# zjykzj/YOLOv4

Hardware: AMD Instinct MI355X
Metric: images/sec fwd+bwd @608x608 bs=64 per GPU (YOLOv4 training step: forward + YOLOLoss + backward) (higher is better)
Workload: dtype f32

## Files before the change

### include/yolov4_amd.h

```cpp
#ifndef YOLOV4_AMD_H
#define YOLOV4_AMD_H

#include <stddef.h>
#include <stdint.h>

#ifdef __cplusplus
extern "C" {
#endif

#define Y4_OK 0
#define Y4_ERR_SHAPE 1
#define Y4_ERR_NULL 2
#define Y4_ERR_LAUNCH 3
#define Y4_ERR_WORKSPACE 4
#define Y4_ERR_NODEVICE 5

#define Y4_ACT_LINEAR 0
#define Y4_ACT_LEAKY 1
#define Y4_ACT_MISH 2
#define Y4_ACT_RELU 3

const char* y4_strerror(int code);
int y4_version(void);
int y4_device_count(void);

int y4_set_conv_mode(int mode);
int y4_get_conv_mode(void);
int y4_set_planes_bf16(int on);
int y4_get_planes_bf16(void);
int y4_conv_planes_fit(int B, int H, int W, int Cin, int Cout, int k, int stride, int dgrad_planes);
size_t y4_conv2d_fwd_workspace(int Cin, int Cout, int k);
int y4_conv2d_fwd_f32(const float* x, int ldx, const float* w, float* y, int ldy,
                      int B, int H, int W, int Cin, int Cout, int k, int stride,
                      const float* scale, const float* shift, int act,
                      const float* residual, int ldr, const unsigned* x_amax ,
                      unsigned* y_amax ,
                      void* workspace, size_t workspace_bytes, void* stream);
size_t y4_conv2d_prepared_bytes(int Cout, int K);
int y4_conv2d_prepare_filter_f32(const float* w, int Cout, int K, void* prepared, size_t prepared_bytes, void* stream);
int y4_conv2d_fwd_prepared_f32(const float* x, int ldx, void* w_prepared, float* y, int ldy,
                               int B, int H, int W, int Cin, int Cout, int k, int stride,
                               const float* scale, const float* shift, int act,
                               const float* residual, int ldr, const unsigned* x_amax, unsigned* y_amax, void* stream);
int y4_amax_f32(const float* x, int ldx, long long M, int C, unsigned* amax_bits, void* stream);
int y4_amax_merge_u32(unsigned* dst, const unsigned* src, void* stream);

int y4_last_conv_kernel(char* buf, int cap);

size_t y4_conv2d_bnstats_workspace(int B, int H, int W, int Cin, int Cout, int k, int stride);
int y4_conv2d_fwd_bnstats_f32(const float* x, int ldx, const float* w, float* y, int ldy,
                              int B, int H, int W, int Cin, int Cout, int k, int stride,
                              float* partials, size_t partial_bytes, long long* nparts_host,
                              const unsigned* x_amax ,
                              void* workspace, size_t workspace_bytes ,
                              void* dgrad_filter ,
                              size_t dgrad_filter_bytes , void* stream);

int y4_planes_split_f32(const float* x, int ldx, long long M, int C, const unsigned* amax, void* planes, void* stream);
int y4_planes_split_into_f32(const float* x, int ldx, long long M, int C, const unsigned* amax, void* planes, int ld_planes, int c_valid,
                             void* stream);
int y4_conv2d_fwd_planes_f32(const void* x_planes, const float* w, float* y, int ldy,
                             int B, int H, int W, int Cin, int Cout, int k, int stride,
                             float* partials, size_t partial_bytes, long long* nparts_host, const unsigned* x_amax,
                             void* workspace, size_t workspace_bytes,
                             void* dgrad_filter ,
                             size_t dgrad_filter_bytes,
                             int y_bf16 ,
                             const float* bias ,
                             void* stream);

int y4_conv2d_dgrad_planes_f32(const void* dy_planes, const float* w , float* dx, int lddx,
                               int B, int H, int W, int Cin, int Cout, int k,
                               int stride ,
                               void* workspace, size_t workspace_bytes, const unsigned* dy_amax,
                               const float* residual, int ldr, void* stream);
size_t y4_conv2d_wgrad_planes_workspace(int B, int H, int W, int Cin, int Cout, int k, int stride);
int y4_conv2d_wgrad_planes_f32(const void* x_planes, const void* dy_planes, float* dw,
                               int B, int H, int W, int Cin, int Cout, int k, int stride,
                               void* workspace, size_t workspace_bytes, const unsigned* x_amax, const unsigned* dy_amax,
                               void* stream);

int y4_conv2d_generic_fwd_f32(const float* x, int ldx, const float* w, float* y, int ldy,
                              int B, int H, int W, int Cin, int Cout, int k, int stride,
                              const float* scale, const float* shift, int act, const float* residual, int ldr, void* stream);
int y4_conv2d_generic_dgrad_f32(const float* dy, int lddy, const float* w, float* dx, int lddx,
                                int B, int H, int W, int Cin, int Cout, int k, int stride,
                                const float* residual, int ldr, void* stream);
int y4_conv2d_generic_wgrad_f32(const float* x, int ldx, const float* dy, int lddy, float* dw,
                                int B, int H, int W, int Cin, int Cout, int k, int stride, void* stream);
int y4_conv2d_stem_dgrad_f32(const float* dy, int lddy, const float* w, float* dx, long long sxb, long long sxc, long long sxh,
                             long long sxw, int B, int H, int W, int Cout, void* stream);

int y4_conv2d_stem_fwd_f32(const float* x, long long sxb, long long sxc, long long sxh, long long sxw,
                           const float* w, float* y, int ldy, int B, int H, int W, int Cout,
                           const float* scale, const float* shift, int act,
                           float* bnstats_partials, void* stream);

size_t y4_conv2d_dgrad_workspace(int Cin, int Cout, int k);
int y4_conv2d_dgrad_f32(const float* dy, int lddy, const float* w , float* dx, int lddx,
                        int B, int H, int W, int Cin, int Cout, int k, int stride,
                        void* workspace, size_t workspace_bytes, const unsigned* dy_amax ,
                        const float* residual, int ldr, void* stream);

size_t y4_conv2d_wgrad_workspace(int B, int H, int W, int Cin, int Cout, int k, int stride);
int y4_conv2d_wgrad_f32(const float* x, int ldx, const float* dy, int lddy, float* dw,
                        int B, int H, int W, int Cin, int Cout, int k, int stride,
                        void* workspace, size_t workspace_bytes,
                        const unsigned* x_amax, const unsigned* dy_amax , void* stream);
size_t y4_conv2d_stem_wgrad_workspace(int B, int H, int W, int Cout);
int y4_conv2d_stem_wgrad_f32(const float* x, long long sxb, long long sxc, long long sxh, long long sxw,
                             const float* dy, int lddy, float* dw, int B, int H, int W, int Cout,
                             void* workspace, size_t workspace_bytes, void* stream);

size_t y4_bn_workspace(long long M, int C);
size_t y4_bn_finalize_workspace(int C);
int y4_bn_stats_f32(const float* y, int ldy, long long M, int C, float* mean, float* invstd,
                    float* running_mean, float* running_var, long long* num_batches_tracked,
                    float momentum, float eps, void* workspace, size_t workspace_bytes, void* stream);
int y4_bn_finalize_partials_f32(const float* partials, long long nparts, long long M, int C,
                                float* mean, float* invstd, float* running_mean, float* running_var,
                                long long* num_batches_tracked, float momentum, float eps,
                                void* workspace, size_t workspace_bytes, void* stream);
int y4_bn_planes_bound_f32(const float* gamma, const float* beta, int C, long long M, const unsigned* floor_word, unsigned* out,
                           void* stream);
int y4_bn_act_fwd_f32(const float* y, int ldy, const float* mean, const float* invstd,
                      const float* gamma, const float* beta, int act,
                      const float* residual, int ldr, float* z, int ldz,
                      long long M, int C, unsigned* out_amax, int z_planes, const unsigned* res_amax, float* planes_twin,
                      void* stream);
int y4_bn_act_bwd_f32(const float* dz, int lddz, const float* y, int ldy,
                      const float* mean, const float* invstd, const float* gamma, const float* beta,
                      int act, float* dy, int lddy, float* dgamma, float* dbeta,
                      long long M, int C, void* workspace, size_t workspace_bytes,
                      unsigned* out_amax ,
                      unsigned* f16_planes ,
                      float* planes_twin ,
                      int frozen_stats ,
                      void* stream);
size_t y4_bias_grad_workspace(long long M, int C);
int y4_bias_grad_f32(const float* dy, int lddy, long long M, int C, float* dbias,
                     void* workspace, size_t workspace_bytes, void* stream);
int y4_bn_fold_f32(const float* gamma, const float* beta, const float* running_mean,
                   const float* running_var, float eps, float* scale, float* shift, int C, void* stream);

int y4_copy_channels_f32(const float* src, int lds, float* dst, int ldd, long long M, int C, void* stream);
int y4_add_f32(const float* a, int lda, const float* b, int ldb, float* out, int ldo,
               long long M, int C, void* stream);
int y4_maxpool_s1_fwd_f32(const float* x, int ldx, float* y, int ldy, signed char* idx,
                          int B, int H, int W, int C, int ksize, void* stream);
int y4_maxpool_s1_bwd_f32(const float* dy, int lddy, const signed char* idx, float* dx, int lddx,
                          int accumulate, int B, int H, int W, int C, int ksize, void* stream);
int y4_upsample2x_fwd_f32(const float* x, int ldx, float* y, int ldy, int B, int H, int W, int C, void* stream);
int y4_upsample2x_bwd_f32(const float* dy, int lddy, float* dx, int lddx, int B, int H, int W, int C, void* stream);

int y4_yolo_decode_train_f32(const float* logits, int ldl, float* output, float* pred,
                             int B, int F, int A, int n_classes, const float* anchors_wh_host, void* stream);
int y4_yolo_decode_eval_f32(const float* logits, int ldl, float* out, long long n_total, long long box_off,
                            int B, int F, int A, int n_classes, const float* anchors_wh_host,
                            float stride, void* stream);
int y4_yolo_decode_bwd_f32(const float* logits, int ldl, const float* g_output, const float* g_pred,
                           float* g_logits, int B, int F, int A, int n_classes,
                           const float* anchors_wh_host, void* stream);

size_t y4_yolo_loss_workspace(int B, int F, int A, int K, int n_classes);
int y4_yolo_loss_fwd_f32(const float* output, const float* pred, const float* labels, int K,
                         int B, int F, int A, int n_classes, float stride, float ignore_thresh,
                         const float* all_anchors_host, int n_all_anchors, const int* anch_mask_host,
                         float* obj_mask, double* loss_parts,
                         void* workspace, size_t workspace_bytes, void* stream);
int y4_yolo_loss_bwd_f32(const float* output, int output_is_masked, const float* obj_mask,
                         const float* gscale, float* g_output,
                         int B, int F, int A, int K, int n_classes,
                         const void* workspace, size_t workspace_bytes, void* stream);
int y4_yolo_loss_mask_output_f32(float* output, const float* obj_mask, int B, int F, int A, int K,
                                 int n_classes, const void* workspace, size_t workspace_bytes, void* stream);
int y4_yolo_loss_dense_targets_f32(float* target, float* tgt_mask, float* tgt_scale,
                                   int B, int F, int A, int K, int n_classes,
                                   const void* workspace, size_t workspace_bytes, void* stream);

int y4_post_scan_i32(const int* counts, int n_segments, long long cap, int* seg_offsets, int* info, void* stream);
int y4_post_compact_f32(const float* det_rows, const int* seg_offsets, const int* kept, int B, int n_classes,
                        float* out_rows, int* out_offsets, int* img_offsets, void* stream);
int y4_post_count_f32(float* prediction, int B, long long N, int n_classes, float conf_thre,
                      int convert_xyxy, int* counts, void* stream);
size_t y4_post_nms_workspace(long long total_candidates, int n_segments);
int y4_post_nms_f32(const float* prediction, int B, long long N, int n_classes, float conf_thre,
                    float nms_thre, const int* seg_offsets , long long total_candidates,
                    float* det_rows , int* kept ,
                    void* workspace, size_t workspace_bytes, void* stream);
size_t y4_nms_workspace(long long R);
int y4_nms_f32(const float* boxes, const float* scores , long long R, float thresh,
               int limit, int* keep_idx , int* n_keep ,
               void* workspace, size_t workspace_bytes, void* stream);

int y4_bboxes_iou_f32(const float* boxes_a, long long Na, const float* boxes_b, long long Nb, int xyxy, float* iou,
                      void* stream);
int y4_act_fwd_f32(const float* x, float* y, long long n, int act, void* stream);
int y4_act_bwd_f32(const float* x, const float* dy, float* dx, long long n, int act, void* stream);
int y4_upsample_nearest_fwd_f32(const float* x, int ldx, float* y, int ldy, int B, int H, int W, int Ho, int Wo, int C,
                                int integer_factor, void* stream);
int y4_upsample_nearest_bwd_f32(const float* dy, int lddy, float* dx, int lddx, int B, int H, int W, int Ho, int Wo, int C,
                                int integer_factor, void* stream);

int y4_adam_step_f32(float* param, const float* grad, float* exp_avg, float* exp_avg_sq, long long n,
                     float lr, float beta1, float beta2, float eps, float weight_decay, int step,
                     float grad_scale, void* stream);
int y4_adam_hyper_f32(float lr, float beta1, float beta2, float weight_decay, int step, float* out4_host);
int y4_adam_multi_step_f32(const void* chunks_dev, int nchunks, const float* hyper_host, int nhyper,
                           float beta1, float beta2, float eps, float grad_scale, void* stream);
int y4_sgd_multi_step_f32(const void* chunks_dev, int nchunks, const float* hyper_host, int nhyper,
                          float grad_scale, void* stream);

int y4_preprocess_u8_f32(const void* src, int src_h, int src_w, long long src_pitch_bytes, int swap_rb,
                         float* dst, long long dst_sc, long long dst_sh, long long dst_sw, int S, void* stream);

#ifdef __cplusplus
}
#endif
#endif
```

### yolov4_amd/_lib.py

```python
import ctypes
import os
from ctypes import c_char_p, c_double, c_float, c_int, c_longlong, c_size_t, c_void_p

_HERE = os.path.dirname(os.path.abspath(__file__))
LIB_PATH = os.environ.get('Y4_LIB_PATH') or os.path.join(_HERE, 'lib', 'libyolov4_amd.so')

ACT_IDS = {'linear': 0, 'leaky_relu': 1, 'mish': 2, 'relu': 3}


class Y4Error(RuntimeError):
    pass


P = c_void_p
I, L, F, Z = c_int, c_longlong, c_float, c_size_t

PROTOTYPES = {
    'y4_strerror': (c_char_p, [I]),
    'y4_version': (I, []),
    'y4_device_count': (I, []),
    'y4_set_conv_mode': (I, [I]),
    'y4_get_conv_mode': (I, []),
    'y4_set_planes_bf16': (I, [I]),
    'y4_get_planes_bf16': (I, []),
    'y4_conv_planes_fit': (I, [I, I, I, I, I, I, I, I]),
    'y4_conv2d_fwd_workspace': (Z, [I, I, I]),
    'y4_conv2d_fwd_f32': (I, [P, I, P, P, I, I, I, I, I, I, I, I, P, P, I, P, I, P, P, P, Z, P]),
    'y4_amax_f32': (I, [P, I, L, I, P, P]),
    'y4_conv2d_prepared_bytes': (Z, [I, I]),
    'y4_conv2d_prepare_filter_f32': (I, [P, I, I, P, Z, P]),
    'y4_conv2d_fwd_prepared_f32': (I, [P, I, P, P, I, I, I, I, I, I, I, I, P, P, I, P, I, P, P, P]),
    'y4_amax_merge_u32': (I, [P, P, P]),
    'y4_last_conv_kernel': (I, [ctypes.c_char_p, I]),
    'y4_conv2d_bnstats_workspace': (Z, [I, I, I, I, I, I, I]),
    'y4_conv2d_fwd_bnstats_f32': (I, [P, I, P, P, I, I, I, I, I, I, I, I, P, Z, P, P, P, Z, P, Z, P]),
    'y4_planes_split_f32': (I, [P, I, L, I, P, P, P]),
    'y4_planes_split_into_f32': (I, [P, I, L, I, P, P, I, I, P]),
    'y4_conv2d_fwd_planes_f32': (I, [P, P, P, I, I, I, I, I, I, I, I, P, Z, P, P, P, Z, P, Z, I, P, P]),
    'y4_conv2d_dgrad_planes_f32': (I, [P, P, P, I, I, I, I, I, I, I, I, P, Z, P, P, I, P]),
    'y4_conv2d_wgrad_planes_workspace': (Z, [I, I, I, I, I, I, I]),
    'y4_conv2d_wgrad_planes_f32': (I, [P, P, P, I, I, I, I, I, I, I, P, Z, P, P, P]),
    'y4_conv2d_generic_fwd_f32': (I, [P, I, P, P, I, I, I, I, I, I, I, I, P, P, I, P, I, P]),
    'y4_conv2d_generic_dgrad_f32': (I, [P, I, P, P, I, I, I, I, I, I, I, I, P, I, P]),
    'y4_conv2d_generic_wgrad_f32': (I, [P, I, P, I, P, I, I, I, I, I, I, I, P]),
    'y4_conv2d_stem_dgrad_f32': (I, [P, I, P, P, L, L, L, L, I, I, I, I, P]),
    'y4_conv2d_stem_fwd_f32': (I, [P, L, L, L, L, P, P, I, I, I, I, I, P, P, I, P, P]),
    'y4_conv2d_dgrad_workspace': (Z, [I, I, I]),
    'y4_conv2d_dgrad_f32': (I, [P, I, P, P, I, I, I, I, I, I, I, I, P, Z, P, P, I, P]),
    'y4_conv2d_wgrad_workspace': (Z, [I, I, I, I, I, I, I]),
    'y4_conv2d_wgrad_f32': (I, [P, I, P, I, P, I, I, I, I, I, I, I, P, Z, P, P, P]),
    'y4_conv2d_stem_wgrad_workspace': (Z, [I, I, I, I]),
    'y4_conv2d_stem_wgrad_f32': (I, [P, L, L, L, L, P, I, P, I, I, I, I, P, Z, P]),
    'y4_bn_workspace': (Z, [L, I]),
    'y4_bn_finalize_workspace': (Z, [I]),
    'y4_bn_finalize_partials_f32': (I, [P, L, L, I, P, P, P, P, P, F, F, P, Z, P]),
    'y4_bn_stats_f32': (I, [P, I, L, I, P, P, P, P, P, F, F, P, Z, P]),
    'y4_bn_act_fwd_f32': (I, [P, I, P, P, P, P, I, P, I, P, I, L, I, P, I, P, P, P]),
    'y4_bn_planes_bound_f32': (I, [P, P, I, L, P, P, P]),
    'y4_bn_act_bwd_f32': (I, [P, I, P, I, P, P, P, P, I, P, I, P, P, L, I, P, Z, P, P, P, I, P]),
    'y4_bias_grad_workspace': (Z, [L, I]),
    'y4_bias_grad_f32': (I, [P, I, L, I, P, P, Z, P]),
    'y4_bn_fold_f32': (I, [P, P, P, P, F, P, P, I, P]),
    'y4_copy_channels_f32': (I, [P, I, P, I, L, I, P]),
    'y4_add_f32': (I, [P, I, P, I, P, I, L, I, P]),
    'y4_maxpool_s1_fwd_f32': (I, [P, I, P, I, P, I, I, I, I, I, P]),
    'y4_maxpool_s1_bwd_f32': (I, [P, I, P, P, I, I, I, I, I, I, I, P]),
    'y4_upsample2x_fwd_f32': (I, [P, I, P, I, I, I, I, I, P]),
    'y4_upsample2x_bwd_f32': (I, [P, I, P, I, I, I, I, I, P]),
    'y4_yolo_decode_train_f32': (I, [P, I, P, P, I, I, I, I, P, P]),
    'y4_yolo_decode_eval_f32': (I, [P, I, P, L, L, I, I, I, I, P, F, P]),
    'y4_yolo_decode_bwd_f32': (I, [P, I, P, P, P, I, I, I, I, P, P]),
    'y4_yolo_loss_workspace': (Z, [I, I, I, I, I]),
    'y4_yolo_loss_fwd_f32': (I, [P, P, P, I, I, I, I, I, F, F, P, I, P, P, P, P, Z, P]),
    'y4_yolo_loss_bwd_f32': (I, [P, I, P, P, P, I, I, I, I, I, P, Z, P]),
    'y4_yolo_loss_mask_output_f32': (I, [P, P, I, I, I, I, I, P, Z, P]),
    'y4_yolo_loss_dense_targets_f32': (I, [P, P, P, I, I, I, I, I, P, Z, P]),
    'y4_post_count_f32': (I, [P, I, L, I, F, I, P, P]),
    'y4_post_scan_i32': (I, [P, I, L, P, P, P]),
    'y4_post_compact_f32': (I, [P, P, P, I, I, P, P, P, P]),
    'y4_post_nms_workspace': (Z, [L, I]),
    'y4_post_nms_f32': (I, [P, I, L, I, F, F, P, L, P, P, P, Z, P]),
    'y4_nms_workspace': (Z, [L]),
    'y4_nms_f32': (I, [P, P, L, F, I, P, P, P, Z, P]),
    'y4_bboxes_iou_f32': (I, [P, L, P, L, I, P, P]),
    'y4_act_fwd_f32': (I, [P, P, L, I, P]),
    'y4_act_bwd_f32': (I, [P, P, P, L, I, P]),
    'y4_upsample_nearest_fwd_f32': (I, [P, I, P, I, I, I, I, I, I, I, I, P]),
    'y4_upsample_nearest_bwd_f32': (I, [P, I, P, I, I, I, I, I, I, I, I, P]),
    'y4_adam_step_f32': (I, [P, P, P, P, L, F, F, F, F, F, I, F, P]),
    'y4_adam_hyper_f32': (I, [F, F, F, F, I, P]),
    'y4_adam_multi_step_f32': (I, [P, I, P, I, F, F, F, F, P]),
    'y4_sgd_multi_step_f32': (I, [P, I, P, I, F, P]),
    'y4_preprocess_u8_f32': (I, [P, I, I, L, I, P, L, L, L, I, P]),
}

_lib = None


def lib():
    global _lib
    if _lib is None:
        if not os.path.isfile(LIB_PATH):
            raise Y4Error(f'{LIB_PATH} is missing: build it with `make -C yolov4_amd/csrc` '
                          '(hipcc --offload-arch=gfx950); there is no fallback path')
        handle = ctypes.CDLL(LIB_PATH)
        for name, (res, args) in PROTOTYPES.items():
            fn = getattr(handle, name)
            fn.restype = res
            fn.argtypes = args
        _lib = handle
        if os.environ.get('Y4_CONV_MODE'):
            handle.y4_set_conv_mode(int(os.environ['Y4_CONV_MODE']))
    return _lib


def check(code, what=''):
    if code != 0:
        msg = lib().y4_strerror(code).decode()
        raise Y4Error(f'{what}: {msg} (code {code})')


def float_array(values):
    arr = (c_float * len(values))(*[float(v) for v in values])
    return arr


def int_array(values):
    return (c_int * len(values))(*[int(v) for v in values])
```

### yolov4_amd/csrc/conv_geom.h

```cpp
#pragma once
#include "common.h"

namespace y4 {

struct ConvGeom {
    const float* src; const float* wt; float* dst;
    const float* scale; const float* shift; const float* res;
    float* stats;
    long long lds_, ldd, ldr;
    int B, Hs, Ws, Cs;
    int Cs_valid;
    int Hd, Wd, N;
    int k, stride, pad;
    int M;
    int K;
    int act;
    int mtiles, ntiles;
    int cls_tile0[5];
    int cls_h[2], cls_w[2];
    int cls_slot0[5];
    unsigned long long src_total_bytes;
    unsigned wt_bytes;
    const unsigned short* wt_planes;
    const unsigned* src_amax; const unsigned* wt_amax;
    unsigned* dst_amax;
};

struct WgradGeom {
    const float* x; const float* dy; float* out;
    long long ldx, lddy;
    int B, H, W, Cin, Ho, Wo, Cout;
    int k, stride, pad;
    int M;
    int J;
    int ntn, ntj, splits, chunks_per_split;
    int tn, tj;
    const unsigned* x_amax; const unsigned* dy_amax;
    unsigned long long x_total_bytes, dy_total_bytes;
};

int f16x2_gather(const ConvGeom& g, bool transposed, hipStream_t st, int* nparts);
int f16x2_wgrad(const WgradGeom& g, hipStream_t st);
int f16x2_refresh_prepared(const float* w, void* prepared, int Cout, int K, hipStream_t st);
int f16x2_filter_planes(const float* w, unsigned short* planes, int Cout, int K, unsigned* amax_out, unsigned* part, hipStream_t st);
int f16x2_filter_planes_dual(const float* w, unsigned short* planes, unsigned* amax_out, unsigned* part, unsigned short* planes_t,
                             unsigned* amax_out_t, int Cout, int Cin, int kk, int Cout_pad, bool mirror, hipStream_t st);
int f16x2_filter_planes_transposed(const float* w, unsigned short* planes, int Cout, int Cin, int kk, int Cout_pad,
                                   unsigned* amax_out, unsigned* part, hipStream_t st, bool mirror = false);
int slab_reduce(const float* slabs, float* dw, long long n, int splits, hipStream_t st);
int amax_launch(const float* x, long long ld, long long M, int C, unsigned* amax_bits, hipStream_t st,
                bool prezeroed = false);
int amax_merge(unsigned* dst, const unsigned* src, hipStream_t st);


bool tile_conv_ok(int Cs, int Cs_valid, int N, int k, int stride, int H, int W);
int f16x2_tile(const ConvGeom& g, hipStream_t st, int* nparts);
bool tile_dgrad_s2_ok(int Cs, int Cs_valid, int N, int k, int stride, int Hs, int Ws);
int f16x2_tile_dgrad_s2(const ConvGeom& g, hipStream_t st);

bool tile_wgrad_ok(int Cin, int Cout, int k, int stride, int H, int W, long long ldx, long long lddy);
int tile_wgrad_slabs(int Cin, int Cout);
int f16x2_wgrad_tile(const WgradGeom& g, hipStream_t st);

bool planes_conv_ok(int Cin, int Cout, int k, int stride);
int planes_conv(const void* src, const unsigned* src_amax, const void* wt_planes, const unsigned* wt_amax, float* dst, long long ldd,
                const float* res, long long ldr, float* stats, int* nparts, int B, int Hs, int Ws, int Cs, int N, int k, int stride,
                hipStream_t st, bool bf = false, bool dst_bf16 = false);
int planes_dgrad_s2(const void* dy, const unsigned* dy_amax, const void* wt_planes, const unsigned* wt_amax, float* dx, long long lddx,
                    int B, int H, int W, int Cin, int Cout, hipStream_t st, bool bf = false);
int planes_split(const float* x, long long ld, long long M, int C, const unsigned* amax, void* planes, hipStream_t st, bool bf = false,
                 long long pitch_ch = 0, int c_valid = 0);
void planes_wgrad_plan(int B, int H, int W, int Cin, int Cout, int k, int* ntn, int* ntj, int* splits, int* sps, int tn = 128, bool bf = false);
int planes_wgrad_tn(int Cout, bool bf);
int planes_wgrad(const void* x, const unsigned* x_amax, const void* dy, const unsigned* dy_amax, float* dw, void* workspace,
                 size_t workspace_bytes, int B, int H, int W, int Cin, int Cout, int k, hipStream_t st, bool bf = false,
                 int stride = 1);

void note_kernel(const char* fmt, ...);
}
```

### yolov4_amd/csrc/conv_igemm.hip

```cpp
#include <stdlib.h>
#include "common.h"
#include <cstdarg>
#include <cstdio>
#include "conv_geom.h"

namespace {

constexpr int BK = 32;


using y4::ConvGeom;
using y4::WgradGeom;

template <int BM, int BN, int WM, int WN, bool TRANSPOSED, int BKT = 32>
__global__ __launch_bounds__(256, (BKT == 16 ? 3 : 2)) void conv_gather_mfma_f32(const ConvGeom g) {
    constexpr int LPR = BKT / 4;
    constexpr int RPP = 256 / LPR;
    constexpr int PA = BM / RPP, PB = BN / RPP;
    constexpr int LDS_PITCH = BKT + 4;
    constexpr int BK = BKT;
    constexpr int WTM = BM / WM, WTN = BN / WN;
    constexpr int TM = WTM / 32, TN = WTN / 32;
    static_assert(WM * WN == 4, "4 waves");
    extern __shared__ __attribute__((aligned(16))) float smem[];
// ... 1073 lines not shown
    f32x4 ra[4], rb[4];
    int ld_chunk = 0;
    auto load_chunk = [&]() {
        const int pbase = (chunk0 + ld_chunk) * 32 + pg * 4;
#pragma unroll
        for (int i = 0; i < 4; ++i) {
            const bool ok = an_ok && pbase + i < g.M;
            ra[i] = y4_buf_load4(dy_rsrc, ok ? a_off0 + (unsigned)i * dy_pix_bytes : OOB, (unsigned)ld_chunk * chunk_bytes);
        }
#pragma unroll
        for (int i = 0; i < 4; ++i) {
            const int hi = pb_h[i] * g.stride - g.pad + jr, wi = pb_w[i] * g.stride - g.pad + jq;
            const bool ok = bj_ok && pbase + i < g.M && (unsigned)hi < (unsigned)g.H && (unsigned)wi < (unsigned)g.W;
            const unsigned off = (unsigned)((pb_b[i] * g.H + hi) * g.W + wi) * x_pix_bytes + (unsigned)jc * 4u;
            rb[i] = y4_buf_load4(x_rsrc, ok ? off : OOB, 0u);
            pb_w[i] += 32;
            while (pb_w[i] >= g.Wo) { pb_w[i] -= g.Wo; if (++pb_h[i] == g.Ho) { pb_h[i] = 0; ++pb_b[i]; } }
        }
        ++ld_chunk;
    };
    auto split_store = [&](const f32x4 (&v)[4], unsigned char* base, int rows) {
        if constexpr (NP == 1) {
#pragma unroll
            for (int e = 0; e < 4; ++e) {
                u32x2 p;
                p[0] = pack_hi16(rn_bf16_bits(v[1][e]), rn_bf16_bits(v[0][e]));
                p[1] = pack_hi16(rn_bf16_bits(v[3][e]), rn_bf16_bits(v[2][e]));
                *reinterpret_cast<u32x2*>(base + (cg * 4 + e) * PITCH_B + pg * 8) = p;
            }
            return;
        }
        unsigned h1[4][4], h2[4][4], h3[4][4];
#pragma unroll
        for (int i = 0; i < 4; ++i)
#pragma unroll
            for (int e = 0; e < 4; ++e) {
                h1[i][e] = __float_as_uint(v[i][e]);
                const float r1 = v[i][e] - __uint_as_float(h1[i][e] & 0xffff0000u);
                h2[i][e] = __float_as_uint(r1);
                const float r2 = r1 - __uint_as_float(h2[i][e] & 0xffff0000u);
                h3[i][e] = __float_as_uint(r2);
            }
#pragma unroll
        for (int e = 0; e < 4; ++e) {
            unsigned char* d = base + (cg * 4 + e) * PITCH_B + pg * 8;
            u32x2 p;
            p[0] = pack_hi16(h1[1][e], h1[0][e]); p[1] = pack_hi16(h1[3][e], h1[2][e]);
            *reinterpret_cast<u32x2*>(d) = p;
            p[0] = pack_hi16(h2[1][e], h2[0][e]); p[1] = pack_hi16(h2[3][e], h2[2][e]);
            *reinterpret_cast<u32x2*>(d + rows * PITCH_B) = p;
            p[0] = pack_hi16(h3[1][e], h3[0][e]); p[1] = pack_hi16(h3[3][e], h3[2][e]);
            *reinterpret_cast<u32x2*>(d + 2 * rows * PITCH_B) = p;
        }
    };
    auto store_chunk = [&]() {
        if (a_act) split_store(ra, As, TN_);
        if (b_act) split_store(rb, Bs, TJ_);
    };

    f32x16 acc[MI][MJ];
#pragma unroll
    for (int i = 0; i < MI; ++i)
#pragma unroll
        for (int jj = 0; jj < MJ; ++jj)
#pragma unroll
            for (int e = 0; e < 16; ++e) acc[i][jj][e] = 0.f;

    const int fr = lane & 31, fh = lane >> 5;
    const unsigned char* a_frag = As + (wm * (TN_ / 2) + fr) * PITCH_B + fh * 16;
    const unsigned char* b_frag = Bs + (wn * (TJ_ / 2) + fr) * PITCH_B + fh * 16;
    if (nchunks > 0) {
        load_chunk();
        store_chunk();
        __syncthreads();
        for (int ch = 0; ch < nchunks; ++ch) {
            if (ch + 1 < nchunks) load_chunk();
#pragma unroll
            for (int ks = 0; ks < 2; ++ks) {
                bf16x8 fa[MI][NP], fb[MJ][NP];
#pragma unroll
                for (int i = 0; i < MI; ++i)
#pragma unroll
                    for (int pl = 0; pl < NP; ++pl)
                        fa[i][pl] = *reinterpret_cast<const bf16x8*>(a_frag + pl * TN_ * PITCH_B + i * 32 * PITCH_B + ks * 32);
#pragma unroll
                for (int jj = 0; jj < MJ; ++jj)
#pragma unroll
                    for (int pl = 0; pl < NP; ++pl)
                        fb[jj][pl] = *reinterpret_cast<const bf16x8*>(b_frag + pl * TJ_ * PITCH_B + jj * 32 * PITCH_B + ks * 32);
#pragma unroll
                for (int i = 0; i < MI; ++i)
#pragma unroll
                    for (int jj = 0; jj < MJ; ++jj) {
                        f32x16 c = acc[i][jj];
                        if constexpr (NP == 3) {
                            c = __builtin_amdgcn_mfma_f32_32x32x16_bf16(fa[i][2], fb[jj][0], c, 0, 0, 0);
                            c = __builtin_amdgcn_mfma_f32_32x32x16_bf16(fa[i][1], fb[jj][1], c, 0, 0, 0);
                            c = __builtin_amdgcn_mfma_f32_32x32x16_bf16(fa[i][0], fb[jj][2], c, 0, 0, 0);
                            c = __builtin_amdgcn_mfma_f32_32x32x16_bf16(fa[i][1], fb[jj][0], c, 0, 0, 0);
                            c = __builtin_amdgcn_mfma_f32_32x32x16_bf16(fa[i][0], fb[jj][1], c, 0, 0, 0);
                        }
                        c = __builtin_amdgcn_mfma_f32_32x32x16_bf16(fa[i][0], fb[jj][0], c, 0, 0, 0);
                        acc[i][jj] = c;
                    }
            }
            __syncthreads();
            if (ch + 1 < nchunks) store_chunk();
            __syncthreads();
        }
    }
    float* out = g.out + (long long)split * g.Cout * g.J;
#pragma unroll
    for (int jj = 0; jj < MJ; ++jj) {
        const int jcol = j0 + wn * (TJ_ / 2) + jj * 32 + fr;
#pragma unroll
        for (int i = 0; i < MI; ++i) {
            const int nb = n0 + wm * (TN_ / 2) + i * 32 + 4 * fh;
#pragma unroll
            for (int e = 0; e < 16; ++e) {
                const int n = nb + (e & 3) + 8 * (e >> 2);
                if (n < g.Cout && jcol < g.J) out[(long long)n * g.J + jcol] = acc[i][jj][e];
            }
        }
    }
}

template <int VEC>
__global__ __launch_bounds__(256) void slab_reduce_vec_kernel(const f32x4* __restrict__ slabs, f32x4* __restrict__ out,
                                                              long long nvec, int splits) {
    constexpr int SG = 256 / VEC;
    __shared__ f32x4 red[SG][VEC];
    const int v = threadIdx.x % VEC, sg = threadIdx.x / VEC;
    const long long i = (long long)blockIdx.x * VEC + v;
    f32x4 s0 = {0.f, 0.f, 0.f, 0.f}, s1 = s0, s2 = s0, s3 = s0;
    if (i < nvec) {
        int k = sg;
        for (; k + 3 * SG < splits; k += 4 * SG) {
            const f32x4 a = slabs[(long long)k * nvec + i], b = slabs[(long long)(k + SG) * nvec + i];
            const f32x4 c = slabs[(long long)(k + 2 * SG) * nvec + i], d = slabs[(long long)(k + 3 * SG) * nvec + i];
            s0 += a; s1 += b; s2 += c; s3 += d;
        }
        for (; k < splits; k += SG) s0 += slabs[(long long)k * nvec + i];
    }
    red[sg][v] = (s0 + s1) + (s2 + s3);
    __syncthreads();
    if (sg == 0 && i < nvec) {
        f32x4 t = red[0][v];
#pragma unroll
        for (int g = 1; g < SG; ++g) t += red[g][v];
        out[i] = t;
    }
}

__global__ void slab_reduce_kernel(const float* __restrict__ slabs, float* __restrict__ out,
                                   long long n, int splits) {
    for (long long i = blockIdx.x * (long long)blockDim.x + threadIdx.x; i < n;
         i += (long long)gridDim.x * blockDim.x) {
        float s = 0.f;
        for (int k = 0; k < splits; ++k) s += slabs[(long long)k * n + i];
        out[i] = s;
    }
}

void wgrad_plan(int B, int H, int W, int Cin, int Cout, int k, int stride, WgradGeom& g) {
    const int pad = (k - 1) / 2;
    g.B = B; g.H = H; g.W = W; g.Cin = Cin; g.Cout = Cout; g.k = k; g.stride = stride; g.pad = pad;
    g.Ho = (H + 2 * pad - k) / stride + 1;
    g.Wo = (W + 2 * pad - k) / stride + 1;
    g.M = B * g.Ho * g.Wo;
    g.J = k * k * Cin;
    g.tn = Cout <= 64 ? 64 : 128;
    g.tj = g.J <= 64 ? 64 : 128;
    g.ntn = (Cout + g.tn - 1) / g.tn;
    g.ntj = (g.J + g.tj - 1) / g.tj;
    const int tiles = g.ntn * g.ntj;
    const int chunks = (g.M + 31) / 32;
    int per_cu = (160 * 1024) / (2 * 32 * (g.tn + g.tj) * 4);
    if (per_cu > 4) per_cu = 4;
    if (g.tn + g.tj == 256 && per_cu > 2) per_cu = 2;
    const int slots = 256 * per_cu;
    int max_s = chunks / 16;
    if (max_s < 1) max_s = 1;
    if (max_s > 4096) max_s = 4096;
    int best_s = 1;
    double best_eff = -1.0;
    for (int sp = 1; sp <= max_s; ++sp) {
        const long long blocks = (long long)tiles * sp;
        const long long rounds = (blocks + slots - 1) / slots;
        double eff = (double)blocks / (double)(rounds * slots);
        if (rounds > 6) eff = 1.0;
        if (eff > best_eff + 0.02) { best_eff = eff; best_s = sp; }
        if (blocks >= 2ll * slots && eff >= 0.93) break;
        if (blocks >= 6ll * slots) break;
    }
    { static const char* fs = getenv("Y4_WGRAD_SPLITS"); if (fs) { best_s = atoi(fs); if (best_s > max_s) best_s = max_s; if (best_s < 1) best_s = 1; } }
    g.chunks_per_split = (chunks + best_s - 1) / best_s;
    const unsigned long long per_px = 8ull * (unsigned long long)((Cout + 3) / 4 * 4 > Cin * stride * stride ? (Cout + 3) / 4 * 4 : Cin * stride * stride);
    const unsigned long long slack = 2ull * g.Ho * g.Wo;
    const unsigned long long max_px = 0xf0000000ull / per_px;
    if (max_px > slack + 32 && (unsigned long long)g.chunks_per_split * 32ull + slack > max_px)
        g.chunks_per_split = (int)((max_px - slack) / 32ull);
    g.splits = (chunks + g.chunks_per_split - 1) / g.chunks_per_split;
}

template <int TN_, int TJ_, int NP = 0>
int launch_wgrad(const WgradGeom& g, hipStream_t st) {
    constexpr bool SPLIT = NP > 0;
    const size_t smem = SPLIT ? (size_t)NP * (TN_ + TJ_) * 80 : 2ull * 32 * (TN_ + TJ_) * sizeof(float);
    void (*kern)(const WgradGeom);
    if constexpr (SPLIT) kern = conv_wgrad_bf16x3<TN_, TJ_, (NP > 0 ? NP : 3)>;
    else kern = conv_wgrad_mfma_f32<TN_, TJ_>;
    static Y4DynLds lds_attr;
    if (!lds_attr.ensure(reinterpret_cast<const void*>(kern), smem)) return Y4_ERR_LAUNCH;
    hipLaunchKernelGGL(kern, dim3(g.ntn * g.ntj * g.splits), dim3(256), smem, st, g);
    Y4_CHECK_LAUNCH();
    return Y4_OK;
}

struct StemGeom {
    const float* x; const float* w; float* y; const float* scale; const float* shift;
    float* stats;
    long long sxb, sxc, sxh, sxw, ldy;
    int B, H, W, Cout, act;
    long long M;
};

__global__ __launch_bounds__(256) void conv_stem_fwd_kernel(const StemGeom g) {
    __shared__ float tile[4][64][33];
    __shared__ __attribute__((aligned(16))) float wl[27 * 32];
    const int tid = threadIdx.x, lane = tid & 63, wave = tid >> 6;
    for (int i = tid; i < 27 * 32; i += 256) {
        const int n = i & 31, kk = i >> 5;
        wl[i] = n < g.Cout ? g.w[n * 27 + kk] : 0.f;
    }
    __syncthreads();
    const long long pix0 = (long long)blockIdx.x * 256 + wave * 64;
    const long long pix = pix0 + lane;
    float acc[32];
#pragma unroll
    for (int n = 0; n < 32; ++n) acc[n] = 0.f;
    if (pix < g.M) {
        const int b = (int)(pix / ((long long)g.H * g.W));
        const int rem = (int)(pix - (long long)b * g.H * g.W);
        const int h = rem / g.W, w = rem - h * g.W;
        const float* xb = g.x + b * g.sxb;
        float xv[27];
#pragma unroll
        for (int r = 0; r < 3; ++r)
#pragma unroll
            for (int q = 0; q < 3; ++q) {
                const int hi = h + r - 1, wi = w + q - 1;
                const bool ok = (unsigned)hi < (unsigned)g.H && (unsigned)wi < (unsigned)g.W;
#pragma unroll
                for (int c = 0; c < 3; ++c) xv[(r * 3 + q) * 3 + c] = ok ? xb[c * g.sxc + hi * g.sxh + wi * g.sxw] : 0.f;
            }
#pragma unroll
        for (int kk = 0; kk < 27; ++kk) {
            const f32x4* wp = reinterpret_cast<const f32x4*>(wl + kk * 32);
            const float v = xv[kk];
#pragma unroll
            for (int n4 = 0; n4 < 8; ++n4) {
                const f32x4 wv = wp[n4];
#pragma unroll
                for (int e = 0; e < 4; ++e) acc[n4 * 4 + e] = fmaf(v, wv[e], acc[n4 * 4 + e]);
            }
            __builtin_amdgcn_sched_barrier(0);
        }
    }
#pragma unroll
    for (int n = 0; n < 32; ++n) {
        float v = acc[n];
        if (n < g.Cout) {
            v = v * (g.scale ? g.scale[n] : 1.f) + (g.shift ? g.shift[n] : 0.f);
            v = y4_act(v, g.act);
        }
        tile[wave][lane][n] = v;
    }
    __syncthreads();
    const int ch = lane & 31;
    if (ch < g.Cout) {
#pragma unroll 4
        for (int it = 0; it < 32; ++it) {
            const int pl = it * 2 + (lane >> 5);
            const long long p = pix0 + pl;
            if (p < g.M) g.y[p * g.ldy + ch] = tile[wave][pl][ch];
        }
    }
    if (g.stats) {
        __shared__ float sred[8][32][2];
        const int grp = tid >> 5;
        float cs = 0.f, css = 0.f;
        for (int i = 0; i < 32; ++i) { const float v = tile[grp >> 1][(grp & 1) * 32 + i][ch]; cs += v; css += v * v; }
        sred[grp][ch][0] = cs; sred[grp][ch][1] = css;
        __syncthreads();
        if (tid < 64) {
            const int c = tid & 31, which = tid >> 5;
            float t = 0.f;
            for (int k = 0; k < 8; ++k) t += sred[k][c][which];
            if (c < g.Cout) g.stats[((long long)blockIdx.x * 2 + which) * g.Cout + c] = t;
        }
    }
}

__global__ __launch_bounds__(256) void conv_stem_fwd_bf16x3_kernel(const StemGeom g, const int ngroups, const float inv_hw,
                                                                   const float inv_w) {
    __shared__ float sred[4][32][2];
    const int tid = threadIdx.x, lane = tid & 63, wave = tid >> 6;
    const int fr = lane & 31, fh = lane >> 5;
    const int HW = g.H * g.W;
    bf16x8 fb[2][3];
    int koff[16];
    int ktap[16];
#pragma unroll
    for (int i = 0; i < 16; ++i) {
        const int k = (i >> 3) * 16 + fh * 8 + (i & 7);
        const int r = k / 9, c = (k - r * 9) / 3, q = k - r * 9 - c * 3;
        const bool kv = k < 27;
        koff[i] = kv ? (int)(c * g.sxc + (r - 1) * g.sxh + (q - 1) * g.sxw) * 4 : 0;
        ktap[i] = kv ? r * 3 + q : 9;
    }
#pragma unroll
    for (int ks = 0; ks < 2; ++ks) {
        f32x4 w0, w1;
#pragma unroll
        for (int i = 0; i < 8; ++i) {
            const int k = ks * 16 + fh * 8 + i;
            const int r = k / 9, c = (k - r * 9) / 3, q = k - r * 9 - c * 3;
            const float v = (k < 27 && fr < g.Cout) ? g.w[fr * 27 + (r * 3 + q) * 3 + c] : 0.f;
            if (i < 4) w0[i] = v; else w1[i - 4] = v;
        }
        u32x2 a1, a2, a3, b1, b2, b3;
        split3x4(w0, a1, a2, a3);
        split3x4(w1, b1, b2, b3);
        const u32x4 q1 = {a1[0], a1[1], b1[0], b1[1]}, q2 = {a2[0], a2[1], b2[0], b2[1]}, q3 = {a3[0], a3[1], b3[0], b3[1]};
        fb[ks][0] = __builtin_bit_cast(bf16x8, q1); fb[ks][1] = __builtin_bit_cast(bf16x8, q2); fb[ks][2] = __builtin_bit_cast(bf16x8, q3);
    }
    const float sc = (g.scale && fr < g.Cout) ? g.scale[fr] : 1.f;
    const float sh = (g.shift && fr < g.Cout) ? g.shift[fr] : 0.f;
    const __amdgpu_buffer_rsrc_t rsrc = y4_make_rsrc(g.x, 0xfffffff0u);
    float xv0[16], xv1[16];
    auto load = [&](float (&xv)[16], long long tile) {
        const long long p = tile * 32 + fr;
        unsigned base = 0xffffffffu;
        unsigned m9 = 0;
        if (p < g.M) {
            int b = (int)((float)p * inv_hw);
            int rem = (int)(p - (long long)b * HW);
            if (rem < 0) { --b; rem += HW; } else if (rem >= HW) { ++b; rem -= HW; }
            int h = (int)((float)rem * inv_w);
            int w = rem - h * g.W;
            if (w < 0) { --h; w += g.W; } else if (w >= g.W) { ++h; w -= g.W; }
            base = (unsigned)(b * g.sxb + h * g.sxh + w * g.sxw) * 4u;
            const unsigned hm = (h > 0 ? 1u : 0u) | 2u | (h + 1 < g.H ? 4u : 0u);
            const unsigned wm = (w > 0 ? 1u : 0u) | 2u | (w + 1 < g.W ? 4u : 0u);
            m9 = ((hm & 1u) ? wm : 0u) | ((hm & 2u) ? wm << 3 : 0u) | ((hm & 4u) ? wm << 6 : 0u);
        }
#pragma unroll
        for (int i = 0; i < 16; ++i) {
            const bool ok = (m9 >> ktap[i]) & 1u;
            xv[i] = __builtin_bit_cast(float, __builtin_amdgcn_raw_buffer_load_b32(rsrc, ok ? (int)(base + (unsigned)koff[i]) : -1, 0, 0));
        }
    };
    float cs = 0.f, css = 0.f;
    auto compute = [&](float (&xv)[16], long long tile) {
        f32x16 acc;
#pragma unroll
        for (int e = 0; e < 16; ++e) acc[e] = 0.f;
#pragma unroll
        for (int ks = 0; ks < 2; ++ks) {
            const f32x4 v0 = {xv[ks * 8 + 0], xv[ks * 8 + 1], xv[ks * 8 + 2], xv[ks * 8 + 3]};
            const f32x4 v1 = {xv[ks * 8 + 4], xv[ks * 8 + 5], xv[ks * 8 + 6], xv[ks * 8 + 7]};
            u32x2 a1, a2, a3, b1, b2, b3;
            split3x4(v0, a1, a2, a3);
            split3x4(v1, b1, b2, b3);
            const u32x4 q1 = {a1[0], a1[1], b1[0], b1[1]}, q2 = {a2[0], a2[1], b2[0], b2[1]}, q3 = {a3[0], a3[1], b3[0], b3[1]};
            const bf16x8 f1 = __builtin_bit_cast(bf16x8, q1), f2 = __builtin_bit_cast(bf16x8, q2), f3 = __builtin_bit_cast(bf16x8, q3);
            acc = __builtin_amdgcn_mfma_f32_32x32x16_bf16(f3, fb[ks][0], acc, 0, 0, 0);
            acc = __builtin_amdgcn_mfma_f32_32x32x16_bf16(f2, fb[ks][1], acc, 0, 0, 0);
            acc = __builtin_amdgcn_mfma_f32_32x32x16_bf16(f1, fb[ks][2], acc, 0, 0, 0);
            acc = __builtin_amdgcn_mfma_f32_32x32x16_bf16(f2, fb[ks][0], acc, 0, 0, 0);
            acc = __builtin_amdgcn_mfma_f32_32x32x16_bf16(f1, fb[ks][1], acc, 0, 0, 0);
            acc = __builtin_amdgcn_mfma_f32_32x32x16_bf16(f1, fb[ks][0], acc, 0, 0, 0);
        }
        const long long mbase = tile * 32 + 4 * fh;
#pragma unroll
        for (int e = 0; e < 16; ++e) {
            const float raw = acc[e];
            cs += raw; css += raw * raw;
            const long long m = mbase + (e & 3) + 8 * (e >> 2);
            if (fr < g.Cout && m < g.M) g.y[m * g.ldy + fr] = y4_act(raw * sc + sh, g.act);
        }
    };
    for (int grp = blockIdx.x; grp < ngroups; grp += gridDim.x) {
        const long long t0 = (long long)grp * 8 + wave * 2;
        load(xv0, t0);
        load(xv1, t0 + 1);
        cs = 0.f; css = 0.f;
        compute(xv0, t0);
        compute(xv1, t0 + 1);
        if (g.stats) {
            cs += __shfl_xor(cs, 32, 64);
            css += __shfl_xor(css, 32, 64);
            if (fh == 0) { sred[wave][fr][0] = cs; sred[wave][fr][1] = css; }
            __syncthreads();
            if (tid < 64) {
                const int c = tid & 31, which = tid >> 5;
                const float t = (sred[0][c][which] + sred[1][c][which]) + (sred[2][c][which] + sred[3][c][which]);
                if (c < g.Cout) g.stats[((long long)grp * 2 + which) * g.Cout + c] = t;
            }
            __syncthreads();
        }
    }
}

struct StemWgradGeom {
    const float* x; const float* dy; float* slabs;
    long long sxb, sxc, sxh, sxw, lddy;
    int B, H, W, Cout;
    long long M, pix_per_wave;
};

__global__ __launch_bounds__(256) void conv_stem_wgrad_kernel(const StemWgradGeom g) {
    const int tid = threadIdx.x, lane = tid & 63;
    const long long wave_id = (long long)blockIdx.x * 4 + (tid >> 6);
    const long long p_begin = wave_id * g.pix_per_wave;
    long long p_end = p_begin + g.pix_per_wave;
    if (p_end > g.M) p_end = g.M;
    const int fr = lane & 31, fh = lane >> 5;
    const bool jok = fr < 27;
    const int tap = jok ? fr / 3 : 0, c = jok ? fr - tap * 3 : 0;
    const int r = tap / 3 - 1, q = tap - (tap / 3) * 3 - 1;
    const bool nok = fr < g.Cout;
    f32x16 acc;
#pragma unroll
    for (int e = 0; e < 16; ++e) acc[e] = 0.f;
    long long p = p_begin + fh;
    int b = 0, h = 0, w = 0;
    if (p < g.M) {
        b = (int)(p / ((long long)g.H * g.W));
        const int rem = (int)(p - (long long)b * g.H * g.W);
        h = rem / g.W; w = rem - h * g.W;
    }
    const long long dy_first = p_begin < g.M ? p_begin : 0;
    const __amdgpu_buffer_rsrc_t dy_rsrc = y4_make_rsrc(g.dy + dy_first * g.lddy, (unsigned)(g.pix_per_wave * g.lddy * 4));
    const __amdgpu_buffer_rsrc_t x_rsrc = y4_make_rsrc(g.x, 0xfffffff0u);
    const unsigned dy_step = (unsigned)g.lddy * 8u;
    unsigned dy_off = ((unsigned)fh * (unsigned)g.lddy + (unsigned)fr) * 4u;
    const long long coff = c * g.sxc;
    for (long long pc = p_begin; pc < p_end; pc += 16) {
        float a[8], bv[8];
#pragma unroll
        for (int u = 0; u < 8; ++u) {
            const bool pok = p < p_end;
            const int hi = h + r, wi = w + q;
            const bool xok = pok && jok && (unsigned)hi < (unsigned)g.H && (unsigned)wi < (unsigned)g.W;
            const unsigned xo = (unsigned)(b * g.sxb + coff + hi * g.sxh + wi * g.sxw) * 4u;
            a[u] = __builtin_bit_cast(float, __builtin_amdgcn_raw_buffer_load_b32(dy_rsrc, (pok && nok) ? (int)dy_off : -1, 0, 0));
            bv[u] = __builtin_bit_cast(float, __builtin_amdgcn_raw_buffer_load_b32(x_rsrc, xok ? (int)xo : -1, 0, 0));
            dy_off += dy_step;
            p += 2;
            w += 2;
            if (w >= g.W) { w -= g.W; if (++h == g.H) { h = 0; ++b; } }
        }
#pragma unroll
        for (int u = 0; u < 8; ++u) acc = __builtin_amdgcn_mfma_f32_32x32x2f32(a[u], bv[u], acc, 0, 0, 0);
    }
    float* out = g.slabs + wave_id * 1024;
#pragma unroll
    for (int e = 0; e < 16; ++e) {
        const int n = (e & 3) + 8 * (e >> 2) + 4 * fh;
        out[n * 32 + fr] = acc[e];
    }
}

__global__ __launch_bounds__(256) void stem_wgrad_reduce1_kernel(const float* __restrict__ slabs, double* __restrict__ part,
                                                                 int nslabs) {
    const int per = (nslabs + gridDim.x - 1) / gridDim.x;
    const int k0 = blockIdx.x * per;
    const int k1 = min(nslabs, k0 + per);
    double s[4] = {0, 0, 0, 0};
    for (int k = k0; k < k1; ++k) {
        const f32x4 v = *reinterpret_cast<const f32x4*>(slabs + (long long)k * 1024 + threadIdx.x * 4);
#pragma unroll
        for (int e = 0; e < 4; ++e) s[e] += (double)v[e];
    }
#pragma unroll
    for (int e = 0; e < 4; ++e) part[(long long)blockIdx.x * 1024 + threadIdx.x * 4 + e] = s[e];
}
__global__ __launch_bounds__(256) void stem_wgrad_reduce2_kernel(const double* __restrict__ part, float* __restrict__ dw,
                                                                 int nparts, int Cout) {
    for (int i = threadIdx.x; i < Cout * 27; i += 256) {
        const int n = i / 27, j = i - n * 27;
        double s = 0.0;
        for (int k = 0; k < nparts; ++k) s += part[(long long)k * 1024 + n * 32 + j];
        dw[i] = (float)s;
    }
}

constexpr int STEM_WAVES = 4096;

}

namespace y4 {
int slab_reduce(const float* slabs, float* dw, long long n, int splits, hipStream_t st) {
    if ((n & 3) == 0 && !(reinterpret_cast<uintptr_t>(dw) & 15) && !(reinterpret_cast<uintptr_t>(slabs) & 15)) {
        const long long nvec = n / 4;
        if (nvec >= 64 * 1024)
            hipLaunchKernelGGL(slab_reduce_vec_kernel<64>, dim3((unsigned)((nvec + 63) / 64)), dim3(256), 0, st,
                               reinterpret_cast<const f32x4*>(slabs), reinterpret_cast<f32x4*>(dw), nvec, splits);
        else
            hipLaunchKernelGGL(slab_reduce_vec_kernel<16>, dim3((unsigned)((nvec + 15) / 16)), dim3(256), 0, st,
                               reinterpret_cast<const f32x4*>(slabs), reinterpret_cast<f32x4*>(dw), nvec, splits);
    } else {
        const int blocks = (int)((n + 255) / 256 > 2048 ? 2048 : (n + 255) / 256);
        hipLaunchKernelGGL(slab_reduce_kernel, dim3(blocks), dim3(256), 0, st, slabs, dw, n, splits);
    }
    Y4_CHECK_LAUNCH();
    return Y4_OK;
}
}

extern "C" {

int y4_set_conv_mode(int mode) {
    if (mode < 0 || mode > 3) return Y4_ERR_SHAPE;
    g_conv_mode = mode;
    return Y4_OK;
}
int y4_get_conv_mode(void) { return g_conv_mode; }

constexpr size_t FWD_WS_HDR = 64 + 4096;

size_t y4_conv2d_fwd_workspace(int Cin, int Cout, int k) {
    if (Cin <= 0 || Cout <= 0 || k <= 0) return 0;
    return FWD_WS_HDR + (size_t)Cout * k * k * Cin * 6;
}

static int conv_fwd_impl(const float* x, int ldx, const float* w, float* y, int ldy,
                         int B, int H, int W, int Cin, int Cout, int k, int stride,
                         const float* scale, const float* shift, int act,
                         const float* residual, int ldr, float* stats, int* nparts, const unsigned* x_amax,
                         unsigned* y_amax, void* workspace, size_t workspace_bytes, void* stream,
                         void* w_prepared = nullptr, void* dgrad_filter = nullptr, size_t dgrad_filter_bytes = 0) {
    if (!x || (!w && !w_prepared) || !y) return Y4_ERR_NULL;
    if (B <= 0 || H <= 0 || W <= 0 || Cout <= 0 || (k != 1 && k != 3) || (stride != 1 && stride != 2))
        return Y4_ERR_SHAPE;
    if (Cin <= 0 || Cin % BK != 0 || ldx < Cin || ldy < Cout || (ldx & 3) || (residual && ldr < Cout))
        return Y4_ERR_SHAPE;
    if ((reinterpret_cast<uintptr_t>(x) & 15) || (reinterpret_cast<uintptr_t>(w) & 15)) return Y4_ERR_SHAPE;
    const int pad = (k - 1) / 2;
    ConvGeom g{};
    g.src = x; g.wt = w; g.dst = y; g.scale = scale; g.shift = shift; g.res = residual; g.stats = stats;
    g.lds_ = ldx; g.ldd = ldy; g.ldr = ldr;
    g.B = B; g.Hs = H; g.Ws = W; g.Cs = Cin; g.Cs_valid = Cin;
    g.Hd = (H + 2 * pad - k) / stride + 1;
    g.Wd = (W + 2 * pad - k) / stride + 1;
    g.N = Cout; g.k = k; g.stride = stride; g.pad = pad;
    const long long M = (long long)B * g.Hd * g.Wd;
    if (M >= (1ll << 31)) return Y4_ERR_SHAPE;
    g.M = (int)M; g.K = k * k * Cin; g.act = act;
    if (w_prepared) {
        if (g_conv_mode != 3) return Y4_ERR_SHAPE;
        if (reinterpret_cast<uintptr_t>(w_prepared) & 15) return Y4_ERR_SHAPE;
        unsigned* hdr = static_cast<unsigned*>(w_prepared);
        g.wt_planes = reinterpret_cast<unsigned short*>(static_cast<char*>(w_prepared) + 64 + 4096);
        if (!x_amax) {
            const int rc = y4::amax_launch(x, ldx, (long long)B * H * W, Cin, hdr + 1, y4_stream(stream));
            if (rc != Y4_OK) return rc;
            x_amax = hdr + 1;
        }
        g.src_amax = x_amax; g.wt_amax = hdr; g.dst_amax = y_amax;
        return y4::f16x2_gather(g, false, y4_stream(stream), nparts);
    }
    if (g_conv_mode != 0) {
        const long long nw = (long long)Cout * g.K;
        if (!workspace) return Y4_ERR_NULL;
        if (workspace_bytes < y4_conv2d_fwd_workspace(Cin, Cout, k)) return Y4_ERR_WORKSPACE;
        if (reinterpret_cast<uintptr_t>(workspace) & 15) return Y4_ERR_SHAPE;
        unsigned* hdr = static_cast<unsigned*>(workspace);
        unsigned short* planes = reinterpret_cast<unsigned short*>(static_cast<char*>(workspace) + FWD_WS_HDR);
        g.wt_planes = planes;
        if (g_conv_mode == 3) {
            int rc;
            if (dgrad_filter) {
                if (dgrad_filter_bytes < y4_conv2d_dgrad_workspace(Cin, Cout, k)) return Y4_ERR_WORKSPACE;
                if (reinterpret_cast<uintptr_t>(dgrad_filter) & 15) return Y4_ERR_SHAPE;
                const int cp = (Cout + 31) / 32 * 32;
                unsigned* hdr_t = reinterpret_cast<unsigned*>(static_cast<char*>(dgrad_filter) + (size_t)Cin * k * k * cp * 6);
                rc = y4::f16x2_filter_planes_dual(w, planes, hdr, hdr + 16, static_cast<unsigned short*>(dgrad_filter), hdr_t, Cout, Cin,
                                                  k * k, cp, y4::tile_conv_ok(cp, Cout, Cin, k, stride, H, W), y4_stream(stream));
            } else {
                rc = y4::f16x2_filter_planes(w, planes, Cout, g.K, hdr, hdr + 16, y4_stream(stream));
            }
            if (rc != Y4_OK) return rc;
            if (!x_amax) {
                rc = y4::amax_launch(x, ldx, (long long)B * H * W, Cin, hdr + 1, y4_stream(stream));
                if (rc != Y4_OK) return rc;
                x_amax = hdr + 1;
            }
            g.src_amax = x_amax; g.wt_amax = hdr; g.dst_amax = y_amax;
            return y4::f16x2_gather(g, false, y4_stream(stream), nparts);
        }
        const int blocks = (int)((nw + 255) / 256 > 4096 ? 4096 : (nw + 255) / 256);
        hipLaunchKernelGGL(split_filter_kernel, dim3(blocks), dim3(256), 0, y4_stream(stream), w, planes, nw,
                           g_conv_mode == 2 ? 1 : 3);
        Y4_CHECK_LAUNCH();
    }
    return dispatch_gather<false>(g, y4_stream(stream), nparts);
}

int y4_conv2d_fwd_f32(const float* x, int ldx, const float* w, float* y, int ldy,
                      int B, int H, int W, int Cin, int Cout, int k, int stride,
                      const float* scale, const float* shift, int act,
                      const float* residual, int ldr, const unsigned* x_amax, unsigned* y_amax,
                      void* workspace, size_t workspace_bytes, void* stream) {
    return conv_fwd_impl(x, ldx, w, y, ldy, B, H, W, Cin, Cout, k, stride, scale, shift, act, residual, ldr, nullptr,
                         nullptr, x_amax, y_amax, workspace, workspace_bytes, stream);
}

int y4_amax_f32(const float* x, int ldx, long long M, int C, unsigned* amax_bits, void* stream) {
    if (!x || !amax_bits) return Y4_ERR_NULL;
    if (M < 0 || C <= 0 || ldx < C) return Y4_ERR_SHAPE;
    return y4::amax_launch(x, ldx, M, C, amax_bits, y4_stream(stream));
}

int y4_amax_merge_u32(unsigned* dst, const unsigned* src, void* stream) {
    if (!dst || !src) return Y4_ERR_NULL;
    return y4::amax_merge(dst, src, y4_stream(stream));
}

size_t y4_conv2d_bnstats_workspace(int B, int H, int W, int Cin, int Cout, int k, int stride) {
    if (B <= 0 || H <= 0 || W <= 0 || Cout <= 0 || (k != 1 && k != 3) || (stride != 1 && stride != 2)) return 0;
    const int pad = (k - 1) / 2;
    const long long M = (long long)B * ((H + 2 * pad - k) / stride + 1) * ((W + 2 * pad - k) / stride + 1);
    long long rows = Cin == 3 ? (M + 255) / 256 : (M + 63) / 64;
    const long long per_img = (long long)B * ((M / B + 127) / 128);
    if (per_img > rows) rows = per_img;
    return (size_t)rows * 2 * Cout * sizeof(float);
}

int y4_conv2d_fwd_bnstats_f32(const float* x, int ldx, const float* w, float* y, int ldy,
                              int B, int H, int W, int Cin, int Cout, int k, int stride,
                              float* partials, size_t partial_bytes, long long* nparts_host, const unsigned* x_amax,
                              void* workspace, size_t workspace_bytes, void* dgrad_filter, size_t dgrad_filter_bytes,
                              void* stream) {
    if (!partials || !nparts_host) return Y4_ERR_NULL;
    if (dgrad_filter && g_conv_mode != 3) return Y4_ERR_SHAPE;
    if (partial_bytes < y4_conv2d_bnstats_workspace(B, H, W, Cin, Cout, k, stride)) return Y4_ERR_WORKSPACE;
    int np = 0;
    const int rc = conv_fwd_impl(x, ldx, w, y, ldy, B, H, W, Cin, Cout, k, stride, nullptr, nullptr, Y4_ACT_LINEAR,
                                 nullptr, 0, partials, &np, x_amax, nullptr, workspace, workspace_bytes, stream, nullptr,
                                 dgrad_filter, dgrad_filter_bytes);
    if (rc != Y4_OK) return rc;
    *nparts_host = np;
    return Y4_OK;
}

size_t y4_conv2d_dgrad_workspace(int Cin, int Cout, int k) {
    const size_t cp = (size_t)((Cout + 31) / 32) * 32;
    return (size_t)Cin * k * k * cp * 6 + 64 + 4096;
}

static int conv_dgrad_impl(const float* dy, int lddy, const float* w, float* dx, int lddx,
                           int B, int H, int W, int Cin, int Cout, int k, int stride,
                           void* workspace, size_t workspace_bytes, const unsigned* dy_amax,
                           const float* residual, int ldr, void* stream) {
    if (!dy || !dx || !workspace) return Y4_ERR_NULL;
    if (!w && g_conv_mode != 3) return Y4_ERR_NULL;
    if (B <= 0 || H <= 0 || W <= 0 || Cin <= 0 || Cout <= 0 || (k != 1 && k != 3) || (stride != 1 && stride != 2))
        return Y4_ERR_SHAPE;
    const int Cout_pad = (Cout + 31) / 32 * 32;
    if (lddy < Cout_pad || (lddy & 3) || lddx < Cin) return Y4_ERR_SHAPE;
    if (workspace_bytes < y4_conv2d_dgrad_workspace(Cin, Cout, k)) return Y4_ERR_WORKSPACE;
    if ((reinterpret_cast<uintptr_t>(dy) & 15) || (reinterpret_cast<uintptr_t>(workspace) & 15)) return Y4_ERR_SHAPE;
    hipStream_t st = y4_stream(stream);
    float* wt = static_cast<float*>(workspace);
    const long long total = (long long)Cin * k * k * Cout_pad;
    const int blocks = (int)((total + 255) / 256 > 4096 ? 4096 : (total + 255) / 256);
    unsigned* hdr = reinterpret_cast<unsigned*>(static_cast<char*>(workspace) + (size_t)total * 6);
    unsigned* wamax = hdr;
    if (g_conv_mode == 3) {
        if (w) {
            const int rc = y4::f16x2_filter_planes_transposed(w, static_cast<unsigned short*>(workspace), Cout, Cin, k * k, Cout_pad,
                                                              wamax, hdr + 16, st, y4::tile_conv_ok(Cout_pad, Cout, Cin, k, stride, H, W));
            if (rc != Y4_OK) return rc;
        }
    } else if (g_conv_mode != 0)
        hipLaunchKernelGGL(transpose_split_filter_kernel, dim3(blocks), dim3(256), 0, st, w,
                           static_cast<unsigned short*>(workspace), Cout, Cin, k * k, Cout_pad, g_conv_mode == 2 ? 1 : 3);
    else
        hipLaunchKernelGGL(transpose_filter_kernel, dim3(blocks), dim3(256), 0, st, w, wt, Cout, Cin, k * k, Cout_pad);
    Y4_CHECK_LAUNCH();
    const int pad = (k - 1) / 2;
    ConvGeom g{};
    if (residual && ldr < Cin) return Y4_ERR_SHAPE;
    g.src = dy; g.wt = wt; g.dst = dx; g.scale = nullptr; g.shift = nullptr; g.res = residual;
    g.wt_planes = static_cast<const unsigned short*>(workspace);
    g.lds_ = lddy; g.ldd = lddx; g.ldr = ldr;
    g.B = B;
    g.Hs = (H + 2 * pad - k) / stride + 1;
    g.Ws = (W + 2 * pad - k) / stride + 1;
    g.Cs = Cout_pad; g.Cs_valid = Cout;
    g.Hd = H; g.Wd = W; g.N = Cin; g.k = k; g.stride = stride; g.pad = pad;
    const long long M = (long long)B * H * W;
    if (M >= (1ll << 31)) return Y4_ERR_SHAPE;
    g.M = (int)M; g.K = k * k * Cout_pad; g.act = Y4_ACT_LINEAR;
    if (g_conv_mode == 3) {
        if (!dy_amax) {
            const int rc = y4::amax_launch(dy, lddy, (long long)B * g.Hs * g.Ws, Cout, hdr + 1, st);
            if (rc != Y4_OK) return rc;
            dy_amax = hdr + 1;
        }
        g.src_amax = dy_amax; g.wt_amax = wamax;
        if (y4::tile_conv_ok(Cout_pad, Cout, Cin, k, stride, H, W)) return y4::f16x2_tile(g, st, nullptr);
        if (y4::tile_dgrad_s2_ok(Cout_pad, Cout, Cin, k, stride, g.Hs, g.Ws)) return y4::f16x2_tile_dgrad_s2(g, st);
        return y4::f16x2_gather(g, true, st, nullptr);
    }
    return dispatch_gather<true>(g, st);
}

int y4_conv2d_dgrad_f32(const float* dy, int lddy, const float* w, float* dx, int lddx,
                        int B, int H, int W, int Cin, int Cout, int k, int stride,
                        void* workspace, size_t workspace_bytes, const unsigned* dy_amax,
                        const float* residual, int ldr, void* stream) {
    return conv_dgrad_impl(dy, lddy, w, dx, lddx, B, H, W, Cin, Cout, k, stride, workspace, workspace_bytes, dy_amax,
                           residual, ldr, stream);
}

int y4_last_conv_kernel(char* buf, int cap) {
    if (!buf || cap <= 0) return Y4_ERR_NULL;
    snprintf(buf, (size_t)cap, "%s", g_last_kernel);
    g_last_kernel[0] = 0;
    return Y4_OK;
}

size_t y4_conv2d_prepared_bytes(int Cout, int K) {
    if (Cout <= 0 || K <= 0) return 0;
    return 64 + 4096 + (size_t)Cout * (size_t)K * 4;
}

int y4_conv2d_prepare_filter_f32(const float* w, int Cout, int K, void* prepared, size_t prepared_bytes, void* stream) {
    if (!w || !prepared) return Y4_ERR_NULL;
    if (Cout <= 0 || K <= 0 || (K & 31)) return Y4_ERR_SHAPE;
    if (prepared_bytes < y4_conv2d_prepared_bytes(Cout, K)) return Y4_ERR_WORKSPACE;
    if ((reinterpret_cast<uintptr_t>(prepared) & 15) || (reinterpret_cast<uintptr_t>(w) & 15)) return Y4_ERR_SHAPE;
    return y4::f16x2_refresh_prepared(w, prepared, Cout, K, y4_stream(stream));
}

int y4_conv2d_fwd_prepared_f32(const float* x, int ldx, void* w_prepared, float* y, int ldy,
                               int B, int H, int W, int Cin, int Cout, int k, int stride,
                               const float* scale, const float* shift, int act,
                               const float* residual, int ldr, const unsigned* x_amax, unsigned* y_amax, void* stream) {
    if (!w_prepared) return Y4_ERR_NULL;
    return conv_fwd_impl(x, ldx, nullptr, y, ldy, B, H, W, Cin, Cout, k, stride, scale, shift, act, residual, ldr, nullptr,
                         nullptr, x_amax, y_amax, nullptr, 0, stream, w_prepared);
}

size_t y4_conv2d_wgrad_workspace(int B, int H, int W, int Cin, int Cout, int k, int stride) {
    WgradGeom g{};
    wgrad_plan(B, H, W, Cin, Cout, k, stride, g);
    int splits = g.splits;
    if (y4::tile_wgrad_ok(Cin, Cout, k, stride, H, W, 0, 0) && y4::tile_wgrad_slabs(Cin, Cout) > splits) splits = y4::tile_wgrad_slabs(Cin, Cout);
    return (splits > 1 ? (size_t)splits * Cout * g.J * sizeof(float) : 0) + 64;
}

int y4_conv2d_wgrad_f32(const float* x, int ldx, const float* dy, int lddy, float* dw,
                        int B, int H, int W, int Cin, int Cout, int k, int stride,
                        void* workspace, size_t workspace_bytes, const unsigned* x_amax, const unsigned* dy_amax,
                        void* stream) {
    if (!x || !dy || !dw) return Y4_ERR_NULL;
    if (B <= 0 || H <= 0 || W <= 0 || Cout <= 0 || (k != 1 && k != 3) || (stride != 1 && stride != 2))
        return Y4_ERR_SHAPE;
    if (Cin <= 0 || (Cin & 3) || ldx < Cin || (ldx & 3) || (lddy & 3) || lddy < ((Cout + 3) & ~3)) return Y4_ERR_SHAPE;
    if ((reinterpret_cast<uintptr_t>(x) & 15) || (reinterpret_cast<uintptr_t>(dy) & 15)) return Y4_ERR_SHAPE;
    WgradGeom g{};
    wgrad_plan(B, H, W, Cin, Cout, k, stride, g);
    if ((long long)B * g.Ho * g.Wo >= (1ll << 31)) return Y4_ERR_SHAPE;
    g.x = x; g.dy = dy; g.ldx = ldx; g.lddy = lddy;
    {
        g.x_total_bytes = (unsigned long long)B * H * W * (unsigned long long)ldx * 4ull;
        g.dy_total_bytes = (unsigned long long)B * g.Ho * g.Wo * (unsigned long long)lddy * 4ull;
        const unsigned long long range_px = (unsigned long long)g.chunks_per_split * 32ull + 2ull * g.Ho * g.Wo;
        const unsigned long long per_px = 4ull * (unsigned long long)(lddy > ldx * stride * stride ? lddy : ldx * stride * stride);
        if (range_px * per_px >= 0xfffffff0ull) return Y4_ERR_SHAPE;
    }
    hipStream_t st = y4_stream(stream);
    const bool tile = g_conv_mode == 3 && y4::tile_wgrad_ok(Cin, Cout, k, stride, H, W, ldx, lddy);
    if (tile) g.splits = y4::tile_wgrad_slabs(Cin, Cout);
    const size_t slab_bytes = g.splits > 1 ? (size_t)g.splits * Cout * g.J * sizeof(float) : 0;
    if (g.splits > 1) {
        if (!workspace) return Y4_ERR_NULL;
        if (workspace_bytes < slab_bytes) return Y4_ERR_WORKSPACE;
        g.out = static_cast<float*>(workspace);
    } else {
        g.out = dw;
    }
    int rc;
    if (g_conv_mode == 3) {
        if (!x_amax || !dy_amax) {
            if (!workspace || workspace_bytes < slab_bytes + 64) return Y4_ERR_WORKSPACE;
            unsigned* hdr = reinterpret_cast<unsigned*>(static_cast<char*>(workspace) + slab_bytes);
            if (!x_amax) {
                rc = y4::amax_launch(x, ldx, (long long)B * H * W, Cin, hdr, st);
                if (rc != Y4_OK) return rc;
                x_amax = hdr;
            }
            if (!dy_amax) {
                rc = y4::amax_launch(dy, lddy, (long long)B * g.Ho * g.Wo, Cout, hdr + 1, st);
                if (rc != Y4_OK) return rc;
                dy_amax = hdr + 1;
            }
        }
        g.x_amax = x_amax; g.dy_amax = dy_amax;
        rc = tile ? y4::f16x2_wgrad_tile(g, st) : y4::f16x2_wgrad(g, st);
    } else if (g_conv_mode == 1) {
        if (g.tn == 128 && g.tj == 128) rc = launch_wgrad<128, 128, 3>(g, st);
        else if (g.tn == 128) rc = launch_wgrad<128, 64, 3>(g, st);
        else if (g.tj == 128) rc = launch_wgrad<64, 128, 3>(g, st);
        else rc = launch_wgrad<64, 64, 3>(g, st);
    } else if (g_conv_mode == 2) {
        if (g.tn == 128 && g.tj == 128) rc = launch_wgrad<128, 128, 1>(g, st);
        else if (g.tn == 128) rc = launch_wgrad<128, 64, 1>(g, st);
        else if (g.tj == 128) rc = launch_wgrad<64, 128, 1>(g, st);
        else rc = launch_wgrad<64, 64, 1>(g, st);
    } else if (g.tn == 128 && g.tj == 128) rc = launch_wgrad<128, 128>(g, st);
    else if (g.tn == 128) rc = launch_wgrad<128, 64>(g, st);
    else if (g.tj == 128) rc = launch_wgrad<64, 128>(g, st);
    else rc = launch_wgrad<64, 64>(g, st);
    if (rc != Y4_OK) return rc;
    if (g.splits > 1) {
        const int rc2 = y4::slab_reduce(static_cast<const float*>(workspace), dw, (long long)Cout * g.J, g.splits, st);
        if (rc2 != Y4_OK) return rc2;
    }
    return Y4_OK;
}

int y4_conv2d_stem_fwd_f32(const float* x, long long sxb, long long sxc, long long sxh, long long sxw,
                           const float* w, float* y, int ldy, int B, int H, int W, int Cout,
                           const float* scale, const float* shift, int act,
                           float* bnstats_partials, void* stream) {
    if (!x || !w || !y) return Y4_ERR_NULL;
    if (B <= 0 || H <= 0 || W <= 0 || Cout <= 0 || Cout > 32 || ldy < Cout) return Y4_ERR_SHAPE;
    StemGeom g{};
    g.x = x; g.w = w; g.y = y; g.scale = scale; g.shift = shift; g.stats = bnstats_partials;
    g.sxb = sxb; g.sxc = sxc; g.sxh = sxh; g.sxw = sxw; g.ldy = ldy;
    g.B = B; g.H = H; g.W = W; g.Cout = Cout; g.act = act;
    g.M = (long long)B * H * W;
    const long long blocks = (g.M + 255) / 256;
    if (blocks >= (1ll << 31)) return Y4_ERR_SHAPE;
    const bool mfma_ok = (g_conv_mode >= 1 && g_conv_mode <= 3) && sxb >= 0 && sxc >= 0 && sxh >= 0 && sxw >= 0 &&
                         ((long long)(B - 1) * sxb + 2 * sxc + (long long)(H - 1) * sxh + (long long)(W - 1) * sxw + 1) * 4 < 0xfffffff0ll &&
                         (long long)H * W < (1 << 24);
    if (mfma_ok) {
        const int grid = (int)(blocks < 2048 ? blocks : 2048);
        hipLaunchKernelGGL(conv_stem_fwd_bf16x3_kernel, dim3(grid), dim3(256), 0, y4_stream(stream), g, (int)blocks,
                           1.0f / (float)((long long)H * W), 1.0f / (float)W);
        Y4_CHECK_LAUNCH();
        return Y4_OK;
    }
    hipLaunchKernelGGL(conv_stem_fwd_kernel, dim3((unsigned)blocks), dim3(256), 0, y4_stream(stream), g);
    Y4_CHECK_LAUNCH();
    return Y4_OK;
}

size_t y4_conv2d_stem_wgrad_workspace(int, int, int, int) {
    return (size_t)STEM_WAVES * 1024 * sizeof(float) + 64 * 1024 * sizeof(double);
}

int y4_conv2d_stem_wgrad_f32(const float* x, long long sxb, long long sxc, long long sxh, long long sxw,
                             const float* dy, int lddy, float* dw, int B, int H, int W, int Cout,
                             void* workspace, size_t workspace_bytes, void* stream) {
    if (!x || !dy || !dw || !workspace) return Y4_ERR_NULL;
    if (B <= 0 || H <= 0 || W < 2 || Cout <= 0 || Cout > 32 || lddy < Cout) return Y4_ERR_SHAPE;
    if (workspace_bytes < y4_conv2d_stem_wgrad_workspace(B, H, W, Cout)) return Y4_ERR_WORKSPACE;
    StemWgradGeom g{};
    g.x = x; g.dy = dy; g.slabs = static_cast<float*>(workspace);
    g.sxb = sxb; g.sxc = sxc; g.sxh = sxh; g.sxw = sxw; g.lddy = lddy;
    g.B = B; g.H = H; g.W = W; g.Cout = Cout;
    g.M = (long long)B * H * W;
    long long ppw = (g.M + STEM_WAVES - 1) / STEM_WAVES;
    ppw = (ppw + 15) & ~15ll;
    if ((long long)ppw * lddy * 4 >= 0xfffffff0ll || sxb < 0 || sxc < 0 || sxh < 0 || sxw < 0 ||
        ((long long)(B - 1) * sxb + 2 * sxc + (long long)(H - 1) * sxh + (long long)(W - 1) * sxw + 1) * 4 >= 0xfffffff0ll)
        return Y4_ERR_SHAPE;
    g.pix_per_wave = ppw;
    hipStream_t st = y4_stream(stream);
    hipLaunchKernelGGL(conv_stem_wgrad_kernel, dim3(STEM_WAVES / 4), dim3(256), 0, st, g);
    Y4_CHECK_LAUNCH();
    double* part = reinterpret_cast<double*>(static_cast<char*>(workspace) + (size_t)STEM_WAVES * 1024 * sizeof(float));
    hipLaunchKernelGGL(stem_wgrad_reduce1_kernel, dim3(64), dim3(256), 0, st, static_cast<const float*>(workspace), part,
                       STEM_WAVES);
    Y4_CHECK_LAUNCH();
    hipLaunchKernelGGL(stem_wgrad_reduce2_kernel, dim3(1), dim3(256), 0, st, part, dw, 64, Cout);
    Y4_CHECK_LAUNCH();
    return Y4_OK;
}

}
```

### yolov4_amd/csrc/pointwise.hip

```cpp
#include "common.h"

namespace {

constexpr int PW_THREADS = 256;
constexpr int PW_UNROLL = 4;
#define Y4_ACT_SWITCH(ACTV, CALL)                                              \
    switch (ACTV) {                                                            \
        case Y4_ACT_MISH: { constexpr int A_ = Y4_ACT_MISH; CALL; } break;     \
        case Y4_ACT_LEAKY: { constexpr int A_ = Y4_ACT_LEAKY; CALL; } break;   \
        case Y4_ACT_RELU: { constexpr int A_ = Y4_ACT_RELU; CALL; } break;     \
        default: { constexpr int A_ = Y4_ACT_LINEAR; CALL; } break;            \
    }

struct RowMap {
    int tpr;
    int rpb;
};
static inline RowMap row_map(int C) {
    RowMap r;
    int c4 = C / 4;
    r.tpr = c4 < PW_THREADS ? c4 : PW_THREADS;
    int p = 1;
    while (p * 2 <= r.tpr) p *= 2;
    r.tpr = p;
// ... 694 lines not shown
    for (long long i = blockIdx.x * (long long)blockDim.x + threadIdx.x; i < total;
         i += (long long)gridDim.x * blockDim.x) {
        const int c = (int)(i % C4) * 4;
        const long long pix = i / C4;
        const int w = (int)(pix % W);
        const int h = (int)((pix / W) % H);
        const long long b = pix / ((long long)W * H);
        const long long o = (b * H2 + 2 * h) * W2 + 2 * w;
        f32x4 s = ld4(dy + o * lddy + c) + ld4(dy + (o + 1) * lddy + c);
        s += ld4(dy + (o + W2) * lddy + c) + ld4(dy + (o + W2 + 1) * lddy + c);
        st4(dx + pix * lddx + c, s);
    }
}

__device__ __forceinline__ int nearest_src(int d, int f, float scale, int n_in) {
    if (f > 0) return d / f;
    const int s = (int)floorf((float)d * scale);
    return s < n_in - 1 ? s : n_in - 1;
}
__global__ __launch_bounds__(PW_THREADS) void upsample_nearest_fwd_kernel(const float* __restrict__ x, long long ldx,
                                                                          float* __restrict__ y, long long ldy,
                                                                          int B, int H, int W, int Ho, int Wo, int C4,
                                                                          int fh, int fw, float sh, float sw) {
    const long long total = (long long)B * Ho * Wo * C4;
    for (long long i = blockIdx.x * (long long)blockDim.x + threadIdx.x; i < total;
         i += (long long)gridDim.x * blockDim.x) {
        const int c = (int)(i % C4) * 4;
        const long long pix = i / C4;
        const int w = (int)(pix % Wo);
        const int h = (int)((pix / Wo) % Ho);
        const long long b = pix / ((long long)Wo * Ho);
        const int hs = nearest_src(h, fh, sh, H), ws = nearest_src(w, fw, sw, W);
        st4(y + pix * ldy + c, ld4(x + ((b * H + hs) * W + ws) * ldx + c));
    }
}
__device__ __forceinline__ void nearest_range(int s, int f, float scale, int n_in, int n_out, int& lo, int& hi) {
    if (f > 0) { lo = s * f; hi = lo + f; if (hi > n_out) hi = n_out; return; }
    int d = (int)((float)s / scale) - 2;
    if (d < 0) d = 0;
    while (d < n_out && nearest_src(d, 0, scale, n_in) < s) ++d;
    lo = d;
    while (d < n_out && nearest_src(d, 0, scale, n_in) == s) ++d;
    hi = d;
}
__global__ __launch_bounds__(PW_THREADS) void upsample_nearest_bwd_kernel(const float* __restrict__ dy, long long lddy,
                                                                          float* __restrict__ dx, long long lddx,
                                                                          int B, int H, int W, int Ho, int Wo, int C4,
                                                                          int fh, int fw, float sh, float sw) {
    const long long total = (long long)B * H * W * C4;
    for (long long i = blockIdx.x * (long long)blockDim.x + threadIdx.x; i < total;
         i += (long long)gridDim.x * blockDim.x) {
        const int c = (int)(i % C4) * 4;
        const long long pix = i / C4;
        const int w = (int)(pix % W);
        const int h = (int)((pix / W) % H);
        const long long b = pix / ((long long)W * H);
        int h0, h1, w0, w1;
        nearest_range(h, fh, sh, H, Ho, h0, h1);
        nearest_range(w, fw, sw, W, Wo, w0, w1);
        f32x4 s = {0.f, 0.f, 0.f, 0.f};
        for (int hh = h0; hh < h1; ++hh)
            for (int ww = w0; ww < w1; ++ww) s += ld4(dy + ((b * Ho + hh) * Wo + ww) * lddy + c);
        st4(dx + pix * lddx + c, s);
    }
}

__global__ __launch_bounds__(PW_THREADS) void act_fwd_flat_kernel(const float* __restrict__ x, float* __restrict__ y,
                                                                  long long n, int act) {
    const long long n4 = n >> 2;
    const bool vec = ((reinterpret_cast<uintptr_t>(x) | reinterpret_cast<uintptr_t>(y)) & 15) == 0;
    const long long stride = (long long)gridDim.x * blockDim.x, t = blockIdx.x * (long long)blockDim.x + threadIdx.x;
    long long done = 0;
    if (vec) {
        for (long long i = t; i < n4; i += stride) {
            f32x4 v = ld4(x + 4 * i);
#pragma unroll
            for (int e = 0; e < 4; ++e) v[e] = y4_act(v[e], act);
            st4(y + 4 * i, v);
        }
        done = n4 << 2;
    }
    for (long long i = done + t; i < n; i += stride) y[i] = y4_act(x[i], act);
}
__global__ __launch_bounds__(PW_THREADS) void act_bwd_flat_kernel(const float* __restrict__ x, const float* __restrict__ dy,
                                                                  float* __restrict__ dx, long long n, int act) {
    const long long n4 = n >> 2;
    const bool vec = ((reinterpret_cast<uintptr_t>(x) | reinterpret_cast<uintptr_t>(dy) | reinterpret_cast<uintptr_t>(dx)) & 15) == 0;
    const long long stride = (long long)gridDim.x * blockDim.x, t = blockIdx.x * (long long)blockDim.x + threadIdx.x;
    long long done = 0;
    if (vec) {
        for (long long i = t; i < n4; i += stride) {
            const f32x4 v = ld4(x + 4 * i), g = ld4(dy + 4 * i);
            f32x4 o;
#pragma unroll
            for (int e = 0; e < 4; ++e) o[e] = g[e] * y4_act_grad(v[e], act);
            st4(dx + 4 * i, o);
        }
        done = n4 << 2;
    }
    for (long long i = done + t; i < n; i += stride) dx[i] = dy[i] * y4_act_grad(x[i], act);
}

inline int grid_for(long long total, int cap = 256 * 16) {
    long long b = (total + PW_THREADS - 1) / PW_THREADS;
    if (b > cap) b = cap;
    if (b < 1) b = 1;
    return (int)b;
}
inline bool vec_ok(const void* p, long long ld, int C) {
    return p && (reinterpret_cast<uintptr_t>(p) & 15) == 0 && (ld & 3) == 0 && (C & 3) == 0 && ld >= C && C > 0;
}

}

extern "C" {

static long long bn_blocks(long long M, int C) {
    const RowMap rm = row_map(C);
    const long long rows_per_block = (long long)rm.rpb * stat_rows(M, rm.rpb);
    return (M + rows_per_block - 1) / rows_per_block;
}
size_t y4_bn_workspace(long long M, int C) {
    if (M <= 0 || C <= 0) return 0;
    return y4_bn_finalize_workspace(C) + (size_t)bn_blocks(M, C) * 2 * C * sizeof(float);
}
size_t y4_bn_finalize_workspace(int C) {
    return C > 0 ? (size_t)(1 + FOLD_BLOCKS) * 2 * C * sizeof(double) : 0;
}
static inline bool bn_loads_nt(long long M, int C) {
    static const char* e = getenv("Y4_BN_NT");
    if (e && *e) return atoi(e) != 0;
    (void)M;
    return C >= 64;
}
static int fold_partials(const float* part, long long nparts, int C, double* bacc, int* nb, hipStream_t st) {
    long long want = (nparts + 15) / 16;
    int blocks = (int)(want < FOLD_BLOCKS ? want : FOLD_BLOCKS);
    if (blocks < 1) blocks = 1;
    const long long per = (nparts + blocks - 1) / blocks;
    blocks = (int)((nparts + per - 1) / per);
    if (blocks < 1) blocks = 1;
    *nb = blocks;
    int cw = 32;
    while (cw < 2 * C && cw < PW_THREADS) cw *= 2;
    hipLaunchKernelGGL(fold_partials_kernel, dim3(blocks), dim3(PW_THREADS), 0, st, part, nparts, 2 * C, cw, bacc);
    Y4_CHECK_LAUNCH();
    return Y4_OK;
}

int y4_bn_stats_f32(const float* y, int ldy, long long M, int C, float* mean, float* invstd,
                    float* running_mean, float* running_var, long long* num_batches_tracked,
                    float momentum, float eps, void* workspace, size_t workspace_bytes, void* stream) {
    if (!y || !mean || !invstd || !workspace) return Y4_ERR_NULL;
    if (!vec_ok(y, ldy, C) || M <= 0) return Y4_ERR_SHAPE;
    if (workspace_bytes < y4_bn_workspace(M, C)) return Y4_ERR_WORKSPACE;
    hipStream_t st = y4_stream(stream);
    double* acc = static_cast<double*>(workspace);
    double* bacc = acc + 2 * C;
    float* part = reinterpret_cast<float*>(acc + (size_t)(1 + FOLD_BLOCKS) * 2 * C);
    const RowMap rm = row_map(C);
    const int nrows = stat_rows(M, rm.rpb);
    const long long blocks = bn_blocks(M, C);
    hipLaunchKernelGGL(bn_stats_kernel, dim3((unsigned)blocks), dim3(PW_THREADS), 0, st, y, (long long)ldy, M, C,
                       rm.tpr, rm.rpb, nrows, part);
    Y4_CHECK_LAUNCH();
    int nb = 0;
    { const int rc = fold_partials(part, blocks, C, bacc, &nb, st); if (rc != Y4_OK) return rc; }
    hipLaunchKernelGGL(bn_finalize_kernel, dim3((C + 31) / 32), dim3(256), 0, st, bacc, nb, M, C, eps, momentum, mean,
                       invstd, running_mean, running_var, num_batches_tracked);
    Y4_CHECK_LAUNCH();
    return Y4_OK;
}

int y4_bn_finalize_partials_f32(const float* partials, long long nparts, long long M, int C,
                                float* mean, float* invstd, float* running_mean, float* running_var,
                                long long* num_batches_tracked, float momentum, float eps,
                                void* workspace, size_t workspace_bytes, void* stream) {
    if (!partials || !mean || !invstd || !workspace) return Y4_ERR_NULL;
    if (nparts <= 0 || M <= 0 || C <= 0) return Y4_ERR_SHAPE;
    if (workspace_bytes < y4_bn_finalize_workspace(C)) return Y4_ERR_WORKSPACE;
    hipStream_t st = y4_stream(stream);
    double* bacc = static_cast<double*>(workspace) + 2 * C;
    int nb = 0;
    { const int rc = fold_partials(partials, nparts, C, bacc, &nb, st); if (rc != Y4_OK) return rc; }
    hipLaunchKernelGGL(bn_finalize_kernel, dim3((C + 31) / 32), dim3(256), 0, st, bacc, nb, M, C, eps, momentum, mean,
                       invstd, running_mean, running_var, num_batches_tracked);
    Y4_CHECK_LAUNCH();
    return Y4_OK;
}

int y4_bn_planes_bound_f32(const float* gamma, const float* beta, int C, long long M, const unsigned* floor_word, unsigned* out,
                           void* stream) {
    if (!gamma || !beta || !out) return Y4_ERR_NULL;
    if (C <= 0 || M <= 0) return Y4_ERR_SHAPE;
    hipLaunchKernelGGL(bn_planes_bound_kernel, dim3(1), dim3(256), 0, y4_stream(stream), gamma, beta, C,
                       sqrtf((float)(M > 1 ? M - 1 : 1)), nullptr, out, floor_word);
    Y4_CHECK_LAUNCH();
    return Y4_OK;
}

int y4_bn_act_fwd_f32(const float* y, int ldy, const float* mean, const float* invstd,
                      const float* gamma, const float* beta, int act,
                      const float* residual, int ldr, float* z, int ldz,
                      long long M, int C, unsigned* out_amax, int z_planes, const unsigned* res_amax, float* planes_twin,
                      void* stream) {
    if (!y || !mean || !invstd || !gamma || !beta) return Y4_ERR_NULL;
    const int ybf = (z_planes >> 4) & 1;
    z_planes &= 15;
    if (!z && (!out_amax || z_planes)) return Y4_ERR_NULL;
    if (z_planes < 0 || z_planes > 3) return Y4_ERR_SHAPE;
    if (planes_twin && (!z_planes || (reinterpret_cast<uintptr_t>(planes_twin) & 15))) return Y4_ERR_SHAPE;
    if (z_planes && ((!out_amax && z_planes != 3) || (C & 31))) return Y4_ERR_SHAPE;
    if (z_planes && !planes_twin && ldz != C && (ldz < C || (ldz & 31) || (reinterpret_cast<uintptr_t>(z) & 127))) return Y4_ERR_SHAPE;
    if (z_planes == 2) {
        if (residual && !res_amax) return Y4_ERR_NULL;
        hipLaunchKernelGGL(bn_planes_bound_kernel, dim3(1), dim3(256), 0, y4_stream(stream), gamma, beta, C,
                           sqrtf((float)(M > 1 ? M - 1 : 1)), residual ? res_amax : nullptr, out_amax);
        Y4_CHECK_LAUNCH();
    }
    if (!vec_ok(y, ldy, C) || (z && !vec_ok(z, ldz, C)) || (residual && !vec_ok(residual, ldr, C)) || M <= 0)
        return Y4_ERR_SHAPE;
    const RowMap rm = row_map(C);
    long long blocks = (M + rm.rpb * PW_UNROLL - 1) / (rm.rpb * PW_UNROLL);
    if (blocks > 256 * 16) blocks = 256 * 16;
    const bool nt = bn_loads_nt(M, C);
#define Y4_BN_FWD(RES_, YBF_)                                                                                                    \
    if (nt) Y4_BN_FWD_(RES_, YBF_, true); else Y4_BN_FWD_(RES_, YBF_, false)
#define Y4_BN_FWD_(RES_, YBF_, NT_)                                                                                              \
    hipLaunchKernelGGL((bn_act_fwd_kernel<A_, RES_, YBF_, NT_>), dim3((unsigned)blocks), dim3(PW_THREADS), 0, y4_stream(stream), y, \
                       (long long)ldy, mean, invstd, gamma, beta, residual, (long long)ldr, z, (long long)ldz, M, C, rm.tpr,      \
                       rm.rpb, z_planes == 3 ? nullptr : out_amax, z_planes == 3 ? 2 : (z_planes ? 1 : 0), planes_twin)
    if (residual) {
        if (ybf) { Y4_ACT_SWITCH(act, Y4_BN_FWD(true, true)); }
        else { Y4_ACT_SWITCH(act, Y4_BN_FWD(true, false)); }
    } else {
        if (ybf) { Y4_ACT_SWITCH(act, Y4_BN_FWD(false, true)); }
        else { Y4_ACT_SWITCH(act, Y4_BN_FWD(false, false)); }
    }
#undef Y4_BN_FWD
#undef Y4_BN_FWD_
    Y4_CHECK_LAUNCH();
    return Y4_OK;
}

static int bn_act_bwd_impl(const float* dz, int lddz, const float* y, int ldy,
                           const float* mean, const float* invstd, const float* gamma, const float* beta,
                           int act, float* dy, int lddy, float* dgamma, float* dbeta,
                           long long M, int C, void* workspace, size_t workspace_bytes, unsigned* out_amax,
                           unsigned* f16_planes, float* planes_twin, int flags, void* stream) {
    if (!dz || !y || !mean || !invstd || !gamma || !beta || !dy || !dgamma || !dbeta || !workspace) return Y4_ERR_NULL;
    const int frozen = flags & 1, bf = (flags >> 1) & 1, ybf = (flags >> 2) & 1;
    if (frozen && f16_planes) return Y4_ERR_SHAPE;
    if (bf && (f16_planes || (!planes_twin && lddy != C) || (C & 31))) return Y4_ERR_SHAPE;
    if (planes_twin && ((!f16_planes && !bf) || (reinterpret_cast<uintptr_t>(planes_twin) & 15))) return Y4_ERR_SHAPE;
    if (!vec_ok(dz, lddz, C) || !vec_ok(y, ldy, C) || !vec_ok(dy, lddy, C) || M <= 0) return Y4_ERR_SHAPE;
    if (workspace_bytes < y4_bn_workspace(M, C)) return Y4_ERR_WORKSPACE;
    hipStream_t st = y4_stream(stream);
    double* acc = static_cast<double*>(workspace);
    double* bacc = acc + 2 * C;
    float* part = reinterpret_cast<float*>(acc + (size_t)(1 + FOLD_BLOCKS) * 2 * C);
    const RowMap rm = row_map(C);
    const int nrows = stat_rows(M, rm.rpb);
    const long long rblocks = bn_blocks(M, C);
    int nb = 0;
    const bool nt = bn_loads_nt(M, C);
    {
#define Y4_BN_RED(BND_, YBF_)                                                                                                    \
        if (nt) Y4_BN_RED_(BND_, YBF_, true); else Y4_BN_RED_(BND_, YBF_, false)
#define Y4_BN_RED_(BND_, YBF_, NT_)                                                                                              \
        hipLaunchKernelGGL((bn_act_bwd_reduce_kernel<A_, BND_, YBF_, NT_>), dim3((unsigned)rblocks), dim3(PW_THREADS), 0, st, dz,  \
                           (long long)lddz, y, (long long)ldy, mean, invstd, gamma, beta, M, C, rm.tpr, rm.rpb, nrows, part,       \
                           f16_planes)
        if (f16_planes && ybf) return Y4_ERR_SHAPE;
        if (f16_planes) { Y4_ACT_SWITCH(act, Y4_BN_RED(true, false)); }
        else if (ybf) { Y4_ACT_SWITCH(act, Y4_BN_RED(false, true)); }
        else { Y4_ACT_SWITCH(act, Y4_BN_RED(false, false)); }
#undef Y4_BN_RED
#undef Y4_BN_RED_
        Y4_CHECK_LAUNCH();
        const int rc = fold_partials(part, rblocks, C, bacc, &nb, st);
        if (rc != Y4_OK) return rc;
    }
    if (f16_planes && ((!planes_twin && lddy != C) || (C & 31))) return Y4_ERR_SHAPE;
    hipLaunchKernelGGL(bn_bwd_finalize_kernel, dim3((C + 31) / 32), dim3(256), 0, st, bacc, nb, C, acc, dgamma, dbeta, gamma,
                       invstd, 1.0 / (double)M, f16_planes);
    Y4_CHECK_LAUNCH();
    long long blocks = (M + rm.rpb * PW_UNROLL - 1) / (rm.rpb * PW_UNROLL);
    if (blocks > 256 * 16) blocks = 256 * 16;
#define Y4_BN_APP(YBF_)                                                                                                          \
    if (nt) Y4_BN_APP_(YBF_, true); else Y4_BN_APP_(YBF_, false)
#define Y4_BN_APP_(YBF_, NT_)                                                                                                    \
    hipLaunchKernelGGL((bn_act_bwd_apply_kernel<A_, YBF_, NT_>), dim3((unsigned)blocks), dim3(PW_THREADS), 0, st, dz,              \
                       (long long)lddz,                                                                                          \
                       y, (long long)ldy, mean, invstd, gamma, beta, acc, dy, (long long)lddy, M, C, rm.tpr, rm.rpb, out_amax,    \
                       f16_planes, frozen ? 1 : 0, bf, planes_twin)
    if (ybf) { Y4_ACT_SWITCH(act, Y4_BN_APP(true)); }
    else { Y4_ACT_SWITCH(act, Y4_BN_APP(false)); }
#undef Y4_BN_APP
#undef Y4_BN_APP_
    Y4_CHECK_LAUNCH();
    return Y4_OK;
}

int y4_bn_act_bwd_f32(const float* dz, int lddz, const float* y, int ldy,
                      const float* mean, const float* invstd, const float* gamma, const float* beta,
                      int act, float* dy, int lddy, float* dgamma, float* dbeta,
                      long long M, int C, void* workspace, size_t workspace_bytes, unsigned* out_amax,
                      unsigned* f16_planes, float* planes_twin, int frozen_stats, void* stream) {
    return bn_act_bwd_impl(dz, lddz, y, ldy, mean, invstd, gamma, beta, act, dy, lddy, dgamma, dbeta, M, C, workspace,
                           workspace_bytes, out_amax, f16_planes, planes_twin, frozen_stats, stream);
}

static int colsum_rows(long long M) { return (int)(M < 1024 ? M : 1024); }

size_t y4_bias_grad_workspace(long long M, int C) {
    if (M <= 0 || C <= 0) return 0;
    return (size_t)colsum_rows(M) * (size_t)C * sizeof(float);
}

int y4_bias_grad_f32(const float* dy, int lddy, long long M, int C, float* dbias,
                     void* workspace, size_t workspace_bytes, void* stream) {
    if (!dy || !dbias || !workspace) return Y4_ERR_NULL;
    if (M <= 0 || C <= 0 || lddy < C) return Y4_ERR_SHAPE;
    if (workspace_bytes < y4_bias_grad_workspace(M, C)) return Y4_ERR_WORKSPACE;
    hipStream_t st = y4_stream(stream);
    float* part = static_cast<float*>(workspace);
    const int R = colsum_rows(M);
    hipLaunchKernelGGL(colsum_kernel, dim3((unsigned)R, (C + 255) / 256), dim3(256), 0, st, dy, (long long)lddy, M, C, part);
    Y4_CHECK_LAUNCH();
    hipLaunchKernelGGL(colsum_finalize_kernel, dim3((C + 7) / 8), dim3(256), 0, st, part, R, C, dbias);
    Y4_CHECK_LAUNCH();
    return Y4_OK;
}

int y4_bn_fold_f32(const float* gamma, const float* beta, const float* running_mean,
                   const float* running_var, float eps, float* scale, float* shift, int C, void* stream) {
    if (!gamma || !beta || !running_mean || !running_var || !scale || !shift) return Y4_ERR_NULL;
    if (C <= 0) return Y4_ERR_SHAPE;
    hipLaunchKernelGGL(bn_fold_kernel, dim3((C + 255) / 256), dim3(256), 0, y4_stream(stream), gamma, beta,
                       running_mean, running_var, eps, scale, shift, C);
    Y4_CHECK_LAUNCH();
    return Y4_OK;
}

int y4_copy_channels_f32(const float* src, int lds, float* dst, int ldd, long long M, int C, void* stream) {
    if (!vec_ok(src, lds, C) || !vec_ok(dst, ldd, C) || M <= 0) return Y4_ERR_SHAPE;
    hipLaunchKernelGGL(copy_rows_kernel, dim3(grid_for(M * (C / 4))), dim3(PW_THREADS), 0, y4_stream(stream),
                       src, (long long)lds, dst, (long long)ldd, M, C / 4);
    Y4_CHECK_LAUNCH();
    return Y4_OK;
}

int y4_add_f32(const float* a, int lda, const float* b, int ldb, float* out, int ldo,
               long long M, int C, void* stream) {
    if (!vec_ok(a, lda, C) || !vec_ok(b, ldb, C) || !vec_ok(out, ldo, C) || M <= 0) return Y4_ERR_SHAPE;
    hipLaunchKernelGGL(add_rows_kernel, dim3(grid_for(M * (C / 4))), dim3(PW_THREADS), 0, y4_stream(stream),
                       a, (long long)lda, b, (long long)ldb, out, (long long)ldo, M, C / 4);
    Y4_CHECK_LAUNCH();
    return Y4_OK;
}

int y4_maxpool_s1_fwd_f32(const float* x, int ldx, float* y, int ldy, signed char* idx,
                          int B, int H, int W, int C, int ksize, void* stream) {
    if (!vec_ok(x, ldx, C) || !vec_ok(y, ldy, C) || B <= 0 || H <= 0 || W <= 0) return Y4_ERR_SHAPE;
    if (ksize < 1 || (ksize & 1) == 0 || ksize > 11) return Y4_ERR_SHAPE;
    hipLaunchKernelGGL(maxpool_fwd_kernel, dim3(grid_for((long long)B * H * W * (C / 4))), dim3(PW_THREADS), 0,
                       y4_stream(stream), x, (long long)ldx, y, (long long)ldy, idx, B, H, W, C / 4, ksize);
    Y4_CHECK_LAUNCH();
    return Y4_OK;
}

int y4_maxpool_s1_bwd_f32(const float* dy, int lddy, const signed char* idx, float* dx, int lddx,
                          int accumulate, int B, int H, int W, int C, int ksize, void* stream) {
    if (!idx) return Y4_ERR_NULL;
    if (!vec_ok(dy, lddy, C) || !vec_ok(dx, lddx, C) || B <= 0 || H <= 0 || W <= 0) return Y4_ERR_SHAPE;
    if (ksize < 1 || (ksize & 1) == 0 || ksize > 11) return Y4_ERR_SHAPE;
    const int grid = grid_for((long long)B * H * W * (C / 4));
    if (accumulate)
        hipLaunchKernelGGL(maxpool_bwd_kernel<true>, dim3(grid), dim3(PW_THREADS), 0, y4_stream(stream), dy,
                           (long long)lddy, idx, dx, (long long)lddx, B, H, W, C / 4, ksize);
    else
        hipLaunchKernelGGL(maxpool_bwd_kernel<false>, dim3(grid), dim3(PW_THREADS), 0, y4_stream(stream), dy,
                           (long long)lddy, idx, dx, (long long)lddx, B, H, W, C / 4, ksize);
    Y4_CHECK_LAUNCH();
    return Y4_OK;
}

int y4_upsample2x_fwd_f32(const float* x, int ldx, float* y, int ldy, int B, int H, int W, int C, void* stream) {
    if (!vec_ok(x, ldx, C) || !vec_ok(y, ldy, C) || B <= 0 || H <= 0 || W <= 0) return Y4_ERR_SHAPE;
    hipLaunchKernelGGL(upsample2x_fwd_kernel, dim3(grid_for((long long)B * 4 * H * W * (C / 4))), dim3(PW_THREADS), 0,
                       y4_stream(stream), x, (long long)ldx, y, (long long)ldy, B, H, W, C / 4);
    Y4_CHECK_LAUNCH();
    return Y4_OK;
}

int y4_upsample2x_bwd_f32(const float* dy, int lddy, float* dx, int lddx, int B, int H, int W, int C, void* stream) {
    if (!vec_ok(dy, lddy, C) || !vec_ok(dx, lddx, C) || B <= 0 || H <= 0 || W <= 0) return Y4_ERR_SHAPE;
    hipLaunchKernelGGL(upsample2x_bwd_kernel, dim3(grid_for((long long)B * H * W * (C / 4))), dim3(PW_THREADS), 0,
                       y4_stream(stream), dy, (long long)lddy, dx, (long long)lddx, B, H, W, C / 4);
    Y4_CHECK_LAUNCH();
    return Y4_OK;
}

int y4_upsample_nearest_fwd_f32(const float* x, int ldx, float* y, int ldy, int B, int H, int W, int Ho, int Wo, int C,
                                int integer_factor, void* stream) {
    if (!vec_ok(x, ldx, C) || !vec_ok(y, ldy, C) || B <= 0 || H <= 0 || W <= 0 || Ho <= 0 || Wo <= 0) return Y4_ERR_SHAPE;
    int fh = 0, fw = 0;
    if (integer_factor) {
        if (Ho % H || Wo % W) return Y4_ERR_SHAPE;
        fh = Ho / H; fw = Wo / W;
    }
    hipLaunchKernelGGL(upsample_nearest_fwd_kernel, dim3(grid_for((long long)B * Ho * Wo * (C / 4))), dim3(PW_THREADS), 0,
                       y4_stream(stream), x, (long long)ldx, y, (long long)ldy, B, H, W, Ho, Wo, C / 4, fh, fw,
                       (float)H / (float)Ho, (float)W / (float)Wo);
    Y4_CHECK_LAUNCH();
    return Y4_OK;
}

int y4_upsample_nearest_bwd_f32(const float* dy, int lddy, float* dx, int lddx, int B, int H, int W, int Ho, int Wo, int C,
                                int integer_factor, void* stream) {
    if (!vec_ok(dy, lddy, C) || !vec_ok(dx, lddx, C) || B <= 0 || H <= 0 || W <= 0 || Ho <= 0 || Wo <= 0) return Y4_ERR_SHAPE;
    int fh = 0, fw = 0;
    if (integer_factor) {
        if (Ho % H || Wo % W) return Y4_ERR_SHAPE;
        fh = Ho / H; fw = Wo / W;
    }
    hipLaunchKernelGGL(upsample_nearest_bwd_kernel, dim3(grid_for((long long)B * H * W * (C / 4))), dim3(PW_THREADS), 0,
                       y4_stream(stream), dy, (long long)lddy, dx, (long long)lddx, B, H, W, Ho, Wo, C / 4, fh, fw,
                       (float)H / (float)Ho, (float)W / (float)Wo);
    Y4_CHECK_LAUNCH();
    return Y4_OK;
}

int y4_act_fwd_f32(const float* x, float* y, long long n, int act, void* stream) {
    if (!x || !y) return Y4_ERR_NULL;
    if (n <= 0 || act < 0 || act > 3) return Y4_ERR_SHAPE;
    hipLaunchKernelGGL(act_fwd_flat_kernel, dim3(grid_for((n + 3) / 4)), dim3(PW_THREADS), 0, y4_stream(stream), x, y, n, act);
    Y4_CHECK_LAUNCH();
    return Y4_OK;
}

int y4_act_bwd_f32(const float* x, const float* dy, float* dx, long long n, int act, void* stream) {
    if (!x || !dy || !dx) return Y4_ERR_NULL;
    if (n <= 0 || act < 0 || act > 3) return Y4_ERR_SHAPE;
    hipLaunchKernelGGL(act_bwd_flat_kernel, dim3(grid_for((n + 3) / 4)), dim3(PW_THREADS), 0, y4_stream(stream), x, dy, dx, n, act);
    Y4_CHECK_LAUNCH();
    return Y4_OK;
}

}
```

### yolov4_amd/ops.py

```python
import ctypes
import functools
import os

import torch

from ._lib import ACT_IDS, Y4Error, check, float_array, int_array, lib

CL = torch.channels_last


def _stream():
    return ctypes.c_void_p(torch.cuda.current_stream().cuda_stream)


def _ptr(t):
    return ctypes.c_void_p(t.data_ptr()) if t is not None else None


def _require_gpu(t, what):
    if not t.is_cuda:
        raise Y4Error(f'{what}: tensor is on {t.device}; the yolov4_amd hot path runs on an MI355X only '
                      '(no CPU fallback)')
    if t.dtype != torch.float32:
        raise Y4Error(f'{what}: expected float32, got {t.dtype}')


def nhwc_pitch(t):
    if t.dim() != 4:
        return None
    B, C, H, W = t.shape
    sb, sc, sh, sw = t.stride()
    if C > 1 and sc != 1:
        return None
    ld = sw if W > 1 else (sh if H > 1 else (sb if B > 1 else C))
    if ld < C:
        return None
    if W > 1 and sw != ld:
        return None
    if H > 1 and sh != W * ld:
        return None
    if B > 1 and sb != H * W * ld:
        return None
    return ld


def empty_nhwc(B, C, H, W, device, pad_to=1):
    Cp = (C + pad_to - 1) // pad_to * pad_to
    buf = torch.empty((B, Cp, H, W), device=device, dtype=torch.float32, memory_format=CL)
    return buf if Cp == C else buf[:, :C]


def as_nhwc(t, need_vec4=True, min_pitch=0):
    ld = nhwc_pitch(t)
    ok = ld is not None and (not need_vec4 or (ld % 4 == 0 and t.data_ptr() % 16 == 0)) and ld >= min_pitch
    if ok:
        return t, ld
    B, C, H, W = t.shape
    pad = 1
    if need_vec4:
        pad = 4
    if min_pitch > C:
        pad = max(pad, 32)
    out = empty_nhwc(B, C, H, W, t.device, pad_to=pad)
    out.copy_(t)
    return out, nhwc_pitch(out)


def krsc(w):
    if w.dim() != 4:
        raise Y4Error('conv weight must be 4-D')
    Co, Ci, kh, kw = w.shape
    exp = (kh * kw * Ci, 1, kw * Ci, Ci)
    st = w.stride()
    same = all(w.shape[i] == 1 or st[i] == exp[i] for i in range(4))
    return w if same else w.contiguous(memory_format=CL)


def _ws(nbytes, device):
    return torch.empty((max(int(nbytes), 16),), dtype=torch.uint8, device=device)


_AMAX = {'pool': {}, 'N': 8192}


def f16x2_mode():
    return lib().y4_get_conv_mode() == 3


def planes_mode():
    m = lib().y4_get_conv_mode()
    if m == 2 or (m == 3 and lib().y4_get_planes_bf16()):
        return 'bf16'
    return 'f16x2' if m == 3 else None


def new_amax(device, n=1):
    key = device.index if device.index is not None else torch.cuda.current_device()
    st = _AMAX['pool'].get(key)
    if st is None:
        st = {'buf': torch.zeros(_AMAX['N'], dtype=torch.int32, device=device), 'i': 0, 'gen': [0, 0]}
        _AMAX['pool'][key] = st
    half = _AMAX['N'] // 2
    i = (st['i'] + n - 1) // n * n
    if i >= _AMAX['N']:
        i = 0
    if i // half != (st['i'] - 1) // half or st['i'] == 0:
        h0 = i // half * half
        st['buf'][h0:h0 + half].zero_()
        st['gen'][i // half] += 1
    st['i'] = i + n
    cell = st['buf'][i:i + n]
    cell.y4_gen = (st, i // half, st['gen'][i // half])
    return cell


PLANES = {'on': os.environ.get('Y4_PLANES', '1') != '0'}
_PCELLS = {}


def planes_cell(device, n=8):
    key = device.index if device.index is not None else torch.cuda.current_device()
    st = _PCELLS.get(key)
    if st is None or st['i'] + n > st['buf'].numel():
        st = {'buf': torch.zeros(2048, dtype=torch.int32, device=device), 'i': 0}
        _PCELLS[key] = st
    cell = st['buf'][st['i']:st['i'] + n]
    st['i'] += n
    return cell


def live(cell):
    if cell is None:
        return None
    g = getattr(cell, 'y4_gen', None)
    if g is None:
        return cell
    st, half, gen = g
    return cell if st['gen'][half] == gen else None


def amax_of(t):
    return live(getattr(t, 'y4_amax', None)) if t is not None else None


def tag_amax(t, cell):
    if cell is not None and t is not None:
        t.y4_amax = cell
    return t


def amax_raw(t, valid_channels=None):
    B, C, H, W = t.shape
    t, ld = as_nhwc(t, need_vec4=False)
    cell = torch.empty(1, dtype=torch.int32, device=t.device)
    check(lib().y4_amax_f32(_ptr(t), ld, B * H * W, int(valid_channels or C), _ptr(cell), _stream()), 'amax')
    return cell


def amax_merge(dst, src):
    check(lib().y4_amax_merge_u32(_ptr(dst), _ptr(src), _stream()), 'amax_merge')


def conv_out_hw(H, W, k, s):
    p = (k - 1) // 2
    return (H + 2 * p - k) // s + 1, (W + 2 * p - k) // s + 1


def prepared_filter(param):
    w = krsc(param)
    L = lib()
    Cout, K = w.shape[0], w.shape[1] * w.shape[2] * w.shape[3]
    key = (w.data_ptr(), Cout, K, w.device)
    hit = getattr(param, '_y4_prepared', None)
    if hit is None or hit[0] != key:
        nbytes = L.y4_conv2d_prepared_bytes(Cout, K)
        buf = torch.empty(nbytes, dtype=torch.uint8, device=w.device)
        buf[:64].zero_()
        hit = (key, buf)
        param._y4_prepared = hit
    buf = hit[1]
    check(L.y4_conv2d_prepare_filter_f32(_ptr(w), Cout, K, _ptr(buf), buf.numel(), _stream()), 'conv2d_prepare_filter')
    return buf


def fast_conv_shape(Cin, k, s):
    return k in (1, 3) and s in (1, 2) and (Cin % 32 == 0 or (Cin == 3 and k == 3 and s == 1))


def planes_stride2_ok(k, s, H, W):
    return (s == 2 and k == 3 and H % 2 == 0 and W % 2 == 0 and _S2_PLANES
            and (planes_mode() == 'f16x2' or (planes_mode() == 'bf16' and f16x2_mode())))


@functools.lru_cache(maxsize=4096)
def _planes_fit(mode, B, H, W, ci, co, k, s, dgrad):
    return bool(lib().y4_conv_planes_fit(B, H, W, ci, co, k, s, 1 if dgrad else 0))


def planes_fit(B, H, W, ci, co, k, s, dgrad=True):
    return _planes_fit((lib().y4_get_conv_mode(), lib().y4_get_planes_bf16()), int(B), int(H), int(W), int(ci), int(co),
                       int(k), int(s), bool(dgrad))


def s2_plane_dgrad(B, H, W, ci, co):
    floor = 64 if planes_mode() == 'bf16' else 128
    return _S2_DGRAD_PLANES and ci >= floor and planes_fit(B, H, W, ci, co, 3, 2, dgrad=True)


_S2_PLANES = os.environ.get('Y4_PLANES_S2', '1') != '0'
_S2_DGRAD_PLANES = os.environ.get('Y4_PLANES_S2_DGRAD', '1') != '0'
_BF16_Y = os.environ.get('Y4_BF16_Y', '1') != '0'


def conv_fwd_raw(x, w, k, s, scale=None, shift=None, act='linear', residual=None, out=None, out_pad=1, x_amax=None,
                 out_amax=None, w_prepared=None):
    L = lib()
    B, Cin, H, W = x.shape
    Cout = w.shape[0]
    Ho, Wo = conv_out_hw(H, W, k, s)
    if out is None:
        out = empty_nhwc(B, Cout, Ho, Wo, x.device, pad_to=out_pad)
    ldy = nhwc_pitch(out)
    w = krsc(w)
    if not fast_conv_shape(Cin, k, s) or (Cin == 3 and (Cout > 32 or residual is not None)):
        if k % 2 == 0:
            raise Y4Error('even kernel sizes are not supported (pad = (k - 1) // 2 would not keep the map size)')
        x, ldx = as_nhwc(x, need_vec4=False)
        ldr = 0
        if residual is not None:
            residual, ldr = as_nhwc(residual, need_vec4=False)
        check(L.y4_conv2d_generic_fwd_f32(_ptr(x), ldx, _ptr(w), _ptr(out), ldy, B, H, W, Cin, Cout, k, s, _ptr(scale), _ptr(shift),
                                          ACT_IDS[act], _ptr(residual), ldr, _stream()), 'conv2d_generic_fwd')
        return out
    if Cin == 3:
        if k != 3 or s != 1 or residual is not None:
            raise Y4Error('Cin=3 is supported for the 3x3/s1 stem only')
        sb, sc, sh, sw = x.stride()
        check(L.y4_conv2d_stem_fwd_f32(_ptr(x), sb, sc, sh, sw, _ptr(w), _ptr(out), ldy, B, H, W, Cout,
                                       _ptr(scale), _ptr(shift), ACT_IDS[act], None, _stream()), 'conv2d_stem_fwd')
        return out
    x, ldx = as_nhwc(x)
    ldr = 0
    if residual is not None:
        residual, ldr = as_nhwc(residual, need_vec4=False)
    if w_prepared is not None:
        check(L.y4_conv2d_fwd_prepared_f32(_ptr(x), ldx, _ptr(w_prepared), _ptr(out), ldy, B, H, W, Cin, Cout, k, s,
                                           _ptr(scale), _ptr(shift), ACT_IDS[act], _ptr(residual), ldr, _ptr(x_amax),
                                           _ptr(out_amax), _stream()), 'conv2d_fwd_prepared')
        return out
    nbytes = L.y4_conv2d_fwd_workspace(Cin, Cout, k)
    ws = _ws(nbytes, x.device)
    check(L.y4_conv2d_fwd_f32(_ptr(x), ldx, _ptr(w), _ptr(out), ldy, B, H, W, Cin, Cout, k, s,
                              _ptr(scale), _ptr(shift), ACT_IDS[act], _ptr(residual), ldr, _ptr(x_amax), _ptr(out_amax),
                              _ptr(ws), nbytes, _stream()), 'conv2d_fwd')
    return out


def dgrad_filter_buffer(Cin, Cout, k, device):
    return _ws(lib().y4_conv2d_dgrad_workspace(Cin, Cout, k), device)


def conv_fwd_bnstats_raw(x, w, k, s, running_mean, running_var, nbt, momentum, eps, x_amax=None, dgrad_filter=None):
    L = lib()
    B, Cin, H, W = x.shape
    Cout = w.shape[0]
    Ho, Wo = conv_out_hw(H, W, k, s)
    if not fast_conv_shape(Cin, k, s) or (Cin == 3 and Cout > 32) or Cout % 4:
        if Cout % 4:
            raise Y4Error('BatchNorm over a channel count that is not a multiple of 4 is not supported')
        y = conv_fwd_raw(x, w, k, s, out=empty_nhwc(B, Cout, Ho, Wo, x.device, pad_to=4), x_amax=x_amax)
        mean, invstd = bn_stats_raw(y, running_mean, running_var, nbt, momentum, eps)
        return y, mean, invstd
    y = empty_nhwc(B, Cout, Ho, Wo, x.device)
    ldy = nhwc_pitch(y)
    w = krsc(w)
    pbytes = L.y4_conv2d_bnstats_workspace(B, H, W, Cin, Cout, k, s)
    part = _ws(pbytes, x.device)
    if Cin == 3:
        if k != 3 or s != 1:
            raise Y4Error('Cin=3 is supported for the 3x3/s1 stem only')
        sb, sc, sh, sw = x.stride()
        check(L.y4_conv2d_stem_fwd_f32(_ptr(x), sb, sc, sh, sw, _ptr(w), _ptr(y), ldy, B, H, W, Cout,
                                       None, None, ACT_IDS['linear'], _ptr(part), _stream()), 'conv2d_stem_fwd')
        nparts = (B * H * W + 255) // 256
    else:
        x, ldx = as_nhwc(x)
        n = ctypes.c_longlong(0)
        nbytes = L.y4_conv2d_fwd_workspace(Cin, Cout, k)
        cws = _ws(nbytes, x.device)
        check(L.y4_conv2d_fwd_bnstats_f32(_ptr(x), ldx, _ptr(w), _ptr(y), ldy, B, H, W, Cin, Cout, k, s,
                                          _ptr(part), pbytes, ctypes.byref(n), _ptr(x_amax), _ptr(cws), nbytes,
                                          _ptr(dgrad_filter), dgrad_filter.numel() if dgrad_filter is not None else 0, _stream()),
              'conv2d_fwd_bnstats')
        nparts = n.value
    mean = torch.empty(Cout, device=x.device, dtype=torch.float32)
    invstd = torch.empty(Cout, device=x.device, dtype=torch.float32)
    wsb = L.y4_bn_finalize_workspace(Cout)
    ws = _ws(wsb, x.device)
    check(L.y4_bn_finalize_partials_f32(_ptr(part), nparts, B * Ho * Wo, Cout, _ptr(mean), _ptr(invstd),
                                        _ptr(running_mean), _ptr(running_var), _ptr(nbt), float(momentum), float(eps),
                                        _ptr(ws), wsb, _stream()), 'bn_finalize_partials')
    return y, mean, invstd


class Planes:
    __slots__ = ('buf', 'shape', 'amax')

    def __init__(self, buf, shape, amax):
        self.buf, self.shape, self.amax = buf, tuple(shape), amax


class PlanesTensor(torch.Tensor):
    __torch_function__ = torch._C._disabled_torch_function_impl

    def _refuse(self, *a, **kw):
        raise Y4Error('this tensor holds a PRE-SPLIT activation (two fp16 pieces per element, csrc/conv_planes.hip), not '
                      'float32 values: only ConvBNAct can consume it.  Register the forward hook before the forward pass '
                      '(hooked modules return fp32), or run with Y4_PLANES=0 to keep every intermediate tensor fp32.')

    cpu = to = numpy = tolist = item = float = double = half = bfloat16 = int = long = clone = _refuse
    sum = mean = abs = max = min = amax = amin = norm = std = var = exp = log = sigmoid = tanh = relu = _refuse
    __add__ = __radd__ = __sub__ = __rsub__ = __mul__ = __rmul__ = __truediv__ = __rtruediv__ = __neg__ = __pow__ = _refuse
    __iadd__ = __isub__ = __imul__ = __itruediv__ = __matmul__ = __getitem__ = __setitem__ = _refuse
    __lt__ = __le__ = __gt__ = __ge__ = __float__ = __int__ = __bool__ = __array__ = __dlpack__ = _refuse
    __reduce_ex__ = __reduce__ = __deepcopy__ = _refuse

    def __repr__(self, *a, **kw):
        return (f'PlanesTensor(shape={tuple(self.shape)}, device={self.device}: pre-split fp16 pairs, NOT float32 values; '
                'see yolov4_amd.ops.PlanesTensor)')

    __str__ = __repr__

    def __format__(self, spec):
        return self.__repr__()

    def detach(self):
        return as_planes(torch.Tensor.detach(self), getattr(self, 'y4_amax', None))


def as_planes(t, cell=None):
    if type(t) is not PlanesTensor:
        t = t.as_subclass(PlanesTensor)
    t.y4_planes = True
    if cell is not None:
        t.y4_amax = cell
    return t


def planes_split_raw(x, amax=None):
    L = lib()
    B, C, H, W = x.shape
    x, ldx = as_nhwc(x)
    if planes_mode() == 'bf16':
        amax = None
    else:
        if amax is None:
            amax = amax_of(x)
        if amax is None:
            amax = amax_raw(x)
    buf = torch.empty((B, H, W, C * 4), dtype=torch.uint8, device=x.device)
    check(L.y4_planes_split_f32(_ptr(x), ldx, B * H * W, C, _ptr(amax), _ptr(buf), _stream()), 'planes_split')
    return Planes(buf, (B, C, H, W), amax)


def conv_fwd_planes_raw(xp, w, k, s, stats=True, dgrad_filter=None, y_bf16=False, bias=None, out=None):
    L = lib()
    B, Cin, H, W = xp.shape
    Cout = w.shape[0]
    Ho, Wo = conv_out_hw(H, W, k, s)
    y = out if _slot_ok(out, (B, Cout, Ho, Wo)) else empty_nhwc(B, Cout, Ho, Wo, xp.buf.device)
    w = krsc(w)
    nbytes = L.y4_conv2d_fwd_workspace(Cin, Cout, k)
    ws = _ws(nbytes, xp.buf.device)
    pbytes = ((B * Ho * Wo + 127) // 128) * 2 * Cout * 4 if stats else 0
    part = _ws(pbytes, xp.buf.device) if stats else None
    n = ctypes.c_longlong(0)
    check(L.y4_conv2d_fwd_planes_f32(_ptr(xp.buf), _ptr(w), _ptr(y), nhwc_pitch(y), B, H, W, Cin, Cout, k, s,
                                     _ptr(part), pbytes, ctypes.byref(n), _ptr(xp.amax), _ptr(ws), nbytes,
                                     _ptr(dgrad_filter), dgrad_filter.numel() if dgrad_filter is not None else 0,
                                     1 if y_bf16 else 0, _ptr(bias), _stream()),
          'conv2d_fwd_planes')
    return (y, part, n.value) if stats else y


def conv_fwd_planes_bnstats_raw(xp, w, k, s, running_mean, running_var, nbt, momentum, eps, dgrad_filter=None, y_bf16=False):
    L = lib()
    y, part, nparts = conv_fwd_planes_raw(xp, w, k, s, dgrad_filter=dgrad_filter, y_bf16=y_bf16)
    Cout = w.shape[0]
    M = y.shape[0] * y.shape[2] * y.shape[3]
    mean = torch.empty(Cout, device=y.device, dtype=torch.float32)
    invstd = torch.empty(Cout, device=y.device, dtype=torch.float32)
    wsb = L.y4_bn_finalize_workspace(Cout)
    ws = _ws(wsb, y.device)
    check(L.y4_bn_finalize_partials_f32(_ptr(part), nparts, M, Cout, _ptr(mean), _ptr(invstd),
                                        _ptr(running_mean), _ptr(running_var), _ptr(nbt), float(momentum), float(eps),
                                        _ptr(ws), wsb, _stream()), 'bn_finalize_partials')
    return y, mean, invstd


def planes_of(t):
    if t is None or not getattr(t, 'y4_planes', False):
        return None
    return Planes(t, t.shape, getattr(t, 'y4_amax', None))


def conv_dgrad_planes_raw(dyp, w, x_shape, k, residual=None, prepared=None, s=1):
    L = lib()
    B, Cin, H, W = x_shape
    Cout = w.shape[0]
    dx = empty_nhwc(B, Cin, H, W, dyp.buf.device)
    nbytes = L.y4_conv2d_dgrad_workspace(Cin, Cout, k)
    ws = prepared if prepared is not None else _ws(nbytes, dyp.buf.device)
    ldr = 0
    if residual is not None:
        residual, ldr = as_nhwc(residual)
    check(L.y4_conv2d_dgrad_planes_f32(_ptr(dyp.buf), None if prepared is not None else _ptr(krsc(w)), _ptr(dx), nhwc_pitch(dx), B, H, W, Cin, Cout, k,
                                       s, _ptr(ws), nbytes, _ptr(dyp.amax), _ptr(residual), ldr, _stream()), 'conv2d_dgrad_planes')
    return dx


def conv_wgrad_planes_raw(xp, dyp, w_shape, k, out=None, s=1):
    L = lib()
    B, Cin, H, W = xp.shape
    Cout = w_shape[0]
    if out is not None and tuple(out.shape) == tuple(w_shape) and _is_krsc_dense(out) and out.data_ptr() % 16 == 0:
        dw = out
        WGRAD_STATS['in_place'] += 1
    else:
        WGRAD_STATS['temporary'] += 1
        dw = krsc(torch.empty(w_shape, device=xp.buf.device, dtype=torch.float32).contiguous(memory_format=CL))
    nbytes = L.y4_conv2d_wgrad_planes_workspace(B, H, W, Cin, Cout, k, s)
    ws = _ws(nbytes, xp.buf.device)
    check(L.y4_conv2d_wgrad_planes_f32(_ptr(xp.buf), _ptr(dyp.buf), _ptr(dw), B, H, W, Cin, Cout, k, s, _ptr(ws), nbytes,
                                       _ptr(xp.amax), _ptr(dyp.amax), _stream()), 'conv2d_wgrad_planes')
    return dw


def conv_stem_dgrad_raw(dy, w, x):
    L = lib()
    B, _, H, W = x.shape
    dy, lddy = as_nhwc(dy, need_vec4=False)
    dx = torch.empty_like(x, memory_format=torch.preserve_format)
    sb, sc, sh, sw = dx.stride()
    check(L.y4_conv2d_stem_dgrad_f32(_ptr(dy), lddy, _ptr(krsc(w)), _ptr(dx), sb, sc, sh, sw, B, H, W, w.shape[0], _stream()),
          'conv2d_stem_dgrad')
    return dx


def last_conv_kernel():
    import ctypes
    buf = ctypes.create_string_buffer(160)
    check(lib().y4_last_conv_kernel(buf, 160), 'last_conv_kernel')
    return buf.value.decode()


def conv_dgrad_raw(dy, w, x_shape, k, s, dy_amax=None, residual=None, prepared=None):
    L = lib()
    B, Cin, H, W = x_shape
    Cout = w.shape[0]
    if k not in (1, 3) or s not in (1, 2):
        dy, lddy = as_nhwc(dy, need_vec4=False)
        dx = empty_nhwc(B, Cin, H, W, dy.device)
        ldr = 0
        if residual is not None:
            residual, ldr = as_nhwc(residual, need_vec4=False)
        check(L.y4_conv2d_generic_dgrad_f32(_ptr(dy), lddy, _ptr(krsc(w)), _ptr(dx), nhwc_pitch(dx), B, H, W, Cin, Cout, k, s,
                                            _ptr(residual), ldr, _stream()), 'conv2d_generic_dgrad')
        return dx
    cpad = (Cout + 31) // 32 * 32
    dy, lddy = as_nhwc(dy, min_pitch=cpad)
    dx = empty_nhwc(B, Cin, H, W, dy.device)
    nbytes = L.y4_conv2d_dgrad_workspace(Cin, Cout, k)
    ws = prepared if prepared is not None else _ws(nbytes, dy.device)
    ldr = 0
    if residual is not None:
        residual, ldr = as_nhwc(residual, need_vec4=False)
    check(L.y4_conv2d_dgrad_f32(_ptr(dy), lddy, None if prepared is not None else _ptr(krsc(w)), _ptr(dx), nhwc_pitch(dx), B, H, W, Cin, Cout, k, s,
                                _ptr(ws), nbytes, _ptr(dy_amax), _ptr(residual), ldr, _stream()),
          'conv2d_dgrad')
    return dx


def _is_krsc_dense(t):
    Co, Ci, kh, kw = t.shape
    exp = (kh * kw * Ci, 1, kw * Ci, Ci)
    st = t.stride()
    return t.dtype == torch.float32 and all(t.shape[i] == 1 or st[i] == exp[i] for i in range(4))


WGRAD_STATS = {'in_place': 0, 'temporary': 0}



def conv_wgrad_raw(x, dy, w_shape, k, s, out=None, x_amax=None, dy_amax=None):
    L = lib()
    B, Cin, H, W = x.shape
    Cout = w_shape[0]
    if out is not None and tuple(out.shape) == tuple(w_shape) and _is_krsc_dense(out) and out.data_ptr() % 16 == 0:
        dw = out
        WGRAD_STATS['in_place'] += 1
    else:
        WGRAD_STATS['temporary'] += 1
        dw = torch.empty(w_shape, device=dy.device, dtype=torch.float32).contiguous(memory_format=CL)
        dw = krsc(dw)
    if k not in (1, 3) or s not in (1, 2) or (Cin % 4 and Cin != 3) or (Cin == 3 and (k != 3 or s != 1 or Cout > 32)):
        xs, ldx = as_nhwc(x, need_vec4=False)
        dys, lddy = as_nhwc(dy, need_vec4=False)
        check(L.y4_conv2d_generic_wgrad_f32(_ptr(xs), ldx, _ptr(dys), lddy, _ptr(dw), B, H, W, Cin, Cout, k, s, _stream()),
              'conv2d_generic_wgrad')
        return dw
    if Cin == 3:
        dy, lddy = as_nhwc(dy, need_vec4=False)
        nbytes = L.y4_conv2d_stem_wgrad_workspace(B, H, W, Cout)
        ws = _ws(nbytes, dy.device)
        sb, sc, sh, sw = x.stride()
        check(L.y4_conv2d_stem_wgrad_f32(_ptr(x), sb, sc, sh, sw, _ptr(dy), lddy, _ptr(dw), B, H, W, Cout,
                                         _ptr(ws), nbytes, _stream()), 'conv2d_stem_wgrad')
        return dw
    x, ldx = as_nhwc(x)
    dy, lddy = as_nhwc(dy, min_pitch=(Cout + 3) // 4 * 4)
    nbytes = L.y4_conv2d_wgrad_workspace(B, H, W, Cin, Cout, k, s)
    ws = _ws(nbytes, dy.device)
    check(L.y4_conv2d_wgrad_f32(_ptr(x), ldx, _ptr(dy), lddy, _ptr(dw), B, H, W, Cin, Cout, k, s,
                                _ptr(ws), nbytes, _ptr(x_amax), _ptr(dy_amax), _stream()), 'conv2d_wgrad')
    return dw


def bn_stats_raw(y, running_mean, running_var, nbt, momentum, eps):
    L = lib()
    B, C, H, W = y.shape
    y, ld = as_nhwc(y)
    mean = torch.empty(C, device=y.device, dtype=torch.float32)
    invstd = torch.empty(C, device=y.device, dtype=torch.float32)
    nbytes = L.y4_bn_workspace(B * H * W, C)
    ws = _ws(nbytes, y.device)
    check(L.y4_bn_stats_f32(_ptr(y), ld, B * H * W, C, _ptr(mean), _ptr(invstd), _ptr(running_mean),
                            _ptr(running_var), _ptr(nbt), float(momentum), float(eps), _ptr(ws), nbytes, _stream()),
          'bn_stats')
    return mean, invstd


def _slot_ok(out, shape):
    if out is None:
        return False
    ld = nhwc_pitch(out)
    return (tuple(out.shape) == tuple(shape) and out.dtype == torch.float32 and ld is not None and ld % 4 == 0
            and out.data_ptr() % 16 == 0)


def bn_act_fwd_raw(y, mean, invstd, gamma, beta, act, residual=None, out=None, out_amax=None, planes=False, y_bf16=False, cell=None):
    L = lib()
    B, C, H, W = y.shape
    y, ldy = as_nhwc(y)
    ldr = 0
    if residual is not None:
        residual, ldr = as_nhwc(residual)
    yb = 16 if y_bf16 else 0
    if planes == 'slot':
        cb = out.y4_cat
        if residual is not None or not _slot_ok(out, (B, C, H, W)):
            raise Y4Error('a pre-split concat slot takes a BatchNorm result of its own shape, without a skip operand')
        bf = planes_mode() == 'bf16'
        zp = out.data_ptr()
        if bf:
            zp = cb.buf.data_ptr() + (zp - cb.buf.data_ptr()) // 2
        check(L.y4_bn_act_fwd_f32(_ptr(y), ldy, _ptr(mean), _ptr(invstd), _ptr(gamma), _ptr(beta), ACT_IDS[act], None, 0,
                                  ctypes.c_void_p(zp), nhwc_pitch(out), B * H * W, C, None if bf else _ptr(cb.cell[0:1]),
                                  (3 if bf else 1) + yb, None, None, _stream()), 'bn_act_fwd(planes slot)')
        return out
    if planes:
        both = planes == 'both'
        zp = empty_nhwc(B, C, H, W, y.device)
        z = (out if _slot_ok(out, (B, C, H, W)) else empty_nhwc(B, C, H, W, y.device)) if both else zp
        args = (_ptr(y), ldy, _ptr(mean), _ptr(invstd), _ptr(gamma), _ptr(beta), ACT_IDS[act], _ptr(residual), ldr)
        if planes_mode() == 'bf16':
            check(L.y4_bn_act_fwd_f32(*args, _ptr(z), nhwc_pitch(z), B * H * W, C, None, 3 + yb, None,
                                      _ptr(zp) if both else None, _stream()), 'bn_act_fwd(bf16)')
            zp = as_planes(zp)
            if both:
                z.y4_twin = zp
                return z
            return zp
        given = cell is not None
        if given and (residual is not None or both):
            raise Y4Error('a given plane scale goes with a plain planes-only result')
        cell = cell if given else planes_cell(y.device)
        res_cell = amax_of(residual) if residual is not None else None
        if given:
            mode = 1
        elif residual is not None and res_cell is None:
            check(L.y4_bn_act_fwd_f32(*args, None, C, B * H * W, C, _ptr(cell), yb, None, None, _stream()), 'bn_act_fwd(measure)')
            mode = 1
        else:
            mode = 2
        check(L.y4_bn_act_fwd_f32(*args, _ptr(z), nhwc_pitch(z), B * H * W, C, _ptr(cell), mode + yb, _ptr(res_cell),
                                  _ptr(zp) if both else None, _stream()), 'bn_act_fwd(planes)')
        zp = as_planes(zp, cell)
        if both:
            z.y4_twin = zp
            return tag_amax(z, cell[0:1])
        return as_planes(zp, cell[0:1])
    z = out if _slot_ok(out, (B, C, H, W)) else empty_nhwc(B, C, H, W, y.device)
    check(L.y4_bn_act_fwd_f32(_ptr(y), ldy, _ptr(mean), _ptr(invstd), _ptr(gamma), _ptr(beta), ACT_IDS[act],
                              _ptr(residual), ldr, _ptr(z), nhwc_pitch(z), B * H * W, C, _ptr(out_amax), yb, None, None, _stream()),
          'bn_act_fwd')
    return z


def bn_act_bwd_raw(dz, y, mean, invstd, gamma, beta, act, dgamma_out=None, dbeta_out=None, out_amax=None, planes=None,
                   frozen=False, bf16=False, twin=False, y_bf16=False):
    L = lib()
    B, C, H, W = y.shape
    dz, lddz = as_nhwc(dz)
    y, ldy = as_nhwc(y)
    dy = empty_nhwc(B, C, H, W, y.device)

    def slot(t):
        ok = t is not None and t.dtype == torch.float32 and tuple(t.shape) == (C,) and t.is_contiguous() and t.is_cuda
        return t if ok else torch.empty(C, device=y.device, dtype=torch.float32)
    dgamma, dbeta = slot(dgamma_out), slot(dbeta_out)
    dyp = empty_nhwc(B, C, H, W, y.device) if twin else None
    nbytes = L.y4_bn_workspace(B * H * W, C)
    ws = _ws(nbytes, y.device)
    check(L.y4_bn_act_bwd_f32(_ptr(dz), lddz, _ptr(y), ldy, _ptr(mean), _ptr(invstd), _ptr(gamma), _ptr(beta),
                              ACT_IDS[act], _ptr(dy), nhwc_pitch(dy), _ptr(dgamma), _ptr(dbeta), B * H * W, C,
                              _ptr(ws), nbytes, _ptr(out_amax), _ptr(planes), _ptr(dyp) if twin else None,
                              (1 if frozen else 0) | (2 if bf16 else 0) | (4 if y_bf16 else 0), _stream()),
          'bn_act_bwd')
    if twin:
        return dy, dgamma, dbeta, dyp
    return dy, dgamma, dbeta


def bias_grad_raw(dy):
    L = lib()
    B, C, H, W = dy.shape
    dy, ld = as_nhwc(dy, need_vec4=False)
    db = torch.empty(C, device=dy.device, dtype=torch.float32)
    nbytes = L.y4_bias_grad_workspace(B * H * W, C)
    ws = _ws(nbytes, dy.device)
    check(L.y4_bias_grad_f32(_ptr(dy), ld, B * H * W, C, _ptr(db), _ptr(ws), nbytes, _stream()), 'bias_grad')
    return db


def bn_fold_raw(gamma, beta, rm, rv, eps):
    L = lib()
    C = gamma.numel()
    scale = torch.empty(C, device=gamma.device, dtype=torch.float32)
    shift = torch.empty(C, device=gamma.device, dtype=torch.float32)
    check(L.y4_bn_fold_f32(_ptr(gamma), _ptr(beta), _ptr(rm), _ptr(rv), float(eps), _ptr(scale), _ptr(shift), C,
                           _stream()), 'bn_fold')
    return scale, shift


def add_raw(a, b):
    L = lib()
    B, C, H, W = a.shape
    a, lda = as_nhwc(a)
    b, ldb = as_nhwc(b)
    out = empty_nhwc(B, C, H, W, a.device)
    check(L.y4_add_f32(_ptr(a), lda, _ptr(b), ldb, _ptr(out), nhwc_pitch(out), B * H * W, C, _stream()), 'add')
    return out


def copy_into_raw(src, dst):
    L = lib()
    B, C, H, W = src.shape
    src, lds = as_nhwc(src)
    ldd = nhwc_pitch(dst)
    if ldd is None:
        raise Y4Error('copy_into: destination is not NHWC')
    check(L.y4_copy_channels_f32(_ptr(src), lds, _ptr(dst), ldd, B * H * W, C, _stream()), 'copy_channels')


_ASYNC = {'on': os.environ.get('Y4_ASYNC_WGRAD', '0') == '1', 'streams': {}, 'join_queued': False}


def set_async_wgrad(on):
    _ASYNC['on'] = bool(on)


def side_stream(device):
    key = device.index if device.index is not None else torch.cuda.current_device()
    st = _ASYNC['streams'].get(key)
    if st is None:
        st = torch.cuda.Stream(device=device)
        _ASYNC['streams'][key] = st
    return st


def join_side_stream(device=None):
    for st in _ASYNC['streams'].values():
        torch.cuda.current_stream(st.device).wait_stream(st)
    _ASYNC['join_queued'] = False


def _wgrad_to_param(x, dy, param, k, s, x_amax=None, dy_amax=None, fn=None):
    main = torch.cuda.current_stream(x.device)
    side = side_stream(x.device)
    ev = main.record_event()
    with torch.cuda.stream(side):
        side.wait_event(ev)
        dw = fn() if fn is not None else conv_wgrad_raw(x, dy, tuple(param.shape), k, s, x_amax=x_amax, dy_amax=dy_amax)
        if param.grad is None:
            dw.record_stream(main)
            param.grad = dw
        else:
            param.grad.record_stream(side)
            param.grad.add_(dw)
        ready = getattr(param, '_y4_grad_ready', None)
        if ready is not None:
            ready()
    x.record_stream(side)
    dy.record_stream(side)
    for cell in (x_amax, dy_amax):
        if cell is not None:
            cell.record_stream(side)
    if not _ASYNC['join_queued']:
        _ASYNC['join_queued'] = True
        torch.autograd.Variable._execution_engine.queue_callback(join_side_stream)


def _pad_out_channels(weight, bias, cop):
    co = weight.shape[0]
    if cop == co:
        return weight, bias
    wp = torch.zeros((cop,) + tuple(weight.shape[1:]), dtype=weight.dtype, device=weight.device).contiguous(memory_format=torch.channels_last)
    wp[:co].copy_(weight)
    bp = None
    if bias is not None:
        bp = torch.zeros(cop, dtype=bias.dtype, device=bias.device)
        bp[:co].copy_(bias)
    return wp, bp


def _split_padded(t, cop, amax=None):
    B, C, H, W = t.shape
    t, ld = as_nhwc(t)
    if ld < cop:
        v = empty_nhwc(B, cop, H, W, t.device)
        v[:, :C].copy_(t)
        t, ld = v, nhwc_pitch(v)
    buf = torch.empty((B, H, W, cop * 4), dtype=torch.uint8, device=t.device)
    check(lib().y4_planes_split_into_f32(_ptr(t), ld, B * H * W, cop, _ptr(amax), _ptr(buf), cop, C, _stream()), 'planes_split(padded)')
    return Planes(buf, (B, cop, H, W), amax)


class ConvBNActFn(torch.autograd.Function):

    @staticmethod
    def forward(ctx, x, weight, bias, gamma, beta, residual, cfg):
        k, s, act, training, bn = cfg['k'], cfg['s'], cfg['act'], cfg['training'], cfg['bn']
        _require_gpu(x, 'ConvBNAct input')
        _require_gpu(weight, 'ConvBNAct weight')
        dest = cfg.pop('out', None)
        ctx.cfg = {key: cfg.get(key) for key in ('k', 's', 'act', 'gamma_param', 'beta_param', 'weight_param',
                                                 'dres_put', 'dres_take', 'dx_put')}
        ctx.x_shape = tuple(x.shape)
        ctx.has_res = residual is not None
        f16 = f16x2_mode() and x.shape[1] != 3
        bfm = planes_mode() == 'bf16'
        xp = planes_of(x)
        if xp is None and cfg.get('x_twin') is not None:
            xp = planes_of(cfg['x_twin'])
        ctx.x_planes = xp is not None
        nobn_planes = xp is not None and not bn and act == 'linear' and residual is None and s == 1 and cfg.get('grad', True)
        if xp is not None and not ((f16 or bfm) and x.shape[1] % 32 == 0 and (nobn_planes or (
                bn and training and weight.shape[0] % 32 == 0 and (s == 1 or planes_stride2_ok(k, s, x.shape[2], x.shape[3]))))):
            raise Y4Error('a pre-split (planes) tensor reached a conv that cannot consume it')
        x_amax = live(cfg.get('x_amax')) if f16 else None
        z_amax = None
        io = cfg.get('io')
        if xp is not None:
            x_amax = xp.amax
        elif f16 and x_amax is None and (ctx.needs_input_grad[0] or ctx.needs_input_grad[1]):
            x_amax = amax_raw(x)
        ctx.x_amax = x_amax
        if bn and training:
            if x.shape[0] * conv_out_hw(x.shape[2], x.shape[3], k, s)[0] * conv_out_hw(x.shape[2], x.shape[3], k, s)[1] <= 1:
                raise ValueError('Expected more than 1 value per channel when training')
            ctx.dgrad_filter = None
            if ((f16 or (bfm and xp is not None)) and ctx.needs_input_grad[0] and x.shape[1] % 32 == 0 and fast_conv_shape(x.shape[1], k, s)
                    and weight.shape[0] % 4 == 0 and (xp is None or weight.shape[0] % 32 == 0)
                    and not (bfm and xp is not None and s == 2
                             and not s2_plane_dgrad(x.shape[0], x.shape[2], x.shape[3], x.shape[1], weight.shape[0]))):
                ctx.dgrad_filter = dgrad_filter_buffer(x.shape[1], weight.shape[0], k, x.device)
            ybf = ctx.y_bf16 = bool(bfm and xp is not None and weight.shape[0] % 32 == 0 and _BF16_Y)
            if xp is not None:
                y, mean, invstd = conv_fwd_planes_bnstats_raw(xp, weight, k, s, cfg['running_mean'], cfg['running_var'],
                                                              cfg['nbt'], cfg['momentum'], cfg['eps'], dgrad_filter=ctx.dgrad_filter,
                                                              y_bf16=ybf)
            else:
                y, mean, invstd = conv_fwd_bnstats_raw(x, weight, k, s, cfg['running_mean'], cfg['running_var'],
                                                       cfg['nbt'], cfg['momentum'], cfg['eps'], x_amax=x_amax,
                                                       dgrad_filter=ctx.dgrad_filter)
            want = cfg.get('out_planes')
            cb = cfg.get('out_cat')
            if cb is not None and cb.planes:
                z = bn_act_fwd_raw(y, mean, invstd, gamma, beta, act, residual, out=dest, planes='slot', y_bf16=ybf)
                if io is not None:
                    io['z_planes'] = True
                z_amax = cb.cell[0:1] if cb.cell is not None else None
            elif want and (f16 or bfm) and y.shape[1] % 32 == 0 and (want == 'both' or dest is None):
                sf = cfg.get('scale_from')
                z = bn_act_fwd_raw(y, mean, invstd, gamma, beta, act, residual, out=dest if want == 'both' else None,
                                   planes='both' if want == 'both' else True, y_bf16=ybf,
                                   cell=sf.cell if (sf is not None and sf.planes and sf.cell is not None and want is True) else None)
                z_amax = getattr(z, 'y4_amax', None)
                if io is not None:
                    io['z_planes'] = want != 'both'
                    io['z_twin'] = getattr(z, 'y4_twin', None)
            else:
                if f16x2_mode():
                    z_amax = live(cfg.get('out_amax')) if (dest is not None and _slot_ok(dest, tuple(y.shape))) else None
                    if z_amax is None:
                        z_amax = new_amax(x.device)
                z = bn_act_fwd_raw(y, mean, invstd, gamma, beta, act, residual, out=dest, out_amax=z_amax, y_bf16=ybf)
            ctx.save_for_backward(xp.buf if xp is not None else x, weight, y, mean, invstd, gamma, beta)
            ctx.mode = 'bn_train'
        elif bn and cfg.get('grad', True) and any(ctx.needs_input_grad[i] for i in (0, 1, 3, 4)):
            y = conv_fwd_raw(x, weight, k, s, x_amax=x_amax, out=empty_nhwc(x.shape[0], weight.shape[0],
                                                                              *conv_out_hw(x.shape[2], x.shape[3], k, s), x.device, pad_to=4))
            invstd, _ = bn_fold_raw(torch.ones_like(gamma), beta, cfg['running_mean'], cfg['running_var'], cfg['eps'])
            mean = cfg['running_mean']
            if f16x2_mode():
                z_amax = live(cfg.get('out_amax')) if (dest is not None and _slot_ok(dest, tuple(y.shape))) else None
                if z_amax is None:
                    z_amax = new_amax(x.device)
            z = bn_act_fwd_raw(y, mean, invstd, gamma, beta, act, residual, out=dest, out_amax=z_amax)
            ctx.save_for_backward(x, weight, y, mean.detach().clone(), invstd, gamma, beta)
            ctx.mode = 'bn_eval_grad'
        elif bn:
            frozen = not cfg.get('grad', True) and os.environ.get('Y4_NO_INFER_CACHE') != '1'
            fast = f16 and fast_conv_shape(x.shape[1], k, s)
            wprep = prepared_filter(cfg['weight_param']) if (frozen and fast and cfg.get('weight_param') is not None) else None
            scale, shift = bn_fold_raw(gamma, beta, cfg['running_mean'], cfg['running_var'], cfg['eps'])
            o = dest
            Ho, Wo = conv_out_hw(x.shape[2], x.shape[3], k, s)
            o = o if _slot_ok(o, (x.shape[0], weight.shape[0], Ho, Wo)) else None
            if fast:
                z_amax = live(cfg.get('out_amax')) if o is not None else None
                if z_amax is None:
                    z_amax = new_amax(x.device)
            z = conv_fwd_raw(x, weight, k, s, scale, shift, act, residual, out=o, x_amax=x_amax, out_amax=z_amax,
                             w_prepared=wprep)
            ctx.mode = 'bn_eval'
        elif nobn_planes:
            co = weight.shape[0]
            q = 64 if bfm else 32
            cop = (co + q - 1) // q * q
            wpad, bpad = _pad_out_channels(weight, bias, cop)
            Ho, Wo = conv_out_hw(x.shape[2], x.shape[3], k, s)
            zf = empty_nhwc(x.shape[0], cop, Ho, Wo, x.device)
            ctx.dgrad_filter = dgrad_filter_buffer(x.shape[1], cop, k, x.device) if ctx.needs_input_grad[0] else None
            conv_fwd_planes_raw(xp, wpad, k, s, stats=False, dgrad_filter=ctx.dgrad_filter, bias=bpad, out=zf)
            z = zf[:, :co]
            ctx.save_for_backward(xp.buf, weight)
            ctx.mode = 'nobn_linear'
        else:
            wprep = prepared_filter(cfg['weight_param']) if (not cfg.get('grad', True) and f16 and fast_conv_shape(x.shape[1], k, s)
                                                              and os.environ.get('Y4_NO_INFER_CACHE') != '1'
                                                              and cfg.get('weight_param') is not None) else None
            z = conv_fwd_raw(x, weight, k, s, None, bias, act, residual, out_pad=32, x_amax=x_amax, w_prepared=wprep)
            if act != 'linear':
                ctx.mode = 'nobn_act'
            else:
                ctx.save_for_backward(x, weight)
                ctx.mode = 'nobn_linear'
        if io is not None:
            io['z_amax'] = z_amax
        return z

    @staticmethod
    def backward(ctx, dz):
        cfg = ctx.cfg
        k, s, act = cfg['k'], cfg['s'], cfg['act']
        f16 = f16x2_mode() and ctx.x_shape[1] != 3
        dy_amax = dy_pl = dyP = wq = None
        x_amax = live(ctx.x_amax)
        x_planes = getattr(ctx, 'x_planes', False)
        if ctx.mode in ('bn_train', 'bn_eval_grad'):
            x, weight, y, mean, invstd, gamma, beta = ctx.saved_tensors
            gp, bp = cfg.get('gamma_param'), cfg.get('beta_param')
            sink = (gp is not None and bp is not None and getattr(gp, '_y4_grad_fresh', False)
                    and getattr(bp, '_y4_grad_fresh', False) and gp.grad is not None and bp.grad is not None
                    and ctx.needs_input_grad[3] and ctx.needs_input_grad[4])
            bfp = x_planes and planes_mode() == 'bf16'
            planes = planes_cell(dz.device, 8) if (x_planes and not bfp) else None
            dy_amax = planes[5:6] if planes is not None else (new_amax(dz.device) if f16 else None)
            twin_dy = x_planes and s == 2 and ctx.needs_input_grad[0] and not s2_plane_dgrad(
                ctx.x_shape[0], ctx.x_shape[2], ctx.x_shape[3], ctx.x_shape[1], dz.shape[1])
            res = bn_act_bwd_raw(dz, y, mean, invstd, gamma, beta, act,
                                 gp.grad if sink else None, bp.grad if sink else None,
                                 out_amax=None if planes is not None else dy_amax, planes=planes,
                                 frozen=ctx.mode == 'bn_eval_grad', bf16=bfp, twin=twin_dy, y_bf16=getattr(ctx, 'y_bf16', False))
            dy, dgamma, dbeta = res[:3]
            dy_pl = res[3] if twin_dy else dy
            if sink and dgamma is gp.grad and dbeta is bp.grad:
                gp._y4_grad_fresh = bp._y4_grad_fresh = False
                gp._y4_grad_ready()
                bp._y4_grad_ready()
                dgamma = dbeta = None
            dbias = None
        elif ctx.mode == 'nobn_linear':
            x, weight = ctx.saved_tensors
            dy = dz
            dgamma = dbeta = None
            dbias = bias_grad_raw(dz) if ctx.needs_input_grad[2] else None
            if x_planes:
                bfp = planes_mode() == 'bf16'
                q = 64 if bfp else 32
                cop = (weight.shape[0] + q - 1) // q * q
                dyP = _split_padded(dz, cop, None if bfp else amax_raw(dz))
                wq = _pad_out_channels(weight, None, cop)[0]
            elif f16:
                dy_amax = amax_raw(dy)
        else:
            raise Y4Error(f'backward through ConvBNAct in mode {ctx.mode} is not implemented')
        dx = None
        take = cfg.get('dres_take')
        skip_grad = take.pop('dres', None) if take is not None else None
        if take is not None and skip_grad is None:
            take['taker_done'] = True
        if ctx.needs_input_grad[0]:
            if ctx.x_shape[1] == 3 and k == 3 and s == 1 and weight.shape[0] <= 32 and skip_grad is None:
                dx = conv_stem_dgrad_raw(dy, weight, x)
            elif x_planes and dyP is not None:
                dx = conv_dgrad_planes_raw(dyP, wq, ctx.x_shape, k, residual=skip_grad, prepared=getattr(ctx, 'dgrad_filter', None))
            elif x_planes and (s == 1 or not twin_dy):
                dx = conv_dgrad_planes_raw(Planes(dy, dy.shape, dy_amax), weight, ctx.x_shape, k, residual=skip_grad,
                                           prepared=getattr(ctx, 'dgrad_filter', None), s=s)
            else:
                dx = conv_dgrad_raw(dy, weight, ctx.x_shape, k, s, dy_amax=dy_amax, residual=skip_grad,
                                    prepared=getattr(ctx, 'dgrad_filter', None) if f16x2_mode() else None)
            ctx.dgrad_filter = None
        elif skip_grad is not None:
            raise Y4Error('a parked skip gradient has no consumer (input of the 1x1 conv does not require grad)')
        fbox = cfg.get('dx_put')
        if fbox is not None and dx is not None and not fbox.get('taker_done'):
            fbox['dres'] = dx
            dx = None
        dw = None
        if ctx.needs_input_grad[1]:
            param = cfg.get('weight_param')

            def wgrad(out=None):
                if x_planes and dyP is not None:
                    return conv_wgrad_planes_raw(Planes(x, ctx.x_shape, ctx.x_amax), dyP, tuple(weight.shape), k, out=out)
                if x_planes:
                    return conv_wgrad_planes_raw(Planes(x, ctx.x_shape, ctx.x_amax), Planes(dy_pl, dy.shape, dy_amax),
                                                 tuple(weight.shape), k, out=out, s=s)
                return conv_wgrad_raw(x, dy, tuple(weight.shape), k, s, out=out, x_amax=x_amax, dy_amax=dy_amax)
            if _ASYNC['on'] and param is not None and param.requires_grad:
                _wgrad_to_param(x, (dyP.buf if dyP is not None else dy_pl) if x_planes else dy, param, k, s,
                                ctx.x_amax if x_planes else x_amax, dyP.amax if dyP is not None else dy_amax,
                                fn=wgrad if x_planes else None)
            elif param is not None and getattr(param, '_y4_grad_fresh', False) and param.grad is not None:
                param._y4_grad_fresh = False
                got = wgrad(out=param.grad)
                if got is not param.grad:
                    param.grad.add_(got)
                param._y4_grad_ready()
            else:
                dw = wgrad()
        dres = dz if ctx.has_res else None
        put = cfg.get('dres_put')
        if dres is not None and put is not None:
            put['dres'] = dres
            dres = None
        return dx, dw, dbias, dgamma, dbeta, dres, None


class Fork2Fn(torch.autograd.Function):

    @staticmethod
    def forward(ctx, x):
        ctx.set_materialize_grads(False)
        return x.view_as(x), x.view_as(x)

    @staticmethod
    def backward(ctx, g1, g2):
        if g1 is None:
            return g2
        if g2 is None:
            return g1
        return add_raw(g1, g2)


def fork(x):
    if not (torch.is_grad_enabled() and x.requires_grad):
        return x, x
    a, b = Fork2Fn.apply(x)
    cell = amax_of(x)
    twin = getattr(x, 'y4_twin', None)
    if twin is not None:
        a.y4_twin = b.y4_twin = twin
    if getattr(x, 'y4_planes', False):
        cell = getattr(x, 'y4_amax', None)
        return as_planes(a, cell), as_planes(b, cell)
    return tag_amax(a, cell), tag_amax(b, cell)


class AddFn(torch.autograd.Function):

    @staticmethod
    def forward(ctx, a, b):
        _require_gpu(a, 'add input')
        _require_gpu(b, 'add input')
        return add_raw(a, b)

    @staticmethod
    def backward(ctx, g):
        return g, g


class CatBuffer:

    def __init__(self, B, sizes, H, W, device, planes_norms=None):
        self.sizes = list(sizes)
        self.buf = empty_nhwc(B, sum(self.sizes), H, W, device)
        self.offsets = [sum(self.sizes[:i]) for i in range(len(self.sizes))]
        self.amax = new_amax(device) if (device.type == 'cuda' and f16x2_mode()) else None
        self.planes = False
        pm = planes_mode()
        q = 64 if pm == 'bf16' else 32
        if planes_norms is not None and pm is not None and device.type == 'cuda' and all(c % q == 0 for c in self.sizes):
            self.planes = True
            self.cell = None
            if pm == 'f16x2':
                self.cell = planes_cell(device)
                for i, n in enumerate(planes_norms):
                    if isinstance(n, torch.Tensor) and not isinstance(n, torch.nn.Module):
                        c = live(amax_of(n))
                        amax_merge(self.cell[0:1], c if c is not None else amax_raw(n))
                        continue
                    n, M = n if isinstance(n, tuple) else (n, B * H * W)
                    check(lib().y4_bn_planes_bound_f32(_ptr(n.weight), _ptr(n.bias), self.sizes[i], M,
                                                       _ptr(self.cell[0:1]) if i else None, _ptr(self.cell[0:1]), _stream()),
                          'bn_planes_bound')
                self.amax = self.cell[0:1]

    def slot(self, i):
        t = tag_amax(self.buf[:, self.offsets[i]:self.offsets[i] + self.sizes[i]], self.amax)
        if self.planes:
            t.y4_cat = self
        return t


def _split_into_slot(t, dst, cb):
    B, C, H, W = t.shape
    t, ldt = as_nhwc(t)
    zp = dst.data_ptr()
    if planes_mode() == 'bf16':
        zp = cb.buf.data_ptr() + (zp - cb.buf.data_ptr()) // 2
    check(lib().y4_planes_split_into_f32(_ptr(t), ldt, B * H * W, C, _ptr(cb.cell[0:1]) if cb.cell is not None else None,
                                         ctypes.c_void_p(zp), nhwc_pitch(dst), 0, _stream()), 'planes_split_into')


class CatFn(torch.autograd.Function):

    @staticmethod
    def forward(ctx, into, *xs):
        B, _, H, W = xs[0].shape
        ctx.sizes = [t.shape[1] for t in xs]
        if into is not None and (into.sizes != ctx.sizes or tuple(into.buf.shape) != (B, sum(ctx.sizes), H, W)):
            into = None
        out = into.buf if into is not None else empty_nhwc(B, sum(ctx.sizes), H, W, xs[0].device)
        o = 0
        for t in xs:
            _require_gpu(t, 'cat input')
            dst = out[:, o:o + t.shape[1]]
            if not (t.data_ptr() == dst.data_ptr() and t.stride() == dst.stride()):
                if into is not None and into.planes:
                    if getattr(t, 'y4_planes', False):
                        raise Y4Error('a pre-split concat buffer takes pre-split inputs only where their producers wrote them in place')
                    _split_into_slot(t, dst, into)
                else:
                    copy_into_raw(t, dst)
            elif into is not None and into.planes != bool(getattr(t, 'y4_planes', False)):
                raise Y4Error('concat buffer and input disagree on the pre-split form')
            o += t.shape[1]
        return out

    @staticmethod
    def backward(ctx, g):
        outs, o = [None], 0
        for c in ctx.sizes:
            outs.append(g[:, o:o + c])
            o += c
        return tuple(outs)


def cat(xs, into=None):
    out = CatFn.apply(into, *xs)
    if into is not None and into.planes and out.data_ptr() == into.buf.data_ptr():
        return as_planes(out, into.cell[0:1] if into.cell is not None else None)
    if into is not None and into.amax is not None and out.data_ptr() == into.buf.data_ptr():
        for t in xs:
            cell = amax_of(t)
            if cell is None:
                cell = amax_raw(t)
            if cell.data_ptr() != into.amax.data_ptr():
                amax_merge(into.amax, cell)
        tag_amax(out, into.amax)
    return out


def cat_buffer(like, sizes, hw=None, planes_norms=None):
    H, W = hw if hw is not None else (like.shape[2], like.shape[3])
    return CatBuffer(like.shape[0], sizes, H, W, like.device, planes_norms=planes_norms)


class SppPoolCatFn(torch.autograd.Function):

    @staticmethod
    def forward(ctx, x, cell=None):
        L = lib()
        _require_gpu(x, 'SPP input')
        B, C, H, W = x.shape
        x, ldx = as_nhwc(x)
        out = empty_nhwc(B, 4 * C, H, W, x.device)
        ldo = nhwc_pitch(out)
        need_idx = ctx.needs_input_grad[0]
        idx5 = torch.empty((B, H, W, C), dtype=torch.int8, device=x.device) if need_idx else None
        idx9 = torch.empty((B, H, W, C), dtype=torch.int8, device=x.device) if need_idx else None
        st = _stream()
        check(L.y4_maxpool_s1_fwd_f32(_ptr(x), ldx, _ptr(out[:, 0:C]), ldo, _ptr(idx5), B, H, W, C, 5, st), 'maxpool5')
        check(L.y4_maxpool_s1_fwd_f32(_ptr(x), ldx, _ptr(out[:, C:2 * C]), ldo, _ptr(idx9), B, H, W, C, 9, st), 'maxpool9')
        copy_into_raw(out[:, 0:C], out[:, 2 * C:3 * C])
        copy_into_raw(x, out[:, 3 * C:4 * C])
        ctx.idx = (idx5, idx9)
        ctx.shape = (B, C, H, W)
        if cell is not None:
            pl = empty_nhwc(B, 4 * C, H, W, x.device)
            check(L.y4_planes_split_f32(_ptr(out), ldo, B * H * W, 4 * C, _ptr(cell.t), _ptr(pl), st), 'planes_split(spp)')
            return pl
        return out

    @staticmethod
    def backward(ctx, g):
        L = lib()
        B, C, H, W = ctx.shape
        idx5, idx9 = ctx.idx
        g, ldg = as_nhwc(g)
        dx = empty_nhwc(B, C, H, W, g.device)
        ldx = nhwc_pitch(dx)
        st = _stream()
        copy_into_raw(g[:, 3 * C:4 * C], dx)
        for sl, idx, ks in ((g[:, 0:C], idx5, 5), (g[:, C:2 * C], idx9, 9), (g[:, 2 * C:3 * C], idx5, 5)):
            check(L.y4_maxpool_s1_bwd_f32(_ptr(sl), ldg, _ptr(idx), _ptr(dx), ldx, 1, B, H, W, C, ks, st), 'maxpool_bwd')
        return dx, None


def spp_pool_cat(x, planes=False):
    pm = planes_mode()
    if planes and pm is not None and x.is_cuda and (4 * x.shape[1]) % (64 if pm == 'bf16' else 32) == 0:
        cell = None
        if pm == 'f16x2':
            cell = planes_cell(x.device)
            src = live(amax_of(x))
            amax_merge(cell[0:1], src if src is not None else amax_raw(x))
        out = SppPoolCatFn.apply(x, Slot(cell[0:1]) if cell is not None else Slot(None))
        return as_planes(out, cell[0:1] if cell is not None else None)
    return tag_amax(SppPoolCatFn.apply(x), amax_of(x))


class MaxPoolS1Fn(torch.autograd.Function):

    @staticmethod
    def forward(ctx, x, ksize):
        L = lib()
        _require_gpu(x, 'maxpool input')
        B, C, H, W = x.shape
        x, ldx = as_nhwc(x)
        out = empty_nhwc(B, C, H, W, x.device)
        idx = torch.empty((B, H, W, C), dtype=torch.int8, device=x.device)
        check(L.y4_maxpool_s1_fwd_f32(_ptr(x), ldx, _ptr(out), nhwc_pitch(out), _ptr(idx), B, H, W, C, ksize,
                                      _stream()), 'maxpool')
        ctx.idx, ctx.ks, ctx.shape = idx, ksize, (B, C, H, W)
        return out

    @staticmethod
    def backward(ctx, g):
# ... 239 lines not shown
```

Before: 452.4.

## Recompute stem conv in fused BN forward and backward instead of storing pre-BN output

For the 3-channel stem conv with training BN, the forward now runs a stats-only conv pass, finalizes BN, then recomputes the conv fused with BN+activation to write only the activated output. The backward recomputes the conv from the input again, fusing activation/BN backward with weight-gradient and dgamma/dbeta reduction, so the pre-BN tensor is never stored or reread. This trades extra cheap MFMA recompute of a K=27 conv for removing large full-resolution memory traffic at 608x608. It adds new kernels and a backward fold/finalize path that is gated by an environment flag, on by default.

```diff
diff --git a/include/yolov4_amd.h b/include/yolov4_amd.h
--- a/include/yolov4_amd.h
+++ b/include/yolov4_amd.h
@@ -95,6 +95,18 @@
                            const float* w, float* y, int ldy, int B, int H, int W, int Cout,
                            const float* scale, const float* shift, int act,
                            float* bnstats_partials, void* stream);
+
+int y4_conv2d_stem_bn_stats_f32(const float* x, long long sxb, long long sxc, long long sxh, long long sxw,
+                                const float* w, int B, int H, int W, int Cout, float* bnstats_partials, void* stream);
+int y4_conv2d_stem_bn_act_fwd_f32(const float* x, long long sxb, long long sxc, long long sxh, long long sxw,
+                                  const float* w, const float* mean, const float* invstd, const float* gamma, const float* beta,
+                                  int act, float* z, int ldz, int B, int H, int W, int Cout, unsigned* out_amax, void* stream);
+size_t y4_conv2d_stem_bn_act_bwd_workspace(int B, int H, int W, int Cout);
+int y4_conv2d_stem_bn_act_bwd_f32(const float* x, long long sxb, long long sxc, long long sxh, long long sxw,
+                                  const float* w, const float* dz, int lddz,
+                                  const float* mean, const float* invstd, const float* gamma, const float* beta, int act,
+                                  float* dw, float* dgamma, float* dbeta, int B, int H, int W, int Cout,
+                                  void* workspace, size_t workspace_bytes, void* stream);
 
 size_t y4_conv2d_dgrad_workspace(int Cin, int Cout, int k);
 int y4_conv2d_dgrad_f32(const float* dy, int lddy, const float* w , float* dx, int lddx,
diff --git a/yolov4_amd/_lib.py b/yolov4_amd/_lib.py
--- a/yolov4_amd/_lib.py
+++ b/yolov4_amd/_lib.py
@@ -51,6 +51,10 @@
     'y4_conv2d_wgrad_f32': (I, [P, I, P, I, P, I, I, I, I, I, I, I, P, Z, P, P, P]),
     'y4_conv2d_stem_wgrad_workspace': (Z, [I, I, I, I]),
     'y4_conv2d_stem_wgrad_f32': (I, [P, L, L, L, L, P, I, P, I, I, I, I, P, Z, P]),
+    'y4_conv2d_stem_bn_stats_f32': (I, [P, L, L, L, L, P, I, I, I, I, P, P]),
+    'y4_conv2d_stem_bn_act_fwd_f32': (I, [P, L, L, L, L, P, P, P, P, P, I, P, I, I, I, I, I, P, P]),
+    'y4_conv2d_stem_bn_act_bwd_workspace': (Z, [I, I, I, I]),
+    'y4_conv2d_stem_bn_act_bwd_f32': (I, [P, L, L, L, L, P, P, I, P, P, P, P, I, P, P, P, I, I, I, I, P, Z, P]),
     'y4_bn_workspace': (Z, [L, I]),
     'y4_bn_finalize_workspace': (Z, [I]),
     'y4_bn_finalize_partials_f32': (I, [P, L, L, I, P, P, P, P, P, F, F, P, Z, P]),
diff --git a/yolov4_amd/csrc/conv_geom.h b/yolov4_amd/csrc/conv_geom.h
--- a/yolov4_amd/csrc/conv_geom.h
+++ b/yolov4_amd/csrc/conv_geom.h
@@ -51,6 +51,8 @@
 int amax_launch(const float* x, long long ld, long long M, int C, unsigned* amax_bits, hipStream_t st,
                 bool prezeroed = false);
 int amax_merge(unsigned* dst, const unsigned* src, hipStream_t st);
+int bn_bwd_fold_finalize(const float* part, long long nparts, int C, void* head, float* dgamma, float* dbeta,
+                         const float* gamma, const float* invstd, long long M, hipStream_t st);
 
 
 bool tile_conv_ok(int Cs, int Cs_valid, int N, int k, int stride, int H, int W);
diff --git a/yolov4_amd/csrc/conv_igemm.hip b/yolov4_amd/csrc/conv_igemm.hip
--- a/yolov4_amd/csrc/conv_igemm.hip
+++ b/yolov4_amd/csrc/conv_igemm.hip
@@ -1399,114 +1399,337 @@
     }
 }
 
+struct StemTileOps {
+    bf16x8 fb[2][3];
+    int koff[16];
+    int ktap[16];
+};
+
+__device__ __forceinline__ void stem_tile_setup(StemTileOps& t, const StemGeom& g, const int fr, const int fh) {
+#pragma unroll
+    for (int i = 0; i < 16; ++i) {
+        const int k = (i >> 3) * 16 + fh * 8 + (i & 7);
+        const int r = k / 9, c = (k - r * 9) / 3, q = k - r * 9 - c * 3;
+        const bool kv = k < 27;
+        t.koff[i] = kv ? (int)(c * g.sxc + (r - 1) * g.sxh + (q - 1) * g.sxw) * 4 : 0;
+        t.ktap[i] = kv ? r * 3 + q : 9;
+    }
+#pragma unroll
+    for (int ks = 0; ks < 2; ++ks) {
+        f32x4 w0, w1;
+#pragma unroll
+        for (int i = 0; i < 8; ++i) {
+            const int k = ks * 16 + fh * 8 + i;
+            const int r = k / 9, c = (k - r * 9) / 3, q = k - r * 9 - c * 3;
+            const float v = (k < 27 && fr < g.Cout) ? g.w[fr * 27 + (r * 3 + q) * 3 + c] : 0.f;
+            if (i < 4) w0[i] = v; else w1[i - 4] = v;
+        }
+        u32x2 a1, a2, a3, b1, b2, b3;
+        split3x4(w0, a1, a2, a3);
+        split3x4(w1, b1, b2, b3);
+        const u32x4 q1 = {a1[0], a1[1], b1[0], b1[1]}, q2 = {a2[0], a2[1], b2[0], b2[1]}, q3 = {a3[0], a3[1], b3[0], b3[1]};
+        t.fb[ks][0] = __builtin_bit_cast(bf16x8, q1); t.fb[ks][1] = __builtin_bit_cast(bf16x8, q2); t.fb[ks][2] = __builtin_bit_cast(bf16x8, q3);
+    }
+}
+
+__device__ __forceinline__ void stem_pixel(const StemGeom& g, const int HW, const float inv_hw, const float inv_w, const long long p,
+                                           int& b, int& h, int& w) {
+    b = (int)((float)p * inv_hw);
+    int rem = (int)(p - (long long)b * HW);
+    if (rem < 0) { --b; rem += HW; } else if (rem >= HW) { ++b; rem -= HW; }
+    h = (int)((float)rem * inv_w);
+    w = rem - h * g.W;
+    if (w < 0) { --h; w += g.W; } else if (w >= g.W) { ++h; w -= g.W; }
+}
+
+__device__ __forceinline__ void stem_tile_load(const StemTileOps& t, const StemGeom& g, const __amdgpu_buffer_rsrc_t rsrc, const int HW,
+                                               const float inv_hw, const float inv_w, const int fr, float (&xv)[16],
+                                               const long long tile) {
+    const long long p = tile * 32 + fr;
+    unsigned base = 0xffffffffu;
+    unsigned m9 = 0;
+    if (p < g.M) {
+        int b, h, w;
+        stem_pixel(g, HW, inv_hw, inv_w, p, b, h, w);
+        base = (unsigned)(b * g.sxb + h * g.sxh + w * g.sxw) * 4u;
+        const unsigned hm = (h > 0 ? 1u : 0u) | 2u | (h + 1 < g.H ? 4u : 0u);
+        const unsigned wm = (w > 0 ? 1u : 0u) | 2u | (w + 1 < g.W ? 4u : 0u);
+        m9 = ((hm & 1u) ? wm : 0u) | ((hm & 2u) ? wm << 3 : 0u) | ((hm & 4u) ? wm << 6 : 0u);
+    }
+#pragma unroll
+    for (int i = 0; i < 16; ++i) {
+        const bool ok = (m9 >> t.ktap[i]) & 1u;
+        xv[i] = __builtin_bit_cast(float, __builtin_amdgcn_raw_buffer_load_b32(rsrc, ok ? (int)(base + (unsigned)t.koff[i]) : -1, 0, 0));
+    }
+}
+
+__device__ __forceinline__ f32x16 stem_tile_mma(const StemTileOps& t, const float (&xv)[16]) {
+    f32x16 acc;
+#pragma unroll
+    for (int e = 0; e < 16; ++e) acc[e] = 0.f;
+#pragma unroll
+    for (int ks = 0; ks < 2; ++ks) {
+        const f32x4 v0 = {xv[ks * 8 + 0], xv[ks * 8 + 1], xv[ks * 8 + 2], xv[ks * 8 + 3]};
+        const f32x4 v1 = {xv[ks * 8 + 4], xv[ks * 8 + 5], xv[ks * 8 + 6], xv[ks * 8 + 7]};
+        u32x2 a1, a2, a3, b1, b2, b3;
+        split3x4(v0, a1, a2, a3);
+        split3x4(v1, b1, b2, b3);
+        const u32x4 q1 = {a1[0], a1[1], b1[0], b1[1]}, q2 = {a2[0], a2[1], b2[0], b2[1]}, q3 = {a3[0], a3[1], b3[0], b3[1]};
+        const bf16x8 f1 = __builtin_bit_cast(bf16x8, q1), f2 = __builtin_bit_cast(bf16x8, q2), f3 = __builtin_bit_cast(bf16x8, q3);
+        acc = __builtin_amdgcn_mfma_f32_32x32x16_bf16(f3, t.fb[ks][0], acc, 0, 0, 0);
+        acc = __builtin_amdgcn_mfma_f32_32x32x16_bf16(f2, t.fb[ks][1], acc, 0, 0, 0);
+        acc = __builtin_amdgcn_mfma_f32_32x32x16_bf16(f1, t.fb[ks][2], acc, 0, 0, 0);
+        acc = __builtin_amdgcn_mfma_f32_32x32x16_bf16(f2, t.fb[ks][0], acc, 0, 0, 0);
+        acc = __builtin_amdgcn_mfma_f32_32x32x16_bf16(f1, t.fb[ks][1], acc, 0, 0, 0);
+        acc = __builtin_amdgcn_mfma_f32_32x32x16_bf16(f1, t.fb[ks][0], acc, 0, 0, 0);
+    }
+    return acc;
+}
+
+__device__ __forceinline__ void stem_stat_add(float& cs, float& css, const float raw) {
+#pragma clang fp contract(off)
+    const float sq = raw * raw;
+    cs += raw;
+    css += sq;
+}
+
+template <typename T>
+__device__ __forceinline__ void stem_group_row(T s0, T s1, T (&sred)[4][32][2], float* __restrict__ row, const int Cout) {
+    const int tid = threadIdx.x, lane = tid & 63, wave = tid >> 6, fr = lane & 31, fh = lane >> 5;
+    s0 += __shfl_xor(s0, 32, 64);
+    s1 += __shfl_xor(s1, 32, 64);
+    if (fh == 0) { sred[wave][fr][0] = s0; sred[wave][fr][1] = s1; }
+    __syncthreads();
+    if (tid < 64) {
+        const int c = tid & 31, which = tid >> 5;
+        const T t = (sred[0][c][which] + sred[1][c][which]) + (sred[2][c][which] + sred[3][c][which]);
+        if (c < Cout) row[which * Cout + c] = (float)t;
+    }
+    __syncthreads();
+}
+
+template <bool STORE>
 __global__ __launch_bounds__(256) void conv_stem_fwd_bf16x3_kernel(const StemGeom g, const int ngroups, const float inv_hw,
                                                                    const float inv_w) {
     __shared__ float sred[4][32][2];
     const int tid = threadIdx.x, lane = tid & 63, wave = tid >> 6;
     const int fr = lane & 31, fh = lane >> 5;
     const int HW = g.H * g.W;
-    bf16x8 fb[2][3];
-    int koff[16];
-    int ktap[16];
-#pragma unroll
-    for (int i = 0; i < 16; ++i) {
-        const int k = (i >> 3) * 16 + fh * 8 + (i & 7);
-        const int r = k / 9, c = (k - r * 9) / 3, q = k - r * 9 - c * 3;
-        const bool kv = k < 27;
-        koff[i] = kv ? (int)(c * g.sxc + (r - 1) * g.sxh + (q - 1) * g.sxw) * 4 : 0;
-        ktap[i] = kv ? r * 3 + q : 9;
-    }
-#pragma unroll
-    for (int ks = 0; ks < 2; ++ks) {
-        f32x4 w0, w1;
-#pragma unroll
-        for (int i = 0; i < 8; ++i) {
-            const int k = ks * 16 + fh * 8 + i;
-            const int r = k / 9, c = (k - r * 9) / 3, q = k - r * 9 - c * 3;
-            const float v = (k < 27 && fr < g.Cout) ? g.w[fr * 27 + (r * 3 + q) * 3 + c] : 0.f;
-            if (i < 4) w0[i] = v; else w1[i - 4] = v;
-        }
-        u32x2 a1, a2, a3, b1, b2, b3;
-        split3x4(w0, a1, a2, a3);
-        split3x4(w1, b1, b2, b3);
-        const u32x4 q1 = {a1[0], a1[1], b1[0], b1[1]}, q2 = {a2[0], a2[1], b2[0], b2[1]}, q3 = {a3[0], a3[1], b3[0], b3[1]};
-        fb[ks][0] = __builtin_bit_cast(bf16x8, q1); fb[ks][1] = __builtin_bit_cast(bf16x8, q2); fb[ks][2] = __builtin_bit_cast(bf16x8, q3);
-    }
-    const float sc = (g.scale && fr < g.Cout) ? g.scale[fr] : 1.f;
-    const float sh = (g.shift && fr < g.Cout) ? g.shift[fr] : 0.f;
+    StemTileOps t;
+    stem_tile_setup(t, g, fr, fh);
+    const float sc = (STORE && g.scale && fr < g.Cout) ? g.scale[fr] : 1.f;
+    const float sh = (STORE && g.shift && fr < g.Cout) ? g.shift[fr] : 0.f;
     const __amdgpu_buffer_rsrc_t rsrc = y4_make_rsrc(g.x, 0xfffffff0u);
     float xv0[16], xv1[16];
-    auto load = [&](float (&xv)[16], long long tile) {
-        const long long p = tile * 32 + fr;
-        unsigned base = 0xffffffffu;
-        unsigned m9 = 0;
-        if (p < g.M) {
-            int b = (int)((float)p * inv_hw);
-            int rem = (int)(p - (long long)b * HW);
-            if (rem < 0) { --b; rem += HW; } else if (rem >= HW) { ++b; rem -= HW; }
-            int h = (int)((float)rem * inv_w);
-            int w = rem - h * g.W;
-            if (w < 0) { --h; w += g.W; } else if (w >= g.W) { ++h; w -= g.W; }
-            base = (unsigned)(b * g.sxb + h * g.sxh + w * g.sxw) * 4u;
-            const unsigned hm = (h > 0 ? 1u : 0u) | 2u | (h + 1 < g.H ? 4u : 0u);
-            const unsigned wm = (w > 0 ? 1u : 0u) | 2u | (w + 1 < g.W ? 4u : 0u);
-            m9 = ((hm & 1u) ? wm : 0u) | ((hm & 2u) ? wm << 3 : 0u) | ((hm & 4u) ? wm << 6 : 0u);
-        }
-#pragma unroll
-        for (int i = 0; i < 16; ++i) {
-            const bool ok = (m9 >> ktap[i]) & 1u;
-            xv[i] = __builtin_bit_cast(float, __builtin_amdgcn_raw_buffer_load_b32(rsrc, ok ? (int)(base + (unsigned)koff[i]) : -1, 0, 0));
-        }
-    };
     float cs = 0.f, css = 0.f;
     auto compute = [&](float (&xv)[16], long long tile) {
-        f32x16 acc;
-#pragma unroll
-        for (int e = 0; e < 16; ++e) acc[e] = 0.f;
-#pragma unroll
-        for (int ks = 0; ks < 2; ++ks) {
-            const f32x4 v0 = {xv[ks * 8 + 0], xv[ks * 8 + 1], xv[ks * 8 + 2], xv[ks * 8 + 3]};
-            const f32x4 v1 = {xv[ks * 8 + 4], xv[ks * 8 + 5], xv[ks * 8 + 6], xv[ks * 8 + 7]};
-            u32x2 a1, a2, a3, b1, b2, b3;
-            split3x4(v0, a1, a2, a3);
-            split3x4(v1, b1, b2, b3);
-            const u32x4 q1 = {a1[0], a1[1], b1[0], b1[1]}, q2 = {a2[0], a2[1], b2[0], b2[1]}, q3 = {a3[0], a3[1], b3[0], b3[1]};
-            const bf16x8 f1 = __builtin_bit_cast(bf16x8, q1), f2 = __builtin_bit_cast(bf16x8, q2), f3 = __builtin_bit_cast(bf16x8, q3);
-            acc = __builtin_amdgcn_mfma_f32_32x32x16_bf16(f3, fb[ks][0], acc, 0, 0, 0);
-            acc = __builtin_amdgcn_mfma_f32_32x32x16_bf16(f2, fb[ks][1], acc, 0, 0, 0);
-            acc = __builtin_amdgcn_mfma_f32_32x32x16_bf16(f1, fb[ks][2], acc, 0, 0, 0);
-            acc = __builtin_amdgcn_mfma_f32_32x32x16_bf16(f2, fb[ks][0], acc, 0, 0, 0);
-            acc = __builtin_amdgcn_mfma_f32_32x32x16_bf16(f1, fb[ks][1], acc, 0, 0, 0);
-            acc = __builtin_amdgcn_mfma_f32_32x32x16_bf16(f1, fb[ks][0], acc, 0, 0, 0);
-        }
+        const f32x16 acc = stem_tile_mma(t, xv);
         const long long mbase = tile * 32 + 4 * fh;
 #pragma unroll
         for (int e = 0; e < 16; ++e) {
             const float raw = acc[e];
-            cs += raw; css += raw * raw;
-            const long long m = mbase + (e & 3) + 8 * (e >> 2);
-            if (fr < g.Cout && m < g.M) g.y[m * g.ldy + fr] = y4_act(raw * sc + sh, g.act);
+            stem_stat_add(cs, css, raw);
+            if constexpr (STORE) {
+                const long long m = mbase + (e & 3) + 8 * (e >> 2);
+                if (fr < g.Cout && m < g.M) g.y[m * g.ldy + fr] = y4_act(raw * sc + sh, g.act);
+            }
         }
     };
     for (int grp = blockIdx.x; grp < ngroups; grp += gridDim.x) {
         const long long t0 = (long long)grp * 8 + wave * 2;
-        load(xv0, t0);
-        load(xv1, t0 + 1);
+        stem_tile_load(t, g, rsrc, HW, inv_hw, inv_w, fr, xv0, t0);
+        stem_tile_load(t, g, rsrc, HW, inv_hw, inv_w, fr, xv1, t0 + 1);
         cs = 0.f; css = 0.f;
         compute(xv0, t0);
         compute(xv1, t0 + 1);
-        if (g.stats) {
-            cs += __shfl_xor(cs, 32, 64);
-            css += __shfl_xor(css, 32, 64);
-            if (fh == 0) { sred[wave][fr][0] = cs; sred[wave][fr][1] = css; }
-            __syncthreads();
-            if (tid < 64) {
-                const int c = tid & 31, which = tid >> 5;
-                const float t = (sred[0][c][which] + sred[1][c][which]) + (sred[2][c][which] + sred[3][c][which]);
-                if (c < g.Cout) g.stats[((long long)grp * 2 + which) * g.Cout + c] = t;
-            }
-            __syncthreads();
-        }
+        if (g.stats) stem_group_row(cs, css, sred, g.stats + (long long)grp * 2 * g.Cout, g.Cout);
+    }
+}
+
+struct StemBnGeom {
+    StemGeom s;
+    int ngroups; float inv_hw, inv_w;
+    const float* mean; const float* invstd; const float* gamma; const float* beta;
+    unsigned* amax;
+    const float* dz; long long lddz;
+    const double* acc;
+    float* slabs;
+};
+
+__device__ __forceinline__ __amdgpu_buffer_rsrc_t stem_rows_rsrc(const float* t, const long long ld, const long long tile, const long long M) {
+    long long rows = M - tile * 32;
+    rows = rows < 0 ? 0 : (rows > 32 ? 32 : rows);
+    return y4_make_rsrc(rows > 0 ? t + tile * 32 * ld : t, (unsigned)(rows * ld * 4));
+}
+
+template <int ACT>
+__global__ __launch_bounds__(256) void conv_stem_bn_act_fwd_kernel(const StemBnGeom q) {
+    __shared__ unsigned wmax[4];
+    const StemGeom& g = q.s;
+    const int tid = threadIdx.x, lane = tid & 63, wave = __builtin_amdgcn_readfirstlane(tid >> 6);
+    const int fr = lane & 31, fh = lane >> 5;
+    const int HW = g.H * g.W;
+    StemTileOps t;
+    stem_tile_setup(t, g, fr, fh);
+    const bool nok = fr < g.Cout;
+    float a = 0.f, b = 0.f;
+    if (nok) {
+        a = q.invstd[fr] * q.gamma[fr];
+        b = fmaf(-q.mean[fr], a, q.beta[fr]);
+    }
+    const __amdgpu_buffer_rsrc_t rsrc = y4_make_rsrc(g.x, 0xfffffff0u);
+    const unsigned zo = nok ? (unsigned)((4 * fh) * g.ldy + fr) * 4u : 0xffffffffu;
+    const unsigned zrow = (unsigned)g.ldy * 4u;
+    unsigned amax = 0u;
+    float xv0[16], xv1[16];
+    auto emit = [&](float (&xv)[16], long long tile) {
+        const f32x16 acc = stem_tile_mma(t, xv);
+        const __amdgpu_buffer_rsrc_t zrs = stem_rows_rsrc(g.y, g.ldy, tile, g.M);
+        const int left = (int)((g.M - tile * 32 < 32 ? g.M - tile * 32 : 32)) - 4 * fh;
+#pragma unroll
+        for (int e = 0; e < 16; ++e) {
+            const int po = (e & 3) + 8 * (e >> 2);
+            const float o = y4_act_t<ACT>(fmaf(acc[e], a, b));
+            __builtin_amdgcn_raw_buffer_store_b32(__builtin_bit_cast(unsigned, o), zrs, nok ? (int)(zo + (unsigned)po * zrow) : -1, 0, 0);
+            const unsigned ob = __builtin_bit_cast(unsigned, o) & 0x7fffffffu;
+            if (nok && po < left && ob < 0x7f800000u && ob > amax) amax = ob;
+        }
+    };
+    for (int grp = blockIdx.x; grp < q.ngroups; grp += gridDim.x) {
+        const long long t0 = (long long)grp * 8 + wave * 2;
+        stem_tile_load(t, g, rsrc, HW, q.inv_hw, q.inv_w, fr, xv0, t0);
+        stem_tile_load(t, g, rsrc, HW, q.inv_hw, q.inv_w, fr, xv1, t0 + 1);
+        emit(xv0, t0);
+        emit(xv1, t0 + 1);
+    }
+    if (q.amax) {
+#pragma unroll
+        for (int off = 32; off > 0; off >>= 1) {
+            const unsigned o = (unsigned)__shfl_xor((int)amax, off, 64);
+            amax = o > amax ? o : amax;
+        }
+        if (lane == 0) wmax[wave] = amax;
+        __syncthreads();
+        if (tid == 0) {
+            unsigned v = wmax[0];
+#pragma unroll
+            for (int w = 1; w < 4; ++w) v = wmax[w] > v ? wmax[w] : v;
+            if (v > __hip_atomic_load(q.amax, __ATOMIC_RELAXED, __HIP_MEMORY_SCOPE_AGENT)) atomicMax(q.amax, v);
+        }
+    }
+}
+
+__device__ __forceinline__ void stem_dz_load(const StemBnGeom& q, const bool nok, const int fr, const int fh, float (&d)[16],
+                                             const long long tile) {
+    const __amdgpu_buffer_rsrc_t drs = stem_rows_rsrc(q.dz, q.lddz, tile, q.s.M);
+    const unsigned d_o = (unsigned)((4 * fh) * q.lddz + fr) * 4u, drow = (unsigned)q.lddz * 4u;
+#pragma unroll
+    for (int e = 0; e < 16; ++e)
+        d[e] = __builtin_bit_cast(float, __builtin_amdgcn_raw_buffer_load_b32(drs, nok ? (int)(d_o + (unsigned)((e & 3) + 8 * (e >> 2)) * drow) : -1, 0, 0));
+}
+
+template <int ACT>
+__global__ __launch_bounds__(256) void conv_stem_bn_bwd_reduce_kernel(const StemBnGeom q) {
+    __shared__ double sred[4][32][2];
+    const StemGeom& g = q.s;
+    const int tid = threadIdx.x, lane = tid & 63, wave = __builtin_amdgcn_readfirstlane(tid >> 6);
+    const int fr = lane & 31, fh = lane >> 5;
+    const int HW = g.H * g.W;
+    StemTileOps t;
+    stem_tile_setup(t, g, fr, fh);
+    const bool nok = fr < g.Cout;
+    const float mu = nok ? q.mean[fr] : 0.f, is = nok ? q.invstd[fr] : 0.f, ga = nok ? q.gamma[fr] : 0.f, be = nok ? q.beta[fr] : 0.f;
+    const __amdgpu_buffer_rsrc_t rsrc = y4_make_rsrc(g.x, 0xfffffff0u);
+    float xv[16], d[16];
+    for (int grp = blockIdx.x; grp < q.ngroups; grp += gridDim.x) {
+        double s = 0.0, sx = 0.0;
+#pragma unroll
+        for (int u = 0; u < 2; ++u) {
+            const long long tile = (long long)grp * 8 + wave * 2 + u;
+            stem_tile_load(t, g, rsrc, HW, q.inv_hw, q.inv_w, fr, xv, tile);
+            stem_dz_load(q, nok, fr, fh, d, tile);
+            const f32x16 acc = stem_tile_mma(t, xv);
+            const int left = (int)((g.M - tile * 32 < 32 ? g.M - tile * 32 : 32)) - 4 * fh;
+#pragma unroll
+            for (int e = 0; e < 16; ++e) {
+                const float xh = (acc[e] - mu) * is;
+                float gg = d[e] * y4_act_grad_t<ACT>(ga * xh + be);
+                if ((e & 3) + 8 * (e >> 2) >= left) gg = 0.f;
+                s += (double)gg;
+                sx = fma((double)gg, (double)xh, sx);
+            }
+        }
+        stem_group_row(s, sx, sred, g.stats + (long long)grp * 2 * g.Cout, g.Cout);
+    }
+}
+
+template <int ACT>
+__global__ __launch_bounds__(256) void conv_stem_bn_bwd_wgrad_kernel(const StemBnGeom q) {
+    const StemGeom& g = q.s;
+    const int tid = threadIdx.x, lane = tid & 63, wave = __builtin_amdgcn_readfirstlane(tid >> 6);
+    const int fr = lane & 31, fh = lane >> 5;
+    const int HW = g.H * g.W;
+    StemTileOps t;
+    stem_tile_setup(t, g, fr, fh);
+    const bool nok = fr < g.Cout;
+    const float mu = nok ? q.mean[fr] : 0.f, is = nok ? q.invstd[fr] : 0.f, ga = nok ? q.gamma[fr] : 0.f, be = nok ? q.beta[fr] : 0.f;
+    const double invM = 1.0 / (double)g.M;
+    const double k1 = nok ? q.acc[fr] * invM : 0.0, k2 = nok ? q.acc[g.Cout + fr] * invM : 0.0;
+    const double gi = (double)ga * (double)is;
+    const bool jok = fr < 27;
+    const int tap = jok ? fr / 3 : 0, jc = jok ? fr - tap * 3 : 0;
+    const int jr = tap / 3 - 1, jq = tap - (tap / 3) * 3 - 1;
+    const unsigned joff = (unsigned)(jc * g.sxc + jr * g.sxh + jq * g.sxw) * 4u;
+    const unsigned step_w = (unsigned)g.sxw * 4u, step_h = (unsigned)(g.sxh - g.W * g.sxw) * 4u, step_b = (unsigned)(g.sxb - g.H * g.sxh) * 4u;
+    const __amdgpu_buffer_rsrc_t rsrc = y4_make_rsrc(g.x, 0xfffffff0u);
+    double dw64[16];
+#pragma unroll
+    for (int e = 0; e < 16; ++e) dw64[e] = 0.0;
+    f32x16 zero;
+#pragma unroll
+    for (int e = 0; e < 16; ++e) zero[e] = 0.f;
+    float xv[16], d[16], bx[16];
+    for (int grp = blockIdx.x; grp < q.ngroups; grp += gridDim.x) {
+#pragma unroll 1
+        for (int u = 0; u < 2; ++u) {
+            const long long tile = (long long)grp * 8 + wave * 2 + u;
+            stem_tile_load(t, g, rsrc, HW, q.inv_hw, q.inv_w, fr, xv, tile);
+            stem_dz_load(q, nok, fr, fh, d, tile);
+            const long long p0 = tile * 32 + 4 * fh;
+            const int left = (int)(g.M - p0 < 32 ? g.M - p0 : 32);
+            int b = 0, h = 0, w = 0;
+            if (left > 0) stem_pixel(g, HW, q.inv_hw, q.inv_w, p0, b, h, w);
+            unsigned xo = (unsigned)(b * g.sxb + h * g.sxh + w * g.sxw) * 4u + joff;
+#pragma unroll
+            for (int e = 0; e < 16; ++e) {
+                const int hi = h + jr, wi = w + jq;
+                const bool ok = jok && (e & 3) + 8 * (e >> 2) < left && (unsigned)hi < (unsigned)g.H && (unsigned)wi < (unsigned)g.W;
+                bx[e] = __builtin_bit_cast(float, __builtin_amdgcn_raw_buffer_load_b32(rsrc, ok ? (int)xo : -1, 0, 0));
+                const int n = (e & 3) == 3 ? 5 : 1;
+                w += n; xo += (unsigned)n * step_w;
+                while (w >= g.W) { w -= g.W; xo += step_h; if (++h == g.H) { h = 0; xo += step_b; } }
+            }
+            const f32x16 acc = stem_tile_mma(t, xv);
+            f32x16 dw = zero;
+#pragma unroll
+            for (int e = 0; e < 16; ++e) {
+                const float xh = (acc[e] - mu) * is;
+                const float gg = d[e] * y4_act_grad_t<ACT>(ga * xh + be);
+                float dy = (float)(gi * fma(-(double)xh, k2, (double)gg - k1));
+                if ((e & 3) + 8 * (e >> 2) >= left) dy = 0.f;
+                dw = __builtin_amdgcn_mfma_f32_32x32x2f32(dy, bx[e], (e & 3) ? dw : zero, 0, 0, 0);
+                if ((e & 3) == 3) {
+#pragma unroll
+                    for (int i = 0; i < 16; ++i) dw64[i] += (double)dw[i];
+                }
+            }
+        }
+    }
+    float* out = q.slabs + ((long long)blockIdx.x * 4 + wave) * 1024;
+#pragma unroll
+    for (int e = 0; e < 16; ++e) {
+        const int n = (e & 3) + 8 * (e >> 2) + 4 * fh;
+        out[n * 32 + fr] = (float)dw64[e];
     }
 }
 
@@ -1950,7 +2173,7 @@
                          (long long)H * W < (1 << 24);
     if (mfma_ok) {
         const int grid = (int)(blocks < 2048 ? blocks : 2048);
-        hipLaunchKernelGGL(conv_stem_fwd_bf16x3_kernel, dim3(grid), dim3(256), 0, y4_stream(stream), g, (int)blocks,
+        hipLaunchKernelGGL(conv_stem_fwd_bf16x3_kernel<true>, dim3(grid), dim3(256), 0, y4_stream(stream), g, (int)blocks,
                            1.0f / (float)((long long)H * W), 1.0f / (float)W);
         Y4_CHECK_LAUNCH();
         return Y4_OK;
@@ -1993,4 +2216,110 @@
     return Y4_OK;
 }
 
-}
+#define Y4_STEM_ACT_SWITCH(ACTV, CALL)                                         \
+    switch (ACTV) {                                                            \
+        case Y4_ACT_MISH: { constexpr int A_ = Y4_ACT_MISH; CALL; } break;     \
+        case Y4_ACT_LEAKY: { constexpr int A_ = Y4_ACT_LEAKY; CALL; } break;   \
+        case Y4_ACT_RELU: { constexpr int A_ = Y4_ACT_RELU; CALL; } break;     \
+        default: { constexpr int A_ = Y4_ACT_LINEAR; CALL; } break;            \
+    }
+static int stem_bn_geom(StemBnGeom& q, const float* x, long long sxb, long long sxc, long long sxh, long long sxw, const float* w,
+                        int B, int H, int W, int Cout) {
+    if (B <= 0 || H <= 0 || W <= 0 || Cout <= 0 || Cout > 32 || (Cout & 3)) return Y4_ERR_SHAPE;
+    if (g_conv_mode < 1 || g_conv_mode > 3) return Y4_ERR_SHAPE;
+    if (sxb < 0 || sxc < 0 || sxh < 0 || sxw < 0 || (long long)H * W >= (1 << 24) ||
+        ((long long)(B - 1) * sxb + 2 * sxc + (long long)(H - 1) * sxh + (long long)(W - 1) * sxw + 1) * 4 >= 0xfffffff0ll)
+        return Y4_ERR_SHAPE;
+    StemGeom& g = q.s;
+    g.x = x; g.w = w;
+    g.sxb = sxb; g.sxc = sxc; g.sxh = sxh; g.sxw = sxw;
+    g.B = B; g.H = H; g.W = W; g.Cout = Cout; g.act = Y4_ACT_LINEAR;
+    g.M = (long long)B * H * W;
+    const long long groups = (g.M + 255) / 256;
+    if (groups >= (1ll << 31)) return Y4_ERR_SHAPE;
+    q.ngroups = (int)groups;
+    q.inv_hw = 1.0f / (float)((long long)H * W);
+    q.inv_w = 1.0f / (float)W;
+    return Y4_OK;
+}
+static inline int stem_grid(const StemBnGeom& q, int most) { return q.ngroups < most ? q.ngroups : most; }
+static inline bool stem_pitch_ok(long long ld, int Cout) { return ld >= Cout && ld < (1 << 24); }
+
+int y4_conv2d_stem_bn_stats_f32(const float* x, long long sxb, long long sxc, long long sxh, long long sxw,
+                                const float* w, int B, int H, int W, int Cout, float* bnstats_partials, void* stream) {
+    if (!x || !w || !bnstats_partials) return Y4_ERR_NULL;
+    StemBnGeom q{};
+    { const int rc = stem_bn_geom(q, x, sxb, sxc, sxh, sxw, w, B, H, W, Cout); if (rc != Y4_OK) return rc; }
+    q.s.stats = bnstats_partials;
+    hipLaunchKernelGGL(conv_stem_fwd_bf16x3_kernel<false>, dim3(stem_grid(q, 2048)), dim3(256), 0, y4_stream(stream), q.s, q.ngroups,
+                       q.inv_hw, q.inv_w);
+    Y4_CHECK_LAUNCH();
+    return Y4_OK;
+}
+
+int y4_conv2d_stem_bn_act_fwd_f32(const float* x, long long sxb, long long sxc, long long sxh, long long sxw,
+                                  const float* w, const float* mean, const float* invstd, const float* gamma, const float* beta,
+                                  int act, float* z, int ldz, int B, int H, int W, int Cout, unsigned* out_amax, void* stream) {
+    if (!x || !w || !mean || !invstd || !gamma || !beta || !z) return Y4_ERR_NULL;
+    StemBnGeom q{};
+    { const int rc = stem_bn_geom(q, x, sxb, sxc, sxh, sxw, w, B, H, W, Cout); if (rc != Y4_OK) return rc; }
+    if (!stem_pitch_ok(ldz, Cout)) return Y4_ERR_SHAPE;
+    q.s.y = z; q.s.ldy = ldz;
+    q.mean = mean; q.invstd = invstd; q.gamma = gamma; q.beta = beta; q.amax = out_amax;
+    hipStream_t st = y4_stream(stream);
+    const int grid = stem_grid(q, 2048);
+#define Y4_STEM_CALL hipLaunchKernelGGL(conv_stem_bn_act_fwd_kernel<A_>, dim3(grid), dim3(256), 0, st, q)
+    Y4_STEM_ACT_SWITCH(act, Y4_STEM_CALL);
+#undef Y4_STEM_CALL
+    Y4_CHECK_LAUNCH();
+    return Y4_OK;
+}
+
+size_t y4_conv2d_stem_bn_act_bwd_workspace(int B, int H, int W, int Cout) {
+    if (B <= 0 || H <= 0 || W <= 0 || Cout <= 0) return 0;
+    const size_t groups = (size_t)(((long long)B * H * W + 255) / 256);
+    const size_t rows = (groups * 2 * (size_t)Cout * sizeof(float) + 15) & ~(size_t)15;
+    return y4_bn_finalize_workspace(Cout) + rows + (size_t)STEM_WAVES * 1024 * sizeof(float) + 64 * 1024 * sizeof(double);
+}
+
+int y4_conv2d_stem_bn_act_bwd_f32(const float* x, long long sxb, long long sxc, long long sxh, long long sxw,
+                                  const float* w, const float* dz, int lddz,
+                                  const float* mean, const float* invstd, const float* gamma, const float* beta, int act,
+                                  float* dw, float* dgamma, float* dbeta, int B, int H, int W, int Cout,
+                                  void* workspace, size_t workspace_bytes, void* stream) {
+    if (!x || !w || !dz || !mean || !invstd || !gamma || !beta || !dw || !dgamma || !dbeta || !workspace) return Y4_ERR_NULL;
+    StemBnGeom q{};
+    { const int rc = stem_bn_geom(q, x, sxb, sxc, sxh, sxw, w, B, H, W, Cout); if (rc != Y4_OK) return rc; }
+    if (!stem_pitch_ok(lddz, Cout)) return Y4_ERR_SHAPE;
+    if (workspace_bytes < y4_conv2d_stem_bn_act_bwd_workspace(B, H, W, Cout)) return Y4_ERR_WORKSPACE;
+    char* ws = static_cast<char*>(workspace);
+    void* head = ws;
+    float* rows = reinterpret_cast<float*>(ws + y4_bn_finalize_workspace(Cout));
+    const size_t rows_bytes = ((size_t)q.ngroups * 2 * (size_t)Cout * sizeof(float) + 15) & ~(size_t)15;
+    float* slabs = reinterpret_cast<float*>(reinterpret_cast<char*>(rows) + rows_bytes);
+    double* part = reinterpret_cast<double*>(slabs + (size_t)STEM_WAVES * 1024);
+    q.s.stats = rows;
+    q.mean = mean; q.invstd = invstd; q.gamma = gamma; q.beta = beta;
+    q.dz = dz; q.lddz = lddz;
+    q.acc = static_cast<const double*>(head);
+    q.slabs = slabs;
+    hipStream_t st = y4_stream(stream);
+    const int rgrid = stem_grid(q, 2048);
+#define Y4_STEM_CALL hipLaunchKernelGGL(conv_stem_bn_bwd_reduce_kernel<A_>, dim3(rgrid), dim3(256), 0, st, q)
+    Y4_STEM_ACT_SWITCH(act, Y4_STEM_CALL);
+#undef Y4_STEM_CALL
+    Y4_CHECK_LAUNCH();
+    { const int rc = y4::bn_bwd_fold_finalize(rows, q.ngroups, Cout, head, dgamma, dbeta, gamma, invstd, q.s.M, st); if (rc != Y4_OK) return rc; }
+    const int wgrid = stem_grid(q, STEM_WAVES / 4);
+#define Y4_STEM_CALL hipLaunchKernelGGL(conv_stem_bn_bwd_wgrad_kernel<A_>, dim3(wgrid), dim3(256), 0, st, q)
+    Y4_STEM_ACT_SWITCH(act, Y4_STEM_CALL);
+#undef Y4_STEM_CALL
+    Y4_CHECK_LAUNCH();
+    hipLaunchKernelGGL(stem_wgrad_reduce1_kernel, dim3(64), dim3(256), 0, st, slabs, part, wgrid * 4);
+    Y4_CHECK_LAUNCH();
+    hipLaunchKernelGGL(stem_wgrad_reduce2_kernel, dim3(1), dim3(256), 0, st, part, dw, 64, Cout);
+    Y4_CHECK_LAUNCH();
+    return Y4_OK;
+}
+
+}
diff --git a/yolov4_amd/csrc/pointwise.hip b/yolov4_amd/csrc/pointwise.hip
--- a/yolov4_amd/csrc/pointwise.hip
+++ b/yolov4_amd/csrc/pointwise.hip
@@ -1020,6 +1020,24 @@
     return Y4_OK;
 }
 
+}
+
+namespace y4 {
+int bn_bwd_fold_finalize(const float* part, long long nparts, int C, void* head, float* dgamma, float* dbeta,
+                         const float* gamma, const float* invstd, long long M, hipStream_t st) {
+    double* acc = static_cast<double*>(head);
+    double* bacc = acc + 2 * C;
+    int nb = 0;
+    { const int rc = fold_partials(part, nparts, C, bacc, &nb, st); if (rc != Y4_OK) return rc; }
+    hipLaunchKernelGGL(bn_bwd_finalize_kernel, dim3((C + 31) / 32), dim3(256), 0, st, bacc, nb, C, acc, dgamma, dbeta, gamma,
+                       invstd, 1.0 / (double)M, static_cast<unsigned*>(nullptr));
+    Y4_CHECK_LAUNCH();
+    return Y4_OK;
+}
+}
+
+extern "C" {
+
 int y4_bn_act_bwd_f32(const float* dz, int lddz, const float* y, int ldy,
                       const float* mean, const float* invstd, const float* gamma, const float* beta,
                       int act, float* dy, int lddy, float* dgamma, float* dbeta,
diff --git a/yolov4_amd/ops.py b/yolov4_amd/ops.py
--- a/yolov4_amd/ops.py
+++ b/yolov4_amd/ops.py
@@ -301,6 +301,74 @@
                                         _ptr(running_mean), _ptr(running_var), _ptr(nbt), float(momentum), float(eps),
                                         _ptr(ws), wsb, _stream()), 'bn_finalize_partials')
     return y, mean, invstd
+
+
+_STEM_RECOMPUTE = os.environ.get('Y4_STEM_RECOMPUTE', '1') != '0'
+
+
+def stem_recompute_fits(x, w, k, s):
+    if x.dim() != 4 or w.dim() != 4 or x.dtype != torch.float32 or w.dtype != torch.float32:
+        return False
+    B, Cin, H, W = x.shape
+    Cout = w.shape[0]
+    if Cin != 3 or k != 3 or s != 1 or Cout > 32 or Cout % 4 or tuple(w.shape[1:]) != (3, 3, 3):
+        return False
+    if lib().y4_get_conv_mode() not in (1, 2, 3):
+        return False
+    sb, sc, sh, sw = x.stride()
+    if min(sb, sc, sh, sw) < 0 or H * W >= 1 << 24 or W < 2:
+        return False
+    return ((B - 1) * sb + 2 * sc + (H - 1) * sh + (W - 1) * sw + 1) * 4 < 0xfffffff0
+
+
+def stem_bn_act_fwd_raw(x, w, gamma, beta, act, running_mean, running_var, nbt, momentum, eps, out_amax=None):
+    L = lib()
+    B, _, H, W = x.shape
+    Cout = w.shape[0]
+    w = krsc(w)
+    sb, sc, sh, sw = x.stride()
+    M = B * H * W
+    part = _ws(L.y4_conv2d_bnstats_workspace(B, H, W, 3, Cout, 3, 1), x.device)
+    check(L.y4_conv2d_stem_bn_stats_f32(_ptr(x), sb, sc, sh, sw, _ptr(w), B, H, W, Cout, _ptr(part), _stream()),
+          'conv2d_stem_bn_stats')
+    mean = torch.empty(Cout, device=x.device, dtype=torch.float32)
+    invstd = torch.empty(Cout, device=x.device, dtype=torch.float32)
+    wsb = L.y4_bn_finalize_workspace(Cout)
+    ws = _ws(wsb, x.device)
+    check(L.y4_bn_finalize_partials_f32(_ptr(part), (M + 255) // 256, M, Cout, _ptr(mean), _ptr(invstd),
+                                        _ptr(running_mean), _ptr(running_var), _ptr(nbt), float(momentum), float(eps),
+                                        _ptr(ws), wsb, _stream()), 'bn_finalize_partials')
+    z = empty_nhwc(B, Cout, H, W, x.device)
+    check(L.y4_conv2d_stem_bn_act_fwd_f32(_ptr(x), sb, sc, sh, sw, _ptr(w), _ptr(mean), _ptr(invstd), _ptr(gamma), _ptr(beta),
+                                          ACT_IDS[act], _ptr(z), nhwc_pitch(z), B, H, W, Cout, _ptr(out_amax), _stream()),
+          'conv2d_stem_bn_act_fwd')
+    return z, mean, invstd
+
+
+def stem_bn_act_bwd_raw(dz, x, w, mean, invstd, gamma, beta, act, dw_out=None, dgamma_out=None, dbeta_out=None):
+    L = lib()
+    B, _, H, W = x.shape
+    Cout = w.shape[0]
+    dz, lddz = as_nhwc(dz, need_vec4=False)
+    if dw_out is not None and tuple(dw_out.shape) == tuple(w.shape) and _is_krsc_dense(dw_out) and dw_out.dtype == torch.float32:
+        dw = dw_out
+        WGRAD_STATS['in_place'] += 1
+    else:
+        WGRAD_STATS['temporary'] += 1
+        dw = krsc(torch.empty(tuple(w.shape), device=dz.device, dtype=torch.float32).contiguous(memory_format=CL))
+
+    def slot(t):
+        ok = t is not None and t.dtype == torch.float32 and tuple(t.shape) == (Cout,) and t.is_contiguous() and t.is_cuda
+        return t if ok else torch.empty(Cout, device=dz.device, dtype=torch.float32)
+    dgamma, dbeta = slot(dgamma_out), slot(dbeta_out)
+    w = krsc(w)
+    sb, sc, sh, sw = x.stride()
+    nbytes = L.y4_conv2d_stem_bn_act_bwd_workspace(B, H, W, Cout)
+    ws = _ws(nbytes, dz.device)
+    check(L.y4_conv2d_stem_bn_act_bwd_f32(_ptr(x), sb, sc, sh, sw, _ptr(w), _ptr(dz), lddz, _ptr(mean), _ptr(invstd),
+                                          _ptr(gamma), _ptr(beta), ACT_IDS[act], _ptr(dw), _ptr(dgamma), _ptr(dbeta),
+                                          B, H, W, Cout, _ptr(ws), nbytes, _stream()), 'conv2d_stem_bn_act_bwd')
+    return dw, dgamma, dbeta
 
 
 class Planes:
@@ -780,6 +848,19 @@
             if x.shape[0] * conv_out_hw(x.shape[2], x.shape[3], k, s)[0] * conv_out_hw(x.shape[2], x.shape[3], k, s)[1] <= 1:
                 raise ValueError('Expected more than 1 value per channel when training')
             ctx.dgrad_filter = None
+            if (_STEM_RECOMPUTE and residual is None and dest is None and not cfg.get('out_planes')
+                    and cfg.get('out_cat') is None and xp is None and not ctx.needs_input_grad[0]
+                    and all(cfg.get(key) is None for key in ('dres_put', 'dres_take', 'dx_put'))
+                    and stem_recompute_fits(x, weight, k, s)):
+                if f16x2_mode():
+                    z_amax = new_amax(x.device)
+                z, mean, invstd = stem_bn_act_fwd_raw(x, weight, gamma, beta, act, cfg['running_mean'], cfg['running_var'],
+                                                      cfg['nbt'], cfg['momentum'], cfg['eps'], out_amax=z_amax)
+                ctx.save_for_backward(x, weight, mean, invstd, gamma, beta)
+                ctx.mode = 'stem_train'
+                if io is not None:
+                    io['z_amax'] = z_amax
+                return z
             if ((f16 or (bfm and xp is not None)) and ctx.needs_input_grad[0] and x.shape[1] % 32 == 0 and fast_conv_shape(x.shape[1], k, s)
                     and weight.shape[0] % 4 == 0 and (xp is None or weight.shape[0] % 32 == 0)
                     and not (bfm and xp is not None and s == 2
@@ -879,6 +960,30 @@
         dy_amax = dy_pl = dyP = wq = None
         x_amax = live(ctx.x_amax)
         x_planes = getattr(ctx, 'x_planes', False)
+        if ctx.mode == 'stem_train':
+            x, weight, mean, invstd, gamma, beta = ctx.saved_tensors
+            gp, bp, wp = cfg.get('gamma_param'), cfg.get('beta_param'), cfg.get('weight_param')
+            sink = (gp is not None and bp is not None and getattr(gp, '_y4_grad_fresh', False)
+                    and getattr(bp, '_y4_grad_fresh', False) and gp.grad is not None and bp.grad is not None
+                    and ctx.needs_input_grad[3] and ctx.needs_input_grad[4])
+            wsink = (wp is not None and getattr(wp, '_y4_grad_fresh', False) and wp.grad is not None
+                     and ctx.needs_input_grad[1])
+            dw, dgamma, dbeta = stem_bn_act_bwd_raw(dz, x, weight, mean, invstd, gamma, beta, act,
+                                                    dw_out=wp.grad if wsink else None,
+                                                    dgamma_out=gp.grad if sink else None, dbeta_out=bp.grad if sink else None)
+            if sink and dgamma is gp.grad and dbeta is bp.grad:
+                gp._y4_grad_fresh = bp._y4_grad_fresh = False
+                gp._y4_grad_ready()
+                bp._y4_grad_ready()
+                dgamma = dbeta = None
+            if wsink:
+                wp._y4_grad_fresh = False
+                if dw is not wp.grad:
+                    wp.grad.add_(dw)
+                wp._y4_grad_ready()
+                dw = None
+            return (None, dw if ctx.needs_input_grad[1] else None, None, dgamma if ctx.needs_input_grad[3] else None,
+                    dbeta if ctx.needs_input_grad[4] else None, None, None)
         if ctx.mode in ('bn_train', 'bn_eval_grad'):
             x, weight, y, mean, invstd, gamma, beta = ctx.saved_tensors
             gp, bp = cfg.get('gamma_param'), cfg.get('beta_param')
```

Result: no change. 454.7, median of 6 (+0.5%).
